# chaoting-sun/GCT-Plus

Measured on AMD Instinct MI355X. Metric: SMILES/sec training step (vaetf, seq_len=80, d_model=512), higher is better.
Workload: dtype f32

## Files before the change

gct_plus_amd/csrc/gemm.hip:

```cpp
#include <limits.h>
#include <stdlib.h>

#include <type_traits>

#include "common.h"

typedef float f32x16 __attribute__((ext_vector_type(16)));

namespace {

constexpr int BM = 128, BN = 128, BK = 32;
constexpr int TILE_FLOATS = BM * BK;

struct Seg3 {
  const float* p0;
  int64_t d1, d2;
};

struct GemmArgs {
  int64_t M, N, K;
  Seg3 a;
  int64_t lda;
  int64_t a_nper;
  Seg3 b;
  int64_t ldb;
  int64_t b_nper;
  float* c0;
  int64_t c_d1, c_d2;
  int64_t ldc;
  int64_t c_nper;
  int64_t slab_stride;
  int64_t ksplit;
  int nsplit;
  int epi;
  const float* bias0;
  int64_t bias_d1, bias_d2;
  const float* resid;
  float* pre;
  const float* pre_in;
  float keep_scale;
  uint32_t thr;
  GctRng rng;
  float* bias_slab;
  int64_t row_base;
  const int32_t* quad_map;
  int64_t pre_rows;
  const int32_t* kt_list;
  const int32_t* kt_count;
  const uint16_t* bp0;
  int64_t bp_stride;
#ifdef GCT_STAMPS
  unsigned long long* stamps;
#endif
};

enum { EPI_SLAB = 32, EPI_D0 = 16 };

__device__ __forceinline__ int64_t pre_row0(const GemmArgs& g, int64_t row) {
  if (g.pre_rows <= 0 || !g.quad_map) return row;
  const int v = g.quad_map[(row + g.row_base) >> 2];
  return v < 0 ? -1 : (int64_t)v * 4;
}

__device__ __forceinline__ uint32_t drop_quad(const GemmArgs& g, int64_t row) {
  int64_t q = (row + g.row_base) >> 2;
  if (g.quad_map) {
    const int v = g.quad_map[q];
    q = v < 0 ? 0 : v;
  }
  return (uint32_t)q;
}

#ifdef GCT_STAMPS
#define STAMP(i)                                                                       \
  do {                                                                                 \
    __builtin_amdgcn_sched_barrier(0);                                                 \
    unsigned long long t__;                                                            \
    asm volatile("s_memtime %0\n\ts_waitcnt lgkmcnt(0)" : "=s"(t__)::"memory");         \
    __builtin_amdgcn_sched_barrier(0);                                                 \
    seg[i] += t__ - tprev;                                                             \
    tprev = t__;                                                                       \
  } while (0)
#else
#define STAMP(i)
#endif

__device__ __forceinline__ const float* seg_ptr(const Seg3& s, int64_t idx, int64_t nper,
                                                int64_t& local) {
  const bool g1 = idx >= nper, g2 = idx >= 2 * nper;
  local = idx - (g2 ? 2 * nper : (g1 ? nper : 0));
  return s.p0 + (g2 ? s.d2 : (g1 ? s.d1 : 0));
}

template <bool VEC, bool SEG_ON_K>
__device__ __forceinline__ void load_kc(float4 (&r)[4], const Seg3& s, int64_t ld, int64_t nper,
                                        int64_t row0, int64_t rows, int64_t k0, int64_t kend,
                                        int tid) {
  const int c8 = tid & 7;
  const int64_t k = k0 + c8 * 4;
#pragma unroll
  for (int i = 0; i < 4; ++i) {
    const int64_t row = row0 + (tid >> 3) + 32 * i;
    float4 v = make_float4(0.f, 0.f, 0.f, 0.f);
    if (row < rows) {
      if (VEC) {
        if (k < kend) {
          int64_t loc;
          const float* base;
          if (SEG_ON_K) {
            base = seg_ptr(s, k, nper, loc);
            v = *reinterpret_cast<const float4*>(base + row * ld + loc);
          } else {
            base = seg_ptr(s, row, nper, loc);
            v = *reinterpret_cast<const float4*>(base + loc * ld + k);
          }
        }
      } else {
        float t[4] = {0.f, 0.f, 0.f, 0.f};
#pragma unroll
        for (int e = 0; e < 4; ++e) {
          if (k + e < kend) {
            int64_t loc;
            if (SEG_ON_K) {
              const float* base = seg_ptr(s, k + e, nper, loc);
              t[e] = base[row * ld + loc];
            } else {
              const float* base = seg_ptr(s, row, nper, loc);
              t[e] = base[loc * ld + k + e];
            }
          }
        }
        v = make_float4(t[0], t[1], t[2], t[3]);
      }
    }
    r[i] = v;
  }
}

template <bool VEC, bool SEG_ON_K>
__device__ __forceinline__ void load_rc(float4 (&r)[4], const Seg3& s, int64_t ld, int64_t nper,
                                        int64_t col0, int64_t cols, int64_t k0, int64_t kend,
                                        int tid) {
  const int c32 = tid & 31;
  const int64_t col = col0 + c32 * 4;
#pragma unroll
  for (int i = 0; i < 4; ++i) {
    const int64_t k = k0 + (tid >> 5) + 8 * i;
    float4 v = make_float4(0.f, 0.f, 0.f, 0.f);
    if (k < kend) {
      if (VEC) {
        if (col < cols) {
          int64_t loc;
          if (SEG_ON_K) {
            const float* base = seg_ptr(s, k, nper, loc);
            v = *reinterpret_cast<const float4*>(base + loc * ld + col);
          } else {
            const float* base = seg_ptr(s, col, nper, loc);
            v = *reinterpret_cast<const float4*>(base + k * ld + loc);
          }
        }
      } else {
        float t[4] = {0.f, 0.f, 0.f, 0.f};
#pragma unroll
        for (int e = 0; e < 4; ++e) {
          if (col + e < cols) {
            int64_t loc;
            if (SEG_ON_K) {
              const float* base = seg_ptr(s, k, nper, loc);
              t[e] = base[loc * ld + col + e];
            } else {
              const float* base = seg_ptr(s, col + e, nper, loc);
              t[e] = base[k * ld + loc];
            }
          }
        }
        v = make_float4(t[0], t[1], t[2], t[3]);
      }
    }
    r[i] = v;
  }
}

__device__ __forceinline__ void store_kc(float* lds, const float4 (&r)[4], int tid) {
  const int c8 = tid & 7;
#pragma unroll
  for (int i = 0; i < 4; ++i) {
    const int row = (tid >> 3) + 32 * i;
    const int chunk = c8 ^ ((row >> 1) & 7);
    *reinterpret_cast<float4*>(lds + row * BK + chunk * 4) = r[i];
  }
}
__device__ __forceinline__ void store_rc(float* lds, const float4 (&r)[4], int tid) {
  const int c32 = tid & 31;
#pragma unroll
  for (int i = 0; i < 4; ++i) {
    const int k = (tid >> 5) + 8 * i;
    *reinterpret_cast<float4*>(lds + k * BM + c32 * 4) = r[i];
  }
}

__device__ __forceinline__ void fragq_kc(float (&f)[2][4], const float* lds, int base, int lane,
                                         int c) {
  const int h = lane >> 5;
#pragma unroll
  for (int t = 0; t < 2; ++t) {
    const int row = base + t * 32 + (lane & 31);
    const int sw = (row >> 1) & 7;
    const float4 v = *reinterpret_cast<const float4*>(lds + row * BK + (((h * 4 + c) ^ sw) * 4));
    f[t][0] = v.x; f[t][1] = v.y; f[t][2] = v.z; f[t][3] = v.w;
  }
}
__device__ __forceinline__ void fragq_rc(float (&f)[2][4], const float* lds, int base, int lane,
                                         int c) {
  const int h = lane >> 5;
#pragma unroll
  for (int t = 0; t < 2; ++t) {
    const int col = base + t * 32 + (lane & 31);
#pragma unroll
    for (int e = 0; e < 4; ++e) f[t][e] = lds[(h * 16 + c * 4 + e) * BM + col];
  }
}

template <bool A_KC, bool B_KC, bool VEC>
__global__ __launch_bounds__(256, 2) void gemm_f32_kernel(const GemmArgs g) {
  __shared__ __attribute__((aligned(16))) float lds[4 * TILE_FLOATS];
  const int tid = threadIdx.x, lane = tid & 63, wave = tid >> 6;
  const int wm = (wave >> 1) * 64, wn = (wave & 1) * 64;

  const unsigned tiles_n = (unsigned)((g.N + BN - 1) / BN);
  const unsigned tiles_m = (unsigned)((g.M + BM - 1) / BM);
  const unsigned per_split = tiles_m * tiles_n;
  const unsigned lid = gct_xcd_remap(blockIdx.x, gridDim.x);
  const unsigned z = lid / per_split, rest = lid - z * per_split;
  const int64_t m0 = (int64_t)(rest / tiles_n) * BM, n0 = (int64_t)(rest % tiles_n) * BN;
  const int64_t kbeg = (int64_t)z * g.ksplit;
  const int64_t kend = (kbeg + g.ksplit < g.K) ? kbeg + g.ksplit : g.K;

  const Seg3 sa = g.a, sb = g.b;

  f32x16 acc[2][2];
#pragma unroll
  for (int i = 0; i < 2; ++i)
#pragma unroll
    for (int j = 0; j < 2; ++j)
#pragma unroll
      for (int r = 0; r < 16; ++r) acc[i][j][r] = 0.f;

  float4 ra[4], rb[4];
  auto gload = [&](int64_t k0) {
    if (A_KC)
      load_kc<VEC, true>(ra, sa, g.lda, g.a_nper, m0, g.M, k0, kend, tid);
    else
      load_rc<VEC, false>(ra, sa, g.lda, g.a_nper, m0, g.M, k0, kend, tid);
    if (B_KC)
      load_kc<VEC, false>(rb, sb, g.ldb, g.b_nper, n0, g.N, k0, kend, tid);
    else
      load_rc<VEC, true>(rb, sb, g.ldb, g.b_nper, n0, g.N, k0, kend, tid);
  };
  auto lstore = [&](int buf) {
    float* la = lds + buf * 2 * TILE_FLOATS;
    float* lb = la + TILE_FLOATS;
    if (A_KC) store_kc(la, ra, tid); else store_rc(la, ra, tid);
    if (B_KC) store_kc(lb, rb, tid); else store_rc(lb, rb, tid);
  };

  const int64_t nkt = (kend - kbeg + BK - 1) / BK;
#ifdef GCT_STAMPS
  unsigned long long seg[8] = {0, 0, 0, 0, 0, 0, 0, 0}, tprev;
  asm volatile("s_memtime %0\n\ts_waitcnt lgkmcnt(0)" : "=s"(tprev)::"memory");
#endif
  if (nkt > 0) {
    gload(kbeg);
    lstore(0);
  }
  __syncthreads();
  STAMP(0);
  for (int64_t kt = 0; kt < nkt; ++kt) {
    const int cur = (int)(kt & 1);
    if (kt + 1 < nkt) gload(kbeg + (kt + 1) * BK);
    STAMP(1);
    const float* la = lds + cur * 2 * TILE_FLOATS;
    const float* lb = la + TILE_FLOATS;
    float fa[2][2][4], fb[2][2][4];
    auto fragq = [&](int set, int c) {
      if (A_KC) fragq_kc(fa[set], la, wm, lane, c); else fragq_rc(fa[set], la, wm, lane, c);
      if (B_KC) fragq_kc(fb[set], lb, wn, lane, c); else fragq_rc(fb[set], lb, wn, lane, c);
    };
    fragq(0, 0);
#pragma unroll
    for (int c = 0; c < 4; ++c) {
      const int set = c & 1;
      if (c < 3) fragq(set ^ 1, c + 1);
      __builtin_amdgcn_sched_barrier(0);
#pragma unroll
      for (int e = 0; e < 4; ++e) {
#pragma unroll
        for (int i = 0; i < 2; ++i)
#pragma unroll
          for (int j = 0; j < 2; ++j)
            acc[i][j] = __builtin_amdgcn_mfma_f32_32x32x2f32(fa[set][i][e], fb[set][j][e], acc[i][j],
                                                             0, 0, 0);
      }
      __builtin_amdgcn_sched_barrier(0);
    }
    STAMP(2);
#ifdef GCT_STAMPS
    asm volatile("s_waitcnt vmcnt(0)" ::: "memory");
    STAMP(3);
#endif
    if (kt + 1 < nkt) lstore(cur ^ 1);
    STAMP(4);
    __syncthreads();
    STAMP(5);
  }

  const int h = lane >> 5;
#pragma unroll
  for (int i = 0; i < 2; ++i) {
#pragma unroll
    for (int j = 0; j < 2; ++j) {
      const int64_t col = n0 + wn + j * 32 + (lane & 31);
      if (col >= g.N) continue;
      int64_t cloc;
      float* cbase;
      float bias = 0.f;
      if (g.epi == EPI_SLAB) {
        cbase = g.c0 + (int64_t)z * g.slab_stride;
        cloc = col;
      } else {
        const bool g1 = col >= g.c_nper, g2 = col >= 2 * g.c_nper;
        cloc = col - (g2 ? 2 * g.c_nper : (g1 ? g.c_nper : 0));
        cbase = g.c0 + (g2 ? g.c_d2 : (g1 ? g.c_d1 : 0));
        if (g.epi < EPI_D0 && g.bias0)
          bias = g.bias0[(g2 ? g.bias_d2 : (g1 ? g.bias_d1 : 0)) + cloc];
      }
#pragma unroll
      for (int q4 = 0; q4 < 4; ++q4) {
        const int64_t row_base = m0 + wm + i * 32 + 8 * q4 + 4 * h;
        uint4 bits = make_uint4(~0u, ~0u, ~0u, ~0u);
        const bool need_rng = g.thr != 0u && (g.epi == GCT_EPI_GELU_DROP ||
                                              g.epi == GCT_EPI_GELU_DROP_SAVE ||
                                              g.epi == GCT_EPI_DROP_RESID ||
                                              g.epi == EPI_D0 + GCT_DEPI_GELU_BWD);
        if (need_rng) bits = gct_drop_bits(g.rng, drop_quad(g, row_base), (uint32_t)col);
#pragma unroll
        for (int e = 0; e < 4; ++e) {
          const int64_t row = row_base + e;
          if (row >= g.M) continue;
          float v = acc[i][j][q4 * 4 + e];
          const int64_t off = row * g.ldc + cloc;
          const bool keep = gct_drop_keep(bits, e, (uint32_t)col, g.thr);
          switch (g.epi) {
            case GCT_EPI_BIAS:
              v += bias;
              break;
            case GCT_EPI_GELU_DROP: {
// ... 568 lines not shown
    if (kt + 1 < nkt) gload(kbeg + (kt + 1) * BK);
    const float* la = lds + cur * 2 * STILE;
    const float* lb = la + STILE;
    const int rowa = wm + (lane & 31), rowb = wn + (lane & 31);
    const int swa = (rowa >> 1) & 7, swb = (rowb >> 1) & 7;
#pragma unroll
    for (int c = 0; c < 4; ++c) {
      const float4 a4 = *reinterpret_cast<const float4*>(la + rowa * BK + (((h * 4 + c) ^ swa) * 4));
      const float4 b4 = *reinterpret_cast<const float4*>(lb + rowb * BK + (((h * 4 + c) ^ swb) * 4));
      acc = __builtin_amdgcn_mfma_f32_32x32x2f32(a4.x, b4.x, acc, 0, 0, 0);
      acc = __builtin_amdgcn_mfma_f32_32x32x2f32(a4.y, b4.y, acc, 0, 0, 0);
      acc = __builtin_amdgcn_mfma_f32_32x32x2f32(a4.z, b4.z, acc, 0, 0, 0);
      acc = __builtin_amdgcn_mfma_f32_32x32x2f32(a4.w, b4.w, acc, 0, 0, 0);
    }
    if (kt + 1 < nkt) lstore(cur ^ 1);
    __syncthreads();
  }
  float* stg = lds + wave * 1024;
  {
    const int c32 = lane & 31;
#pragma unroll
    for (int r = 0; r < 16; ++r) stg[((r & 3) + 8 * (r >> 2) + 4 * h) * 32 + c32] = acc[r];
  }
  __builtin_amdgcn_s_waitcnt(0xC07F);
  __builtin_amdgcn_wave_barrier();
  const FastEpi ep{g};
  const int rg = lane >> 3, c4 = lane & 7;
  const int64_t row0 = m0 + wm + rg * 4, col0 = n0 + wn + c4 * 4;
  if (row0 < g.M && col0 < g.N) {
    float4 v[4];
#pragma unroll
    for (int rr = 0; rr < 4; ++rr) v[rr] = *reinterpret_cast<const float4*>(stg + (rg * 4 + rr) * 32 + c4 * 4);
    if (g.epi == EPI_SLAB) {
      float* sl = g.c0 + (int64_t)z * g.slab_stride;
#pragma unroll
      for (int rr = 0; rr < 4; ++rr)
        if (row0 + rr < g.M) *reinterpret_cast<float4*>(sl + (row0 + rr) * g.N + col0) = v[rr];
      return;
    }
    const bool q1 = col0 >= g.c_nper, q2 = col0 >= 2 * g.c_nper;
    const int64_t cloc = col0 - (q2 ? 2 * g.c_nper : (q1 ? g.c_nper : 0));
    float* cbase = g.c0 + (q2 ? g.c_d2 : (q1 ? g.c_d1 : 0));
    float4 bias = make_float4(0.f, 0.f, 0.f, 0.f);
    if (g.bias0) bias = *reinterpret_cast<const float4*>(g.bias0 + (q2 ? g.bias_d2 : (q1 ? g.bias_d1 : 0)) + cloc);
    ep.apply(v, row0, col0, cbase, cloc, bias);
  }
}


template <int TN, bool RAGGED = false>
__global__ __launch_bounds__(256) void gemm_f32_panel_kernel(const GemmArgs g) {
  constexpr int TM = 32, KC = 256, SD = KC + 4, NBL = TN / 4;
  extern __shared__ __attribute__((aligned(16))) float plds[];
  float* As = plds;
  float* Bs = plds + TM * SD;
  const int tid = threadIdx.x, lane = tid & 63, wave = tid >> 6, g4 = lane >> 4, c16 = lane & 15;
  const unsigned tiles_m = (unsigned)((g.M + TM - 1) / TM);
  const unsigned lid = gct_xcd_remap(blockIdx.x, gridDim.x);
  const int64_t m0 = (int64_t)(lid % tiles_m) * TM, n0 = (int64_t)(lid / tiles_m) * TN;
  const bool s1 = n0 >= g.b_nper, s2 = n0 >= 2 * g.b_nper;
  const float* bbase = g.b.p0 + (s2 ? g.b.d2 : (s1 ? g.b.d1 : 0)) + (n0 - (s2 ? 2 * g.b_nper : (s1 ? g.b_nper : 0))) * g.ldb;
  const float* abase = g.a.p0;
  uint32_t offa[8], offb[NBL];
#pragma unroll
  for (int i = 0; i < 8; ++i) {
    const int idx = tid + 256 * i, row = idx >> 6, c4 = idx & 63;
    int64_t r = m0 + row;
    if (r > g.M - 1) r = g.M - 1;
    offa[i] = (uint32_t)(r * g.lda + c4 * 4);
  }
#pragma unroll
  for (int i = 0; i < NBL; ++i) {
    const int idx = tid + 256 * i, c4 = idx & 63;
    int64_t row = idx >> 6;
    if (RAGGED && n0 + row > g.N - 1) row = g.N - 1 - n0;
    offb[i] = (uint32_t)(row * g.ldb + c4 * 4);
  }
  f32x4_t ra[8], rb[NBL];
  auto gload = [&](int64_t k0) {
#pragma unroll
    for (int i = 0; i < 8; ++i) ra[i] = *reinterpret_cast<const f32x4_t*>(abase + k0 + offa[i]);
#pragma unroll
    for (int i = 0; i < NBL; ++i) rb[i] = *reinterpret_cast<const f32x4_t*>(bbase + k0 + offb[i]);
  };
  auto lstore = [&]() {
#pragma unroll
    for (int i = 0; i < 8; ++i) {
      const int idx = tid + 256 * i;
      *reinterpret_cast<f32x4_t*>(As + (idx >> 6) * SD + (idx & 63) * 4) = ra[i];
    }
#pragma unroll
    for (int i = 0; i < NBL; ++i) {
      const int idx = tid + 256 * i;
      *reinterpret_cast<f32x4_t*>(Bs + (idx >> 6) * SD + (idx & 63) * 4) = rb[i];
    }
  };
  constexpr int NS = TN / 32;
  const int wm = (wave >> 1) * 16, wn = (wave & 1) * (TN / 2);
  f32x4_t acc[NS];
#pragma unroll
  for (int j = 0; j < NS; ++j) acc[j] = (f32x4_t){0.f, 0.f, 0.f, 0.f};
  const int64_t nch = g.K / KC;
  gload(0);
  lstore();
  __syncthreads();
  for (int64_t c = 0; c < nch; ++c) {
    if (c + 1 < nch) gload((c + 1) * KC);
    const float* ap = As + (wm + c16) * SD + g4 * 64;
#pragma unroll 4
    for (int j = 0; j < 16; ++j) {
      const float4 a4 = *reinterpret_cast<const float4*>(ap + 4 * j);
#pragma unroll
      for (int u = 0; u < NS; ++u) {
        const float4 b4 = *reinterpret_cast<const float4*>(Bs + (wn + 16 * u + c16) * SD + g4 * 64 + 4 * j);
        acc[u] = __builtin_amdgcn_mfma_f32_16x16x4f32(a4.x, b4.x, acc[u], 0, 0, 0);
        acc[u] = __builtin_amdgcn_mfma_f32_16x16x4f32(a4.y, b4.y, acc[u], 0, 0, 0);
        acc[u] = __builtin_amdgcn_mfma_f32_16x16x4f32(a4.z, b4.z, acc[u], 0, 0, 0);
        acc[u] = __builtin_amdgcn_mfma_f32_16x16x4f32(a4.w, b4.w, acc[u], 0, 0, 0);
      }
    }
    __syncthreads();
    if (c + 1 < nch) {
      lstore();
      __syncthreads();
    }
  }
  float* stg = plds + wave * (16 * 20);
  const FastEpi ep{g};
#pragma unroll
  for (int u = 0; u < NS; ++u) {
#pragma unroll
    for (int i = 0; i < 4; ++i) stg[(4 * g4 + i) * 20 + c16] = acc[u][i];
    __builtin_amdgcn_s_waitcnt(0xC07F);
    __builtin_amdgcn_wave_barrier();
    if (lane < 16) {
      const int pr = lane >> 2, pc = lane & 3;
      const int64_t row0 = m0 + wm + 4 * pr, col0 = n0 + wn + 16 * u + 4 * pc;
      if (RAGGED) {
        for (int rr = 0; rr < 4; ++rr)
          for (int cc = 0; cc < 4; ++cc)
            if (row0 + rr < g.M && col0 + cc < g.N)
              g.c0[(row0 + rr) * g.ldc + col0 + cc] = stg[(4 * pr + rr) * 20 + 4 * pc + cc] + (g.bias0 ? g.bias0[col0 + cc] : 0.f);
      } else if (row0 < g.M && col0 < g.N) {
        float4 v[4];
#pragma unroll
        for (int rr = 0; rr < 4; ++rr) v[rr] = *reinterpret_cast<const float4*>(stg + (4 * pr + rr) * 20 + 4 * pc);
        const bool q1 = col0 >= g.c_nper, q2 = col0 >= 2 * g.c_nper;
        const int64_t cloc = col0 - (q2 ? 2 * g.c_nper : (q1 ? g.c_nper : 0));
        float* cbase = g.c0 + (q2 ? g.c_d2 : (q1 ? g.c_d1 : 0));
        float4 bias = make_float4(0.f, 0.f, 0.f, 0.f);
        if (g.bias0) bias = *reinterpret_cast<const float4*>(g.bias0 + (q2 ? g.bias_d2 : (q1 ? g.bias_d1 : 0)) + cloc);
        ep.apply(v, row0, col0, cbase, cloc, bias);
      }
    }
    __builtin_amdgcn_s_waitcnt(0xC07F);
    __builtin_amdgcn_wave_barrier();
  }
}

template <int TN, bool RAGGED = false>
int launch_panel(const GemmArgs& g, hipStream_t st) {
  constexpr size_t LDS = (size_t)(32 + TN) * 260 * sizeof(float);
  static bool attr_set = false;
  if (!attr_set) {
    hipError_t e = hipFuncSetAttribute((const void*)gemm_f32_panel_kernel<TN, RAGGED>, hipFuncAttributeMaxDynamicSharedMemorySize, (int)LDS);
    if (e != hipSuccess) {
      gct_set_error("gemm_f32_panel: cannot reserve %zu bytes of LDS: %s", LDS, hipGetErrorString(e));
      return GCT_ERR_HIP;
    }
    attr_set = true;
  }
  const int64_t tiles = ((g.M + 31) / 32) * (RAGGED ? 1 : g.N / TN);
  hipLaunchKernelGGL((gemm_f32_panel_kernel<TN, RAGGED>), dim3((unsigned)tiles), dim3(256), LDS, st, g);
  GCT_LAUNCH_CHECK("gemm_f32_panel");
  return GCT_OK;
}

__global__ __launch_bounds__(256) void splitk_epilogue_kernel(const GemmArgs g, const float* slabs,
                                                              int nslab, int64_t slab_stride) {
  const int64_t pc = g.N / 4, pr = (g.M + 3) / 4;
  const int64_t idx = (int64_t)blockIdx.x * blockDim.x + threadIdx.x;
  if (idx >= pc * pr) return;
  const int64_t row0 = (idx / pc) * 4, col0 = (idx % pc) * 4;
  float4 v[4];
#pragma unroll
  for (int rr = 0; rr < 4; ++rr) {
    v[rr] = make_float4(0.f, 0.f, 0.f, 0.f);
    if (row0 + rr < g.M) {
      const float* p = slabs + (row0 + rr) * g.N + col0;
      for (int s = 0; s < nslab; ++s) {
        const float4 t = *reinterpret_cast<const float4*>(p + (int64_t)s * slab_stride);
        v[rr].x += t.x; v[rr].y += t.y; v[rr].z += t.z; v[rr].w += t.w;
      }
    }
  }
  const bool q1 = col0 >= g.c_nper, q2 = col0 >= 2 * g.c_nper;
  const int64_t cloc = col0 - (q2 ? 2 * g.c_nper : (q1 ? g.c_nper : 0));
  float* cbase = g.c0 + (q2 ? g.c_d2 : (q1 ? g.c_d1 : 0));
  float4 bias = make_float4(0.f, 0.f, 0.f, 0.f);
  if (g.bias0) bias = *reinterpret_cast<const float4*>(g.bias0 + (q2 ? g.bias_d2 : (q1 ? g.bias_d1 : 0)) + cloc);
  const FastEpi ep{g};
  ep.apply(v, row0, col0, cbase, cloc, bias);
}

int g_gemm_mode = -1;
int64_t g_gemm_launches[2] = {0, 0};
inline int gemm_mode() {
  if (g_gemm_mode < 0) {
    const char* e = getenv("GCT_GEMM_MODE");
    g_gemm_mode = (e && (e[0] == 'f' || e[0] == '0')) ? GCT_GEMM_F32 : GCT_GEMM_BF16X6;
  }
  return g_gemm_mode;
}

template <bool A_KC, bool B_KC>
bool fast_ok(const GemmArgs& g, bool vec) {
  auto seg_ok = [](int64_t nper, int64_t extent, int64_t gran) { return nper >= extent || nper % gran == 0; };
  return vec && g.K % BK == 0 && g.ksplit % BK == 0 && g.M >= 4 && g.N >= 4 &&
         (A_KC ? seg_ok(g.a_nper, g.K, BK) : (seg_ok(g.a_nper, g.M, BM) && g.M % 4 == 0)) &&
         (B_KC ? seg_ok(g.b_nper, g.N, BN) : (seg_ok(g.b_nper, g.K, BK) && g.N % 4 == 0)) &&
         g.N % 4 == 0 && g.ldc % 4 == 0 && gct_aligned16(g.c0) && g.c_d1 % 4 == 0 && g.c_d2 % 4 == 0 &&
         (g.c_nper >= g.N || g.c_nper % 4 == 0) && g.slab_stride % 4 == 0 &&
         (!g.bias0 || (gct_aligned16(g.bias0) && g.bias_d1 % 4 == 0 && g.bias_d2 % 4 == 0)) &&
         (!g.resid || gct_aligned16(g.resid)) && (!g.pre || gct_aligned16(g.pre)) &&
         (!g.pre_in || gct_aligned16(g.pre_in)) && 130 * g.lda < (1ll << 31) && 130 * g.ldb < (1ll << 31);
}


inline int64_t slab_bytes(int64_t s, int64_t rows, int64_t cols) {
  return s > 1 ? s * rows * cols * (int64_t)sizeof(float) : 0;
}

inline bool skinny_m(int64_t M, int64_t N) { return ((M + BM - 1) / BM) * ((N + BN - 1) / BN) < 192; }

int skinny_splits(int64_t M, int64_t N, int64_t K) {
  const int64_t tiles = ((M + 63) / 64) * ((N + 63) / 64);
  if (tiles <= 0) return 1;
  int64_t ns = 768 / tiles;
  if (ns > K / BK / 4) ns = K / BK / 4;
  return ns < 1 ? 1 : (int)ns;
}

int x6_tail_plan(int64_t M, int64_t N, int64_t K, int64_t* m1_out) {
  constexpr int64_t CUS = 256;
  const int64_t tm = (M + XBM - 1) / XBM, tn = (N + XBN - 1) / XBN, tiles = tm * tn;
  const int64_t rem = tiles % CUS;
  if (tiles <= CUS || rem == 0 || rem % tn != 0 || K % XBK != 0) return 1;
  const int64_t nkt = K / XBK;
  int best = 1;
  double cost = 1.0;
  const double o = 3.3;
  for (int s2 = 2; s2 <= 8 && nkt / s2 >= 2; ++s2) {
    const double c = (double)((rem * s2 + CUS - 1) / CUS) * (o + (double)nkt / s2) / (o + nkt) + 0.05;
    if (c < cost - 1e-9) { cost = c; best = s2; }
  }
  if (best == 1 || cost > 0.75) return 1;
  *m1_out = (tiles - rem) / tn * XBM;
  return best;
}

int x6_splitk_all_plan(int64_t M, int64_t N, int64_t K) {
  constexpr int64_t CUS = 256;
  const int64_t tiles = ((M + XBM - 1) / XBM) * ((N + XBN - 1) / XBN), nkt = K / XBK;
  if (tiles > CUS / 2 || K % XBK != 0 || nkt < 32 || M < 1024 || (nkt < 64 && M < 2048)) return 1;
  int64_t sp = CUS / tiles;
  if (sp > nkt / 8) sp = nkt / 8;
  if (sp > 8) sp = 8;
  return sp < 2 ? 1 : (int)sp;
}


inline int64_t x6s_tiles(int64_t M, int64_t N) { return ((M + SBM - 1) / SBM) * ((N + SBN - 1) / SBN); }

inline bool x6s_shape(const GemmArgs& g) {
  const int64_t big = ((g.M + XBM - 1) / XBM) * ((g.N + XBN - 1) / XBN), small = x6s_tiles(g.M, g.N), nkt = g.K / XBK;
  return big <= 160 && small >= 96 && small <= (nkt <= 16 ? 512 : 256) && nkt <= 32;
}

constexpr int64_t X6_TAIL_SMALL_MAX = 512;

constexpr int64_t PANEL32_MAX_TILES = 4096, PANEL64_MAX_TILES = 768;


static_assert(BK == XBK, "the fp32 and bf16x6 kernels split K at the same granularity");
GemmArgs slab_args(const GemmArgs& g, int splits, float* ws) {
  const int64_t nkt = g.K / BK;
  GemmArgs p = g;
  p.ksplit = ((nkt + splits - 1) / splits) * BK;
  p.nsplit = (int)((g.K + p.ksplit - 1) / p.ksplit);
  p.epi = EPI_SLAB; p.c0 = ws; p.ldc = g.N; p.slab_stride = g.M * g.N;
  p.c_d1 = p.c_d2 = 0; p.c_nper = INT64_MAX / 4; p.bias0 = nullptr; p.resid = nullptr; p.pre = nullptr; p.pre_in = nullptr;
  return p;
}

int launch_fixup(const GemmArgs& g, const GemmArgs& slabs, hipStream_t st, const char* name) {
  const int64_t patches = ((g.M + 3) / 4) * (g.N / 4);
  hipLaunchKernelGGL(splitk_epilogue_kernel, dim3((unsigned)((patches + 255) / 256)), dim3(256), 0, st, g,
                     (const float*)slabs.c0, slabs.nsplit, slabs.slab_stride);
  GCT_LAUNCH_CHECK(name);
  return GCT_OK;
}

template <int MODE, int NP>
int launch_x6_tail_split(const GemmArgs& g, hipStream_t st, float* ws, int64_t ws_bytes) {
  if (MODE == X6_WGRAD || g.nsplit != 1 || !ws || !gct_aligned16(ws)) return launch_x6<MODE, NP>(g, st);
  int64_t m1 = 0;
  const int best = x6_tail_plan(g.M, g.N, g.K, &m1);
  const int64_t m2 = g.M - m1, nkt = g.K / XBK;
  hipStreamCaptureStatus cap = hipStreamCaptureStatusNone;
  if (best == 1 || slab_bytes(best, m2, g.N) > ws_bytes ||
      hipStreamIsCapturing(st, &cap) != hipSuccess || cap != hipStreamCaptureStatusNone)
    return launch_x6<MODE, NP>(g, st);
  GemmArgs head = g;
  head.M = m1;
  int rc = launch_x6<MODE, NP>(head, st);
  if (rc) return rc;
  GemmArgs e = g;
  e.M = m2; e.row_base = g.row_base + m1;
  e.a.p0 += m1 * g.lda;
  e.c0 += m1 * g.ldc;
  if (e.resid) e.resid += m1 * g.ldc;
  if (e.pre) e.pre += m1 * g.ldc;
  if (e.pre_in && !(g.pre_rows > 0 && g.quad_map)) e.pre_in += m1 * g.ldc;
  if (nkt <= 32 && x6s_tiles(m2, g.N) <= X6_TAIL_SMALL_MAX) {
    if (MODE == X6_FWD && x6s_ok(e, true)) return launch_x6s<X6_FWD, NP>(e, st);
    if (MODE == X6_DGRAD && x6s_dgrad_ok(e, true)) return launch_x6s<X6_DGRAD, NP>(e, st);
  }
  const GemmArgs p = slab_args(e, best, ws);
  rc = launch_x6<MODE, NP>(p, st);
  if (rc) return rc;
  return launch_fixup(e, p, st, "x6 tail fix-up");
}

struct GemmRoute {
  enum Kind {
    X6S,
    X6_SPLITK_ALL,
    PANEL_THIN,
    PANEL32,
    PANEL64,
    F32_SMALL,
    X6,
    F32_FAST,
    F32_VEC,
    F32,
  } kind;
  int splits;
};

template <bool A_KC, bool B_KC>
GemmRoute plan_gemm(const GemmArgs& g, bool vec, int mode, const float* ws, int64_t ws_bytes) {
  constexpr bool FWD = A_KC && B_KC, DGRAD = A_KC && !B_KC;
  constexpr int MODE = A_KC ? (B_KC ? X6_FWD : X6_DGRAD) : X6_WGRAD;
  const bool x6 = mode == GCT_GEMM_BF16X6 || mode == GCT_GEMM_BF16X3;
  const bool x6_fwd = x6 && FWD && g.epi < EPI_D0, x6_dgrad = x6 && DGRAD && g.epi >= EPI_D0 && g.epi < EPI_SLAB;
  const bool ws_ok = ws && gct_aligned16(ws);
  if (x6_fwd || x6_dgrad) {
    const bool x6s = x6_fwd ? x6s_ok(g, vec) : x6s_dgrad_ok(g, vec);
    if (x6s && x6s_shape(g)) return {GemmRoute::X6S, 1};
    if (x6_fwd && x6s && !x6_ok<X6_FWD>(g, vec) && x6s_tiles(g.M, g.N) >= 96) return {GemmRoute::X6S, 1};
    const int sp = x6_splitk_all_plan(g.M, g.N, g.K);
    if (x6_ok<MODE>(g, vec) && g.nsplit == 1 && ws_ok && sp > 1 && slab_bytes(sp, g.M, g.N) <= ws_bytes)
      return {GemmRoute::X6_SPLITK_ALL, sp};
  }
  if (FWD && vec && g.N <= 32 && g.K % 256 == 0 && g.epi == GCT_EPI_BIAS && g.nsplit == 1 && g.b_nper >= g.N &&
      g.c_nper >= g.N && g.M >= 1 && g.lda * 4 * 33 < (1ll << 31) && g.ldb * 4 * 33 < (1ll << 31) && g.M < (1ll << 36))
    return {GemmRoute::PANEL_THIN, 1};
  const bool fast = fast_ok<A_KC, B_KC>(g, vec);
  if (FWD && fast && g.nsplit == 1 && skinny_m(g.M, g.N) && g.epi < EPI_D0 && (g.b_nper >= g.N || g.b_nper % 64 == 0)) {
    if (g.K % 256 == 0 && g.lda * 4 * 33 < (1ll << 31) && g.ldb * 4 * 65 < (1ll << 31) &&
        (g.c_nper >= g.N || g.c_nper % 64 == 0)) {
      const int64_t tm32 = (g.M + 31) / 32;
      if (g.N % 32 == 0 && (g.b_nper >= g.N || g.b_nper % 32 == 0) && tm32 * (g.N / 32) <= PANEL32_MAX_TILES)
        return {GemmRoute::PANEL32, 1};
      if (g.N % 64 == 0 && tm32 * (g.N / 64) <= PANEL64_MAX_TILES) return {GemmRoute::PANEL64, 1};
    }
    int64_t ns = 1;
    if (ws_ok) {
      const int64_t slab = g.M * g.N * (int64_t)sizeof(float);
      ns = skinny_splits(g.M, g.N, g.K);
      if (ns * slab > ws_bytes) ns = ws_bytes / slab;
      if (ns < 1) ns = 1;
    }
    return {GemmRoute::F32_SMALL, (int)ns};
  }
  if (x6 && (A_KC || !B_KC) && x6_ok<MODE>(g, vec)) return {GemmRoute::X6, 1};
  return {fast ? GemmRoute::F32_FAST : (vec ? GemmRoute::F32_VEC : GemmRoute::F32), 1};
}

template <bool A_KC, bool B_KC>
int launch(const GemmArgs& g, bool vec, hipStream_t st, float* ws = nullptr, int64_t ws_bytes = 0) {
  constexpr int MODE = A_KC ? (B_KC ? X6_FWD : X6_DGRAD) : X6_WGRAD;
  const int64_t tiles = ((g.M + BM - 1) / BM) * ((g.N + BN - 1) / BN) * g.nsplit;
  if (tiles <= 0) return GCT_OK;
  if (tiles > INT_MAX) {
    gct_set_error("gemm: grid too large");
    return GCT_ERR_ARG;
  }
  const int mode = gemm_mode();
  const bool x3 = mode == GCT_GEMM_BF16X3;
  const GemmRoute r = plan_gemm<A_KC, B_KC>(g, vec, mode, ws, ws_bytes);
  switch (r.kind) {
    case GemmRoute::X6S:
      if (x3) return launch_x6s<B_KC ? X6_FWD : X6_DGRAD, 2>(g, st);
      ++g_gemm_launches[1];
      return launch_x6s<B_KC ? X6_FWD : X6_DGRAD, 3>(g, st);
    case GemmRoute::X6_SPLITK_ALL: {
      const GemmArgs p = slab_args(g, r.splits, ws);
      int rc = x3 ? launch_x6<MODE, 2>(p, st) : launch_x6<MODE, 3>(p, st);
      if (!rc) rc = launch_fixup(g, p, st, "x6 split-K fix-up");
      if (!rc && !x3) ++g_gemm_launches[1];
      return rc;
    }
    case GemmRoute::PANEL_THIN:
      ++g_gemm_launches[0];
      return launch_panel<32, true>(g, st);
    case GemmRoute::PANEL32:
      return launch_panel<32>(g, st);
    case GemmRoute::PANEL64:
      return launch_panel<64>(g, st);
    case GemmRoute::F32_SMALL: {
      const int64_t tiles64 = ((g.M + 63) / 64) * ((g.N + 63) / 64);
      if (r.splits == 1) {
        hipLaunchKernelGGL(gemm_f32_small_kernel, dim3((unsigned)tiles64), dim3(256), 0, st, g);
        GCT_LAUNCH_CHECK("gemm_f32_small");
        return GCT_OK;
      }
      const GemmArgs p = slab_args(g, r.splits, ws);
      hipLaunchKernelGGL(gemm_f32_small_kernel, dim3((unsigned)(tiles64 * p.nsplit)), dim3(256), 0, st, p);
      GCT_LAUNCH_CHECK("gemm_f32_small(split-K)");
      return launch_fixup(g, p, st, "splitk_epilogue");
    }
    case GemmRoute::X6:
      if (x3) return launch_x6_tail_split<MODE, 2>(g, st, ws, ws_bytes);
      ++g_gemm_launches[1];
      return launch_x6_tail_split<MODE, 3>(g, st, ws, ws_bytes);
    default:
      break;
  }
  ++g_gemm_launches[0];
  const dim3 grid((unsigned)tiles), block(256);
  if (r.kind == GemmRoute::F32_FAST)
    hipLaunchKernelGGL((gemm_f32_fast_kernel<A_KC, B_KC>), grid, block, 0, st, g);
  else if (r.kind == GemmRoute::F32_VEC)
    hipLaunchKernelGGL((gemm_f32_kernel<A_KC, B_KC, true>), grid, block, 0, st, g);
  else
    hipLaunchKernelGGL((gemm_f32_kernel<A_KC, B_KC, false>), grid, block, 0, st, g);
  GCT_LAUNCH_CHECK("gemm_f32");
  return GCT_OK;
}

inline bool al16(const void* p) { return p == nullptr || gct_aligned16(p); }

inline Seg3 mkseg(const float* p0, const float* p1, const float* p2) {
  Seg3 r;
  r.p0 = p0;
  r.d1 = p1 ? (int64_t)(p1 - p0) : 0;
  r.d2 = p2 ? (int64_t)(p2 - p0) : 0;
  return r;
}

}

int gct_reduce_slabs_seg(const float* slabs, int nslab, int64_t stride, float* d0, float* d1,
                         float* d2, int64_t nper_elems, int64_t n, hipStream_t st);
int gct_reduce_slabs_seg2(const float* sa, int nslab, int64_t stride_a, float* a0, float* a1, float* a2,
                          int64_t nper_a, int64_t na, const float* sb, int64_t stride_b, float* b0, float* b1,
                          float* b2, int64_t nper_b, int64_t nb, hipStream_t st);
int gct_colsum(const float* y0, const float* y1, const float* y2, int64_t ld, int64_t M, int nseg,
               int nper, float* d0, float* d1, float* d2, float* ws, hipStream_t st);
int64_t gct_colsum_ws_floats(int64_t M, int64_t N);

static int wgrad_splits(int64_t M, int64_t Ntot, int64_t K, bool x6 = false) {
  const int64_t tiles = x6 ? ((Ntot + XBM - 1) / XBM) * ((K + XBN - 1) / XBN)
                           : ((Ntot + BM - 1) / BM) * ((K + BN - 1) / BN);
  int64_t want = (x6 ? 256 : 512) / tiles;
  const int64_t maxs = (M + 4 * BK - 1) / (4 * BK);
  if (want > maxs) want = maxs;
  if (want < 1) want = 1;
  if (want > 64) want = 64;
  return (int)want;
}

extern "C" int64_t gct_wgrad_ws_bytes(int64_t M, int64_t Ntot, int64_t K) {
  const int s1 = wgrad_splits(M, Ntot, K), s2 = wgrad_splits(M, Ntot, K, true);
  const int s = s1 > s2 ? s1 : s2;
  const int64_t slab = (int64_t)s * Ntot * K;
  const int64_t cs = gct_colsum_ws_floats(M, Ntot);
  const int64_t need = slab + 4 + (int64_t)s * Ntot;
  return (need > cs ? need : cs) * (int64_t)sizeof(float) + 256;
}

extern "C" int gct_linear_fwd(const float* x, int64_t ldx, int64_t M, int K, const float* w0,
                              const float* w1, const float* w2, int64_t ldw, const uint16_t* wp0,
                              int64_t plane_stride, const float* b0, const float* b1,
                              const float* b2, int nseg, int nper, float* y0, float* y1, float* y2,
                              int64_t ldy, int epi, const float* resid, float* pre, float p,
                              uint64_t seed, uint32_t site, float* ws, int64_t ws_bytes,
                              const int32_t* quad_map, void* stream) {
  GCT_CHECK_ARG(x && w0 && y0 && M >= 0 && K > 0 && nseg >= 1 && nseg <= 3 && nper > 0,
                "linear_fwd: bad args");
  GCT_CHECK_ARG(!quad_map || M % 4 == 0, "linear_fwd: compacted rows come in quads");
  GCT_CHECK_ARG(ws_bytes >= 0, "linear_fwd: negative workspace size");
  GCT_CHECK_ARG(nseg < 2 || (w1 && y1), "linear_fwd: missing segment 1");
  GCT_CHECK_ARG(nseg < 3 || (w2 && y2), "linear_fwd: missing segment 2");
  GCT_CHECK_ARG(epi == GCT_EPI_BIAS || nseg == 1, "linear_fwd: fused epilogues need nseg == 1");
  GCT_CHECK_ARG(epi >= GCT_EPI_BIAS && epi <= GCT_EPI_GELU_DROP_SAVE, "linear_fwd: unknown epilogue %d", epi);
  GCT_CHECK_ARG((epi != GCT_EPI_GELU_DROP && epi != GCT_EPI_GELU_DROP_SAVE) || pre, "linear_fwd: GELU epilogue needs pre");
  GCT_CHECK_ARG(epi != GCT_EPI_DROP_RESID || resid, "linear_fwd: residual epilogue needs resid");
  GCT_CHECK_ARG(p >= 0.f && p < 1.f, "linear_fwd: dropout p out of range");
  GemmArgs g = {};
  g.M = M; g.N = (int64_t)nseg * nper; g.K = K;
  GCT_CHECK_ARG(!b0 || nseg < 2 || b1, "linear_fwd: bias of segment 1 missing");
  GCT_CHECK_ARG(!b0 || nseg < 3 || b2, "linear_fwd: bias of segment 2 missing");
  g.a = mkseg(x, nullptr, nullptr); g.lda = ldx; g.a_nper = INT64_MAX / 4;
  g.b = mkseg(w0, w1, w2); g.ldb = ldw; g.b_nper = nper;
  g.c0 = y0; g.c_d1 = y1 ? y1 - y0 : 0; g.c_d2 = y2 ? y2 - y0 : 0; g.ldc = ldy; g.c_nper = nper;
  g.ksplit = K; g.nsplit = 1; g.epi = epi;
  g.bias0 = b0; g.bias_d1 = (b0 && b1) ? b1 - b0 : 0; g.bias_d2 = (b0 && b2) ? b2 - b0 : 0;
  g.resid = resid; g.pre = pre;
  g.thr = gct_drop_threshold(p); g.keep_scale = 1.0f / (1.0f - p); g.rng = gct_rng_make(seed, site);
  g.bp0 = wp0; g.bp_stride = plane_stride;
  g.quad_map = quad_map;
  const bool vec = al16(x) && al16(w0) && al16(w1) && al16(w2) && (ldx % 4 == 0) &&
                   (ldw % 4 == 0) && (K % 4 == 0);
  return launch<true, true>(g, vec, (hipStream_t)stream, ws, ws ? ws_bytes : 0);
}

extern "C" int gct_gemm_set_mode(int mode) {
  GCT_CHECK_ARG(mode == GCT_GEMM_F32 || mode == GCT_GEMM_BF16X6 || mode == GCT_GEMM_BF16X3,
                "gemm_set_mode: unknown mode %d", mode);
  g_gemm_mode = mode;
  return GCT_OK;
}
extern "C" int gct_gemm_get_mode(void) { return gemm_mode(); }
extern "C" int64_t gct_gemm_x6_kernel_launches(void) { return g_x6_kernel_launches; }
extern "C" int64_t gct_gemm_x3_launches(void) { return g_x3_kernel_launches; }
extern "C" int gct_gemm_launch_counts(int64_t* out2) {
  GCT_CHECK_ARG(out2, "gemm_launch_counts: null");
  out2[0] = g_gemm_launches[0]; out2[1] = g_gemm_launches[1];
  return GCT_OK;
}

extern "C" int gct_split_planes(const float* src, int64_t numel, uint16_t* planes, int64_t plane_stride,
                                void* stream) {
  GCT_CHECK_ARG(src && planes && numel >= 0 && numel % 4 == 0 && plane_stride >= numel && plane_stride % 4 == 0 &&
                    gct_aligned16(src) && ((((uintptr_t)planes) & 7u) == 0),
                "split_planes: bad args (numel and plane_stride must be multiples of 4, src 16-B aligned)");
  if (numel == 0) return GCT_OK;
  const int64_t n4 = numel / 4;
  hipLaunchKernelGGL(split_planes_kernel, dim3((unsigned)((n4 + 255) / 256)), dim3(256), 0, (hipStream_t)stream,
                     src, planes, n4, plane_stride);
  GCT_LAUNCH_CHECK("split_planes");
  return GCT_OK;
}

extern "C" int64_t gct_linear_fwd_ws_bytes(int64_t M, int K, int Ntot) {
  int64_t need = 0, m1 = 0;
  if (skinny_m(M, Ntot)) {
    need = slab_bytes(skinny_splits(M, Ntot, K), M, Ntot);
  } else {
    const int s = x6_tail_plan(M, Ntot, K, &m1);
    need = slab_bytes(s, M - m1, Ntot);
  }
  const int64_t all = slab_bytes(x6_splitk_all_plan(M, Ntot, K), M, Ntot);
  return (need > all ? need : all) + 256;
}

extern "C" int64_t gct_linear_dgrad_ws_bytes(int64_t M, int Ntot, int K) {
  int64_t m1 = 0;
  const int s = x6_tail_plan(M, K, Ntot, &m1);
  const int64_t tail = slab_bytes(s, M - m1, K);
  const int64_t all = slab_bytes(x6_splitk_all_plan(M, K, Ntot), M, K);
  return (tail > all ? tail : all) + 256;
}

extern "C" int gct_linear_dgrad(const float* dy0, const float* dy1, const float* dy2, int64_t lddy,
                                int64_t M, int nseg, int nper, const float* w0, const float* w1,
                                const float* w2, int64_t ldw, const uint16_t* wp0,
                                int64_t plane_stride, int K, float* dx, int64_t lddx, int depi,
                                const float* pre, float p, uint64_t seed, uint32_t site,
                                float* ws, int64_t ws_bytes, const int32_t* quad_map, int64_t pre_rows,
                                void* stream) {
  GCT_CHECK_ARG(ws_bytes >= 0, "linear_dgrad: negative workspace size");
  GCT_CHECK_ARG(dy0 && w0 && dx && M >= 0 && K > 0 && nseg >= 1 && nseg <= 3 && nper > 0,
                "linear_dgrad: bad args");
  GCT_CHECK_ARG(!quad_map || M % 4 == 0, "linear_dgrad: compacted rows come in quads");
  GCT_CHECK_ARG(nseg < 2 || (w1 && dy1), "linear_dgrad: missing segment 1");
  GCT_CHECK_ARG(nseg < 3 || (w2 && dy2), "linear_dgrad: missing segment 2");
  GCT_CHECK_ARG(depi >= GCT_DEPI_STORE && depi <= GCT_DEPI_MUL_SAVED, "linear_dgrad: unknown epilogue %d", depi);
  GCT_CHECK_ARG(depi != GCT_DEPI_GELU_BWD || pre, "linear_dgrad: GELU bwd needs pre");
  GCT_CHECK_ARG(depi != GCT_DEPI_MUL_SAVED || pre, "linear_dgrad: saved-factor epilogue needs pre");
  GCT_CHECK_ARG(p >= 0.f && p < 1.f, "linear_dgrad: dropout p out of range");
  GemmArgs g = {};
  g.M = M; g.N = K; g.K = (int64_t)nseg * nper;
  g.a = mkseg(dy0, dy1, dy2); g.lda = lddy; g.a_nper = nper;
  g.b = mkseg(w0, w1, w2); g.ldb = ldw; g.b_nper = nper;
  g.c0 = dx; g.ldc = lddx; g.c_nper = INT64_MAX / 4;
  g.ksplit = g.K; g.nsplit = 1; g.epi = EPI_D0 + depi;
  g.pre_in = pre;
  g.thr = gct_drop_threshold(p); g.keep_scale = 1.0f / (1.0f - p); g.rng = gct_rng_make(seed, site);
  g.bp0 = wp0; g.bp_stride = plane_stride;
  g.quad_map = quad_map;
  g.pre_rows = quad_map ? pre_rows : 0;
  const bool vec = al16(dy0) && al16(dy1) && al16(dy2) && al16(w0) && al16(w1) && al16(w2) &&
                   (lddy % 4 == 0) && (ldw % 4 == 0) && (nper % 4 == 0) && (K % 4 == 0);
  return launch<true, false>(g, vec, (hipStream_t)stream, ws, ws ? ws_bytes : 0);
}

extern "C" int gct_linear_wgrad(const float* dy0, const float* dy1, const float* dy2, int64_t lddy,
                                int64_t M, int nseg, int nper, const float* x, int64_t ldx, int K,
                                float* dw0, float* dw1, float* dw2, int64_t lddw, float* db0,
                                float* db1, float* db2, float* ws, const int32_t* tile_list,
                                const int32_t* tile_count, void* stream) {
  GCT_CHECK_ARG(dy0 && x && dw0 && ws && M >= 0 && K > 0 && nseg >= 1 && nseg <= 3 && nper > 0,
                "linear_wgrad: bad args");
  GCT_CHECK_ARG(nseg < 2 || (dy1 && dw1), "linear_wgrad: missing segment 1");
  GCT_CHECK_ARG(nseg < 3 || (dy2 && dw2), "linear_wgrad: missing segment 2");
  GCT_CHECK_ARG(lddw == K, "linear_wgrad: dW must be dense [nper][K]");
  hipStream_t st = (hipStream_t)stream;
  const int64_t Ntot = (int64_t)nseg * nper;
  const bool vec = al16(dy0) && al16(dy1) && al16(dy2) && al16(x) && (lddy % 4 == 0) &&
                   (ldx % 4 == 0) && (nper % 4 == 0) && (K % 4 == 0);
  GemmArgs g = {};
  g.M = Ntot; g.N = K; g.K = M;
  g.a = mkseg(dy0, dy1, dy2); g.lda = lddy; g.a_nper = nper;
  g.b = mkseg(x, nullptr, nullptr); g.ldb = ldx; g.b_nper = INT64_MAX / 4;
  g.c0 = ws; g.ldc = K; g.c_nper = INT64_MAX / 4;
  g.slab_stride = Ntot * K;
  g.ksplit = BK; g.nsplit = 1; g.epi = EPI_SLAB;
  const bool use_x6 = gemm_mode() != GCT_GEMM_F32 && x6_ok<X6_WGRAD>(g, vec);
  if (use_x6 && tile_list && tile_count) { g.kt_list = tile_list; g.kt_count = tile_count; }
  const int splits = wgrad_splits(M, Ntot, K, use_x6);
  int64_t ks = (M + splits - 1) / splits;
  ks = (ks + BK - 1) / BK * BK;
  g.ksplit = ks > 0 ? ks : BK;
  g.nsplit = (int)((M + g.ksplit - 1) / g.ksplit);
  if (g.nsplit < 1) g.nsplit = 1;
  g.epi = EPI_SLAB;
  float* bslab = nullptr;
  if (db0) {
    if (use_x6 || fast_ok<false, false>(g, vec)) {
      int64_t off = (int64_t)g.nsplit * g.slab_stride;
      off = (off + 3) / 4 * 4;
      bslab = ws + off;
      g.bias_slab = bslab;
    } else {
      int rc = gct_colsum(dy0, dy1, dy2, lddy, M, nseg, nper, db0, db1, db2, ws, st);
      if (rc) return rc;
    }
  }
  int rc = launch<false, false>(g, vec, st);
  if (rc) return rc;
  if (bslab)
    return gct_reduce_slabs_seg2(ws, g.nsplit, g.slab_stride, dw0, dw1, dw2, (int64_t)nper * K, Ntot * K, bslab, Ntot,
                                 db0, db1, db2, nper, Ntot, st);
  return gct_reduce_slabs_seg(ws, g.nsplit, g.slab_stride, dw0, dw1, dw2, (int64_t)nper * K, Ntot * K, st);
}
```

gct_plus_amd/csrc/gemm_x6.inc:

```

typedef __bf16 x6_bf16x8 __attribute__((ext_vector_type(8)));
typedef __bf16 x6_bf16x2 __attribute__((ext_vector_type(2)));
typedef float x6_f32x2 __attribute__((ext_vector_type(2)));
typedef unsigned x6_u32x4 __attribute__((ext_vector_type(4)));
typedef unsigned x6_u32x2 __attribute__((ext_vector_type(2)));
typedef short x6_s16x4 __attribute__((ext_vector_type(4)));
typedef short x6_s16x8 __attribute__((ext_vector_type(8)));

enum { X6_FWD = 0, X6_DGRAD = 1, X6_WGRAD = 2 };
constexpr int XBM = 128, XBN = 256, XBK = 32;
constexpr int X_APL = 8192, X_BPL = 16384, X_STAGE = 3 * X_APL + 3 * X_BPL;
constexpr int X_KLIST_MAX = 1024;
constexpr int X_LDS_BYTES = 2 * X_STAGE + X_KLIST_MAX * 4;

__device__ __forceinline__ unsigned x6_pk(float a, float b) {
  x6_f32x2 v = {a, b};
  return __builtin_bit_cast(unsigned, __builtin_convertvector(v, x6_bf16x2));
}
__device__ __forceinline__ float x6_sub(float a, float b) {
  float r;
  asm("v_sub_f32 %0, %1, %2" : "=v"(r) : "v"(a), "v"(b));
  return r;
}
__device__ __forceinline__ void x6_split2(float a, float b, unsigned& h, unsigned& m, unsigned& l) {
  h = x6_pk(a, b);
  const float ra = x6_sub(a, __uint_as_float(h << 16)), rb = x6_sub(b, __uint_as_float(h & 0xffff0000u));
  m = x6_pk(ra, rb);
  const float sa = x6_sub(ra, __uint_as_float(m << 16)), sb = x6_sub(rb, __uint_as_float(m & 0xffff0000u));
  l = x6_pk(sa, sb);
}
__device__ __forceinline__ void x6_split4(const float4 v, x6_u32x2& h, x6_u32x2& m, x6_u32x2& l) {
  unsigned h0, m0, l0, h1, m1, l1;
  x6_split2(v.x, v.y, h0, m0, l0);
  x6_split2(v.z, v.w, h1, m1, l1);
  h = x6_u32x2{h0, h1}; m = x6_u32x2{m0, m1}; l = x6_u32x2{l0, l1};
}
template <int NP>
__device__ __forceinline__ void x6_split4n(const float4 v, x6_u32x2 (&pc)[NP]) {
  if constexpr (NP == 3) {
    x6_split4(v, pc[0], pc[1], pc[2]);
  } else {
    static_assert(NP == 2, "bf16x6 (3 pieces) or bf16x3 (2 pieces)");
    unsigned h0, h1;
    h0 = x6_pk(v.x, v.y);
    h1 = x6_pk(v.z, v.w);
    const float r0 = x6_sub(v.x, __uint_as_float(h0 << 16)), r1 = x6_sub(v.y, __uint_as_float(h0 & 0xffff0000u));
    const float r2 = x6_sub(v.z, __uint_as_float(h1 << 16)), r3 = x6_sub(v.w, __uint_as_float(h1 & 0xffff0000u));
    pc[0] = x6_u32x2{h0, h1};
    pc[1] = x6_u32x2{x6_pk(r0, r1), x6_pk(r2, r3)};
  }
}

__device__ __forceinline__ int x6_row_off(int r, int c) {
  const int g = (0x78 >> (2 * ((r >> 2) & 3))) & 3;
  return r * 64 + ((c ^ g) << 4);
}
__device__ __forceinline__ int x6_tr_off(int k, int cb, int stride) {
  return k * stride + (cb ^ (((k & 3) << 6) | (((k >> 3) & 1) << 5)));
}

__device__ __forceinline__ x6_bf16x8 x6_tr_frag(const unsigned char* p, int stride) {
  typedef __attribute__((address_space(3))) x6_s16x4 lds_s16x4;
  const x6_s16x4 lo = __builtin_amdgcn_ds_read_tr16_b64_v4i16((lds_s16x4*)(p));
  const x6_s16x4 hi = __builtin_amdgcn_ds_read_tr16_b64_v4i16((lds_s16x4*)(p + 4 * stride));
  const x6_s16x8 v = __builtin_shufflevector(lo, hi, 0, 1, 2, 3, 4, 5, 6, 7);
  return __builtin_bit_cast(x6_bf16x8, v);
}

typedef float x6_f32x4 __attribute__((ext_vector_type(4)));
#define X6_MFMA(a_, b_, c_) c_ = __builtin_amdgcn_mfma_f32_16x16x32_bf16(a_, b_, c_, 0, 0, 0)

template <int MODE, int NP = 3>
__global__ __launch_bounds__(512) __attribute__((amdgpu_waves_per_eu(2, 2))) void
gemm_x6_kernel(const GemmArgs g) {
  static_assert(NP == 2 || NP == 3, "bf16x3 or bf16x6");
  extern __shared__ __attribute__((aligned(16))) unsigned char xlds[];
  constexpr bool A_TR = MODE == X6_WGRAD, B_TR = MODE != X6_FWD, B_PL = MODE != X6_WGRAD;
  constexpr int NB = B_PL ? 2 : 4;
  const int tid = threadIdx.x, lane = tid & 63, wave = tid >> 6;
  const int wm = (wave >> 2) * 64, wn = (wave & 3) * 64;

  const unsigned tiles_n = (unsigned)((g.N + XBN - 1) / XBN);
  const unsigned tiles_m = (unsigned)((g.M + XBM - 1) / XBM);
  const unsigned per_split = tiles_m * tiles_n;
  const unsigned lid = gct_xcd_remap(blockIdx.x, gridDim.x);
  const unsigned z = lid / per_split, rest = lid - z * per_split;
  const int64_t m0 = (int64_t)(rest / tiles_n) * XBM, n0 = (int64_t)(rest % tiles_n) * XBN;
  const int64_t kbeg = (int64_t)z * g.ksplit;
  const int64_t kend = (kbeg + g.ksplit < g.K) ? kbeg + g.ksplit : g.K;

  uint32_t offa[2], offb[NB];
  int sta[2], stb[NB];
#pragma unroll
  for (int j = 0; j < 2; ++j) {
    if (!A_TR) {
      int64_t r = (tid >> 3) + 64 * j;
      sta[j] = x6_row_off((int)r, (tid & 7) >> 1) + (tid & 1) * 8;
      if (m0 + r > g.M - 1) r = g.M - 1 - m0;
      offa[j] = (uint32_t)(r * g.lda + (tid & 7) * 4);
    } else {
      const int kr = (tid >> 5) + 16 * j;
      int64_t c = (tid & 31) * 4;
      sta[j] = x6_tr_off(kr, (tid & 31) * 8, 256);
      if (m0 + c > g.M - 4) c = g.M - 4 - m0;
      offa[j] = (uint32_t)(kr * g.lda + c);
    }
  }
#pragma unroll
  for (int j = 0; j < NB; ++j) {
    if (MODE == X6_FWD) {
      int64_t r = (tid >> 2) + 128 * j;
      stb[j] = x6_row_off((int)r, tid & 3);
      if (n0 + r > g.N - 1) r = g.N - 1 - n0;
      offb[j] = (uint32_t)(r * g.ldb + (tid & 3) * 8);
    } else if (MODE == X6_DGRAD) {
      const int kr = (tid >> 5) + 16 * j;
      int64_t c = (tid & 31) * 8;
      stb[j] = x6_tr_off(kr, (tid & 31) * 16, 512);
      if (n0 + c > g.N - 8) c = g.N - 8 - n0;
      offb[j] = (uint32_t)(kr * g.ldb + c);
    } else {
      const int kr = (tid >> 6) + 8 * j;
      int64_t c = (tid & 63) * 4;
      stb[j] = x6_tr_off(kr, (tid & 63) * 8, 512);
      if (n0 + c > g.N - 4) c = g.N - 4 - n0;
      offb[j] = (uint32_t)(kr * g.ldb + c);
    }
  }
  auto seg_off = [](const Seg3& s, int64_t idx, int64_t nper, int64_t& local) -> int64_t {
    const bool g1 = idx >= nper, g2 = idx >= 2 * nper;
    local = idx - (g2 ? 2 * nper : (g1 ? nper : 0));
    return g2 ? s.d2 : (g1 ? s.d1 : 0);
  };
  int64_t a_fix = 0, b_fix = 0;
  {
    int64_t loc;
    if (A_TR) { a_fix = seg_off(g.a, m0, g.a_nper, loc); a_fix += loc; }
    else a_fix = m0 * g.lda;
    if (MODE == X6_FWD) { b_fix = seg_off(g.b, n0, g.b_nper, loc); b_fix += loc * g.ldb; }
    else b_fix = n0;
  }
  auto abase = [&](int64_t k0) -> const float* {
    if (A_TR) return g.a.p0 + a_fix + k0 * g.lda;
    int64_t loc;
    const int64_t so = seg_off(g.a, k0, g.a_nper, loc);
    return g.a.p0 + so + a_fix + loc;
  };
  auto boff = [&](int64_t k0) -> int64_t {
    if (MODE == X6_FWD) return b_fix + k0;
    int64_t loc;
    const int64_t so = seg_off(g.b, k0, g.b_nper, loc);
    return so + loc * g.ldb + b_fix;
  };

  x6_f32x4 acc[4][4];
#pragma unroll
  for (int i = 0; i < 4; ++i)
#pragma unroll
    for (int j = 0; j < 4; ++j) acc[i][j] = x6_f32x4{0.f, 0.f, 0.f, 0.f};

  float4 pa[2];
  x6_u32x4 pbp[NP][2];
  float4 pbf[4];
#define X6_GLOAD(k0_)                                                                          \
  do {                                                                                         \
    const float* ab__ = abase(k0_);                                                            \
    const int64_t bo__ = boff(k0_);                                                            \
    _Pragma("unroll") for (int j = 0; j < 2; ++j)                                              \
        pa[j] = *reinterpret_cast<const float4*>(ab__ + offa[j]);                              \
    if (B_PL) {                                                                                \
      _Pragma("unroll") for (int p = 0; p < NP; ++p)                                           \
      _Pragma("unroll") for (int j = 0; j < 2; ++j)                                            \
          pbp[p][j] = *reinterpret_cast<const x6_u32x4*>(g.bp0 + p * g.bp_stride + bo__ + offb[j]); \
    } else {                                                                                   \
      _Pragma("unroll") for (int j = 0; j < 4; ++j)                                            \
          pbf[j] = *reinterpret_cast<const float4*>(g.b.p0 + bo__ + offb[j]);                  \
    }                                                                                          \
  } while (0)
#define X6_LSTORE(st_)                                                                         \
  do {                                                                                         \
    unsigned char* s__ = (st_);                                                                \
    _Pragma("unroll") for (int j = 0; j < 2; ++j) {                                            \
      x6_u32x2 pc__[NP];                                                                       \
      x6_split4n<NP>(pa[j], pc__);                                                             \
      _Pragma("unroll") for (int p = 0; p < NP; ++p)                                           \
          *reinterpret_cast<x6_u32x2*>(s__ + p * X_APL + sta[j]) = pc__[p];                    \
    }                                                                                          \
    if (B_PL) {                                                                                \
      _Pragma("unroll") for (int p = 0; p < NP; ++p)                                           \
      _Pragma("unroll") for (int j = 0; j < 2; ++j)                                            \
          *reinterpret_cast<x6_u32x4*>(s__ + 3 * X_APL + p * X_BPL + stb[j]) = pbp[p][j];      \
    } else {                                                                                   \
      _Pragma("unroll") for (int j = 0; j < 4; ++j) {                                          \
        x6_u32x2 pc__[NP];                                                                     \
        x6_split4n<NP>(pbf[j], pc__);                                                          \
        _Pragma("unroll") for (int p = 0; p < NP; ++p)                                         \
            *reinterpret_cast<x6_u32x2*>(s__ + 3 * X_APL + p * X_BPL + stb[j]) = pc__[p];      \
      }                                                                                        \
    }                                                                                          \
  } while (0)

  constexpr bool BAL = B_PL;
  x6_u32x2 pk[2][NP];
#define X6_GLOAD_A(k0_)                                                                        \
  do {                                                                                         \
    const float* ab__ = abase(k0_);                                                            \
    _Pragma("unroll") for (int j = 0; j < 2; ++j)                                              \
        pa[j] = *reinterpret_cast<const float4*>(ab__ + offa[j]);                              \
  } while (0)
#define X6_GLOAD_B(k0_)                                                                        \
  do {                                                                                         \
    const int64_t bo__ = boff(k0_);                                                            \
    _Pragma("unroll") for (int p = 0; p < NP; ++p)                                             \
    _Pragma("unroll") for (int j = 0; j < 2; ++j)                                              \
        pbp[p][j] = *reinterpret_cast<const x6_u32x4*>(g.bp0 + p * g.bp_stride + bo__ + offb[j]); \
  } while (0)
#define X6_SPLIT_A()                                                                           \
  _Pragma("unroll") for (int j = 0; j < 2; ++j) x6_split4n<NP>(pa[j], pk[j]);
#define X6_LSTORE_PK(st_)                                                                      \
  do {                                                                                         \
    unsigned char* s__ = (st_);                                                                \
    _Pragma("unroll") for (int j = 0; j < 2; ++j)                                              \
    _Pragma("unroll") for (int p = 0; p < NP; ++p)                                             \
        *reinterpret_cast<x6_u32x2*>(s__ + p * X_APL + sta[j]) = pk[j][p];                     \
    _Pragma("unroll") for (int p = 0; p < NP; ++p)                                             \
    _Pragma("unroll") for (int j = 0; j < 2; ++j)                                              \
        *reinterpret_cast<x6_u32x4*>(s__ + 3 * X_APL + p * X_BPL + stb[j]) = pbp[p][j];        \
  } while (0)

  const int fr = lane & 15, fc = lane >> 4;
  const int tq = (lane & 15) >> 2, tp = lane & 3;
  int fao[4], fbo[4];
#pragma unroll
  for (int i = 0; i < 4; ++i) {
    fao[i] = A_TR ? x6_tr_off(8 * fc + tq, (wm + 16 * i + 4 * tp) * 2, 256) : x6_row_off(wm + 16 * i + fr, fc);
    fbo[i] = 3 * X_APL + (B_TR ? x6_tr_off(8 * fc + tq, (wn + 16 * i + 4 * tp) * 2, 512)
                               : x6_row_off(wn + 16 * i + fr, fc));
  }
  x6_bf16x8 fA01[2][NP], fA23[2][NP], fB01[2][NP], fB23[2][NP];
#define X6_LD_A(dst_, st_, i0_)                                                                \
  _Pragma("unroll") for (int ii = 0; ii < 2; ++ii)                                             \
  _Pragma("unroll") for (int p = 0; p < NP; ++p) {                                             \
    if (A_TR) dst_[ii][p] = x6_tr_frag((st_) + p * X_APL + fao[(i0_) + ii], 256);              \
    else dst_[ii][p] = *reinterpret_cast<const x6_bf16x8*>((st_) + p * X_APL + fao[0] + ((i0_) + ii) * 1024); \
  }
#define X6_LD_B(dst_, st_, j0_)                                                                \
  _Pragma("unroll") for (int jj = 0; jj < 2; ++jj)                                             \
  _Pragma("unroll") for (int p = 0; p < NP; ++p) {                                             \
    if (B_TR) dst_[jj][p] = x6_tr_frag((st_) + p * X_BPL + fbo[(j0_) + jj], 512);              \
    else dst_[jj][p] = *reinterpret_cast<const x6_bf16x8*>((st_) + p * X_BPL + fbo[0] + ((j0_) + jj) * 1024); \
  }
#define X6_MM(a_, b_, i0_, j0_)                                                                \
  _Pragma("unroll") for (int ii = 0; ii < 2; ++ii)                                             \
  _Pragma("unroll") for (int jj = 0; jj < 2; ++jj) {                                           \
    if constexpr (NP == 3) {                                                                   \
      X6_MFMA(a_[ii][NP - 1], b_[jj][0], acc[(i0_) + ii][(j0_) + jj]);                         \
      X6_MFMA(a_[ii][0], b_[jj][NP - 1], acc[(i0_) + ii][(j0_) + jj]);                         \
      X6_MFMA(a_[ii][1], b_[jj][1], acc[(i0_) + ii][(j0_) + jj]);                              \
    }                                                                                          \
    X6_MFMA(a_[ii][1], b_[jj][0], acc[(i0_) + ii][(j0_) + jj]);                                \
    X6_MFMA(a_[ii][0], b_[jj][1], acc[(i0_) + ii][(j0_) + jj]);                                \
    X6_MFMA(a_[ii][0], b_[jj][0], acc[(i0_) + ii][(j0_) + jj]);                                \
  }

  float4 bsum = make_float4(0.f, 0.f, 0.f, 0.f);
  const float bw0 = (MODE == X6_WGRAD && g.bias_slab && n0 == 0) ? 1.f : 0.f;
#define X6_BSUM(w_)                                                                            \
  _Pragma("unroll") for (int j = 0; j < 2; ++j) {                                              \
    bsum.x = fmaf(w_, pa[j].x, bsum.x); bsum.y = fmaf(w_, pa[j].y, bsum.y);                    \
    bsum.z = fmaf(w_, pa[j].z, bsum.z); bsum.w = fmaf(w_, pa[j].w, bsum.w);                    \
  }

#ifdef GCT_STAMPS
  unsigned long long seg[8] = {0, 0, 0, 0, 0, 0, 0, 0}, tprev;
  asm volatile("s_memtime %0\n\ts_waitcnt lgkmcnt(0)" : "=s"(tprev)::"memory");
#endif
  int64_t nkt = (kend - kbeg) / XBK;
  int64_t lt0 = 0;
  const int32_t* klist = (MODE == X6_WGRAD) ? g.kt_list : nullptr;
  if (klist) {
    const int64_t cnt = *g.kt_count;
    const int64_t per = (cnt + g.nsplit - 1) / g.nsplit;
    lt0 = (int64_t)z * per;
    nkt = cnt - lt0 < per ? cnt - lt0 : per;
    if (nkt < 0) nkt = 0;
  }
  int32_t* kl_s = reinterpret_cast<int32_t*>(xlds + 2 * X_STAGE);
  const bool kl_cached = klist && nkt <= X_KLIST_MAX;
  if (kl_cached) {
    for (int i = tid; i < nkt; i += 512) kl_s[i] = klist[lt0 + i];
    __syncthreads();
  }
  auto ktile = [&](int64_t t) -> int64_t {
    const int64_t tc = t < nkt ? t : nkt - 1;
    if (kl_cached) return (int64_t)__builtin_amdgcn_readfirstlane(kl_s[tc]) * XBK;
    return klist ? (int64_t)klist[lt0 + tc] * XBK : kbeg + tc * XBK;
  };
  if (nkt > 0) {
    if (BAL) {
      X6_GLOAD_A(ktile(0));
      X6_GLOAD_B(ktile(0));
      X6_SPLIT_A()
      X6_LSTORE_PK(xlds);
      X6_GLOAD_A(ktile(1));
      X6_GLOAD_B(ktile(1));
      X6_SPLIT_A()
      X6_GLOAD_A(ktile(2));
    } else {
      X6_GLOAD(ktile(0));
      if (MODE == X6_WGRAD) { X6_BSUM(bw0) }
      X6_LSTORE(xlds);
      X6_GLOAD(ktile(1));
    }
  }
  __syncthreads();
  if (nkt > 0) {
    X6_LD_A(fA01, xlds, 0)
    X6_LD_B(fB01, xlds, 0)
  }
  STAMP(0);
  constexpr int RA = 2 * NP * (A_TR ? 2 : 1), RB = 2 * NP * (B_TR ? 2 : 1);
  constexpr int NWR = B_PL ? 4 * NP : 6 * NP;
  constexpr int NG = 2 * NP;
  constexpr int MPW = NP == 3 ? 2 : 1;
  auto ktile_in = [&](int64_t t) -> int64_t { return kbeg + t * XBK; };
  int64_t k2n = nkt > 0 ? ktile(2) : 0;
  const int64_t mw = m0 + wm, nw = n0 + wn;
  constexpr int SIDE = MODE == X6_FWD ? 1 : (MODE == X6_DGRAD ? 2 : 3);
  EpiLane el;
  EpiAhead ah;
  float4 ex[4][4];
  int qv[4];
  if (BAL) epi_ahead_quads<SIDE>(g, lane, mw, nw, qv);
  auto ktile_iter = [&](auto tail_c, const int64_t kt) __attribute__((always_inline)) {
    constexpr int TAIL = decltype(tail_c)::value;
    constexpr bool NEXT1 = TAIL != 1 && TAIL != 4, NEXT2 = TAIL == 0 || TAIL == 3, NEXT3 = TAIL == 0, AHEAD = TAIL == 4;
    unsigned char* st = xlds + (kt & 1) * X_STAGE;
    unsigned char* stn = xlds + ((kt + 1) & 1) * X_STAGE;
    const int64_t k2 = k2n;
    if (TAIL == 0) k2n = BAL ? ktile_in(kt + 3) : ktile(kt + 3);
    __builtin_amdgcn_sched_barrier(0);
    X6_LD_A(fA23, st, 2)
    X6_LD_B(fB23, st, 2)
    if (MODE == X6_WGRAD) {
      const float bw = (kt + 1 < nkt) ? bw0 : 0.f;
      X6_BSUM(bw)
    }
    if (BAL) {
      if (NEXT1) { X6_LSTORE_PK(stn); }
      if (NEXT2) { X6_GLOAD_B(k2); }
      if (AHEAD) epi_ahead_issue<0, 1>(g, ah, ex);
    } else {
      X6_LSTORE(stn);
    }
    X6_MM(fA01, fB01, 0, 0)
    X6_MM(fA23, fB01, 2, 0)
#pragma unroll
    for (int q = 0; q < NG; ++q) {
      __builtin_amdgcn_sched_group_barrier(0x008, 1, 0);
      __builtin_amdgcn_sched_group_barrier(0x100, (RA + RB) / NG, 0);
    }
    if (BAL) {
#pragma unroll
      for (int q = 0; q < (NEXT1 ? NWR : 0); ++q) {
        __builtin_amdgcn_sched_group_barrier(0x008, MPW, 0);
        __builtin_amdgcn_sched_group_barrier(0x200, 1, 0);
      }
#pragma unroll
      for (int q = 0; q < (NEXT2 ? 2 * NP : (AHEAD ? 4 : 0)); ++q) {
        __builtin_amdgcn_sched_group_barrier(0x008, 2, 0);
        __builtin_amdgcn_sched_group_barrier(0x020, 1, 0);
      }
    } else {
#pragma unroll
      for (int q = 0; q < (NP == 3 ? 21 : 8); ++q) {
        __builtin_amdgcn_sched_group_barrier(0x008, 1, 0);
        __builtin_amdgcn_sched_group_barrier(0x002, NP == 3 ? 6 : 9, 0);
      }
#pragma unroll
      for (int q = 0; q < NWR; ++q) {
        __builtin_amdgcn_sched_group_barrier(0x008, 1, 0);
        __builtin_amdgcn_sched_group_barrier(0x200, 1, 0);
      }
    }
    __builtin_amdgcn_sched_barrier(0);
    STAMP(1);
    __syncthreads();
    STAMP(2);
    if (NEXT1) { X6_LD_B(fB01, stn, 0) }
    if (BAL) {
      if (NEXT2) { X6_SPLIT_A() }
      if (NEXT3) { X6_GLOAD_A(k2n); }
      if (AHEAD) epi_ahead_issue<1, 2>(g, ah, ex);
    } else {
      X6_GLOAD(k2);
    }
    X6_MM(fA01, fB23, 0, 2)
#pragma unroll
    for (int q = 0; q < (NEXT1 ? NG : 0); ++q) {
      __builtin_amdgcn_sched_group_barrier(0x008, 1, 0);
      __builtin_amdgcn_sched_group_barrier(0x100, RB / NG, 0);
    }
    if (BAL) {
#pragma unroll
      for (int q = 0; q < (NEXT2 ? (NP == 3 ? 14 : 6) : 0); ++q) {
        __builtin_amdgcn_sched_group_barrier(0x008, 1, 0);
        __builtin_amdgcn_sched_group_barrier(0x002, NP == 3 ? 3 : 4, 0);
      }
      if (NEXT3) {
        __builtin_amdgcn_sched_group_barrier(0x008, 2, 0);
        __builtin_amdgcn_sched_group_barrier(0x020, 2, 0);
      }
#pragma unroll
      for (int q = 0; q < (AHEAD ? 4 : 0); ++q) {
        __builtin_amdgcn_sched_group_barrier(0x008, 2, 0);
        __builtin_amdgcn_sched_group_barrier(0x020, 1, 0);
      }
    } else {
#pragma unroll
      for (int q = 0; q < (NP == 3 ? 8 : 4); ++q) {
        __builtin_amdgcn_sched_group_barrier(0x008, 2, 0);
        __builtin_amdgcn_sched_group_barrier(0x020, 1, 0);
      }
    }
    __builtin_amdgcn_sched_barrier(0);
    if (NEXT1) { X6_LD_A(fA01, stn, 0) }
    if (AHEAD) epi_ahead_issue<2, 4>(g, ah, ex);
    X6_MM(fA23, fB23, 2, 2)
#pragma unroll
    for (int q = 0; q < (AHEAD ? 8 : 0); ++q) {
      __builtin_amdgcn_sched_group_barrier(0x008, 2, 0);
      __builtin_amdgcn_sched_group_barrier(0x020, 1, 0);
    }
#pragma unroll
    for (int q = 0; q < (NEXT1 ? NG : 0); ++q) {
      __builtin_amdgcn_sched_group_barrier(0x008, 1, 0);
      __builtin_amdgcn_sched_group_barrier(0x100, RA / NG, 0);
    }
    __builtin_amdgcn_sched_barrier(0);
    STAMP(3);
    };
  if (BAL) {
    int64_t kt = 0;
    for (; kt < nkt - 3; ++kt) ktile_iter(std::integral_constant<int, 0>{}, kt);
    el = epi_lane(g, lane, nw, z);
    const bool ahead = nkt > 0 && epi_ahead_ok<SIDE>(g);
    ah.have = 0;
    if (ahead) ah = epi_ahead_plan<SIDE>(g, el, lane, mw, qv);
    if (nkt >= 3) ktile_iter(std::integral_constant<int, 3>{}, nkt - 3);
    if (nkt >= 2) ktile_iter(std::integral_constant<int, 2>{}, nkt - 2);
    if (ahead) ktile_iter(std::integral_constant<int, 4>{}, nkt - 1);
    else if (nkt >= 1) ktile_iter(std::integral_constant<int, 1>{}, nkt - 1);
  } else {
    for (int64_t kt = 0; kt < nkt; ++kt) ktile_iter(std::integral_constant<int, 0>{}, kt);
    __syncthreads();
  }
#undef X6_GLOAD
#undef X6_GLOAD_A
#undef X6_GLOAD_B
#undef X6_SPLIT_A
#undef X6_LSTORE_PK
#undef X6_LSTORE
#undef X6_LD_A
#undef X6_LD_B
#undef X6_MM
#undef X6_BSUM
  if (MODE == X6_WGRAD) {
    if (g.bias_slab && n0 == 0) {
      float4* red = reinterpret_cast<float4*>(xlds);
      red[tid] = bsum;
      __syncthreads();
      if (tid < 32) {
        float4 t4 = red[tid];
        for (int r = 1; r < 16; ++r) {
          const float4 u = red[r * 32 + tid];
          t4.x += u.x; t4.y += u.y; t4.z += u.z; t4.w += u.w;
        }
        const int64_t col = m0 + tid * 4;
        if (col + 3 < g.M) *reinterpret_cast<float4*>(g.bias_slab + (int64_t)z * g.M + col) = t4;
      }
      __syncthreads();
    }
  }
  STAMP(4);
  {
    float* stg = reinterpret_cast<float*>(xlds) + wave * 4096;
#pragma unroll
    for (int i = 0; i < 4; ++i)
#pragma unroll
      for (int j = 0; j < 4; ++j)
#pragma unroll
        for (int r = 0; r < 4; ++r) stg[(16 * i + 4 * fc + r) * 64 + 16 * j + fr] = acc[i][j][r];
#ifdef GCT_LAB_NO_EPI
    if (acc[0][0][0] == 123456.789f)
#endif
    {
      if (BAL) wave_epilogue_finish<SIDE>(g, stg, lane, mw, el, ex, ah.have);
      else wave_epilogue_tail<SIDE>(g, stg, lane, mw, nw, z);
    }
  }
#ifdef GCT_STAMPS
  __builtin_amdgcn_s_waitcnt(0x0070);
  STAMP(5);
  if (g.stamps && (threadIdx.x & 63) == 0 && blockIdx.x < 64) {
    for (int i = 0; i < 8; ++i) g.stamps[((size_t)blockIdx.x * 8 + (threadIdx.x >> 6)) * 8 + i] = seg[i];
  }
#endif
}

template <int MODE>
bool x6_ok(const GemmArgs& g, bool vec, int fwd_bn = XBN) {
  auto seg_ok = [](int64_t nper, int64_t extent, int64_t gran) { return nper >= extent || nper % gran == 0; };
  const bool common = vec && g.K % XBK == 0 && g.ksplit % XBK == 0 && g.K >= XBK && g.M >= 8 && g.N >= 8 &&
      g.N % 4 == 0 && g.ldc % 4 == 0 && gct_aligned16(g.c0) && g.c_d1 % 4 == 0 && g.c_d2 % 4 == 0 &&
      (g.c_nper >= g.N || g.c_nper % 4 == 0) && g.slab_stride % 4 == 0 &&
      (!g.bias0 || (gct_aligned16(g.bias0) && g.bias_d1 % 4 == 0 && g.bias_d2 % 4 == 0)) &&
      (!g.resid || gct_aligned16(g.resid)) && (!g.pre || gct_aligned16(g.pre)) &&
      (!g.pre_in || gct_aligned16(g.pre_in)) && 130 * g.lda < (1ll << 31) && 260 * g.ldb < (1ll << 31);
  if (!common) return false;
  if (MODE == X6_FWD)
    return g.bp0 && seg_ok(g.a_nper, g.K, XBK) && seg_ok(g.b_nper, g.N, fwd_bn) && g.ldb % 8 == 0 &&
           g.b.d1 % 8 == 0 && g.b.d2 % 8 == 0 && g.bp_stride % 8 == 0 && (((uintptr_t)g.bp0) & 15u) == 0;
  if (MODE == X6_DGRAD)
    return g.bp0 && seg_ok(g.a_nper, g.K, XBK) && seg_ok(g.b_nper, g.K, XBK) && g.N % 8 == 0 && g.ldb % 8 == 0 &&
           g.b.d1 % 8 == 0 && g.b.d2 % 8 == 0 && g.bp_stride % 8 == 0 && (((uintptr_t)g.bp0) & 15u) == 0;
  return seg_ok(g.a_nper, g.M, XBM) && g.M % 4 == 0;
}

template <int MODE, int NP>
int launch_x6(const GemmArgs& g, hipStream_t st) {
  const int64_t tiles = ((g.M + XBM - 1) / XBM) * ((g.N + XBN - 1) / XBN) * g.nsplit;
  if (tiles <= 0) return GCT_OK;
  if (tiles > INT_MAX) {
    gct_set_error("gemm_x6: grid too large");
    return GCT_ERR_ARG;
  }
  static bool attr_set = false;
  if (!attr_set) {
    hipError_t e = hipFuncSetAttribute((const void*)gemm_x6_kernel<MODE, NP>,
                                       hipFuncAttributeMaxDynamicSharedMemorySize, X_LDS_BYTES);
    if (e != hipSuccess) {
      gct_set_error("gemm_x6: cannot reserve %d bytes of LDS: %s", X_LDS_BYTES, hipGetErrorString(e));
      return GCT_ERR_HIP;
    }
    attr_set = true;
  }
  hipLaunchKernelGGL((gemm_x6_kernel<MODE, NP>), dim3((unsigned)tiles), dim3(512), X_LDS_BYTES, st, g);
  ++(NP == 3 ? g_x6_kernel_launches : g_x3_kernel_launches);
  GCT_LAUNCH_CHECK("gemm_x6");
  return GCT_OK;
}

constexpr int SBM = 64, SBN = 128;
constexpr int XS_APL = SBM * 64, XS_BPL = SBN * 64, XS_STAGE = 3 * XS_APL + 3 * XS_BPL;
constexpr int XS_LDS_BYTES = 2 * XS_STAGE;

template <int MODE, int NP = 3>
__global__ __launch_bounds__(512) void gemm_x6s_kernel(const GemmArgs g) {
  static_assert(NP == 2 || NP == 3, "bf16x3 or bf16x6");
  extern __shared__ __attribute__((aligned(16))) unsigned char xlds[];
  constexpr bool B_TR = MODE == X6_DGRAD;
  const int tid = threadIdx.x, lane = tid & 63, wave = tid >> 6;
  const int wm = (wave >> 2) * 32, wn = (wave & 3) * 32;
  const unsigned tiles_n = (unsigned)((g.N + SBN - 1) / SBN);
  const unsigned lid = gct_xcd_remap(blockIdx.x, gridDim.x);
  const int64_t m0 = (int64_t)(lid / tiles_n) * SBM, n0 = (int64_t)(lid % tiles_n) * SBN;
  int64_t ra = tid >> 3, rb = tid >> 2;
  const int sta = x6_row_off((int)ra, (tid & 7) >> 1) + (tid & 1) * 8;
  const int stb = B_TR ? x6_tr_off(tid >> 4, (tid & 15) * 16, 256) : x6_row_off((int)rb, tid & 3);
  if (m0 + ra > g.M - 1) ra = g.M - 1 - m0;
  if (n0 + rb > g.N - 1) rb = g.N - 1 - n0;
  const float* ap = g.a.p0 + (m0 + ra) * g.lda + (tid & 7) * 4;
  int64_t bo;
  if (B_TR) {
    int64_t c = (tid & 15) * 8;
    if (n0 + c > g.N - 8) c = g.N - 8 - n0;
    bo = (int64_t)(tid >> 4) * g.ldb + n0 + c;
  } else {
    const bool s1 = n0 >= g.b_nper, s2 = n0 >= 2 * g.b_nper;
    bo = (s2 ? g.b.d2 : (s1 ? g.b.d1 : 0)) + (n0 - (s2 ? 2 * g.b_nper : (s1 ? g.b_nper : 0)) + rb) * g.ldb + (tid & 3) * 8;
  }
  const uint16_t* bp = g.bp0 + bo;
  auto koff = [&](int64_t k0, int64_t& ao, int64_t& bko) {
    if (!B_TR) { ao = k0; bko = k0; return; }
    const bool a1 = k0 >= g.a_nper, a2 = k0 >= 2 * g.a_nper;
    ao = (a2 ? g.a.d2 : (a1 ? g.a.d1 : 0)) + (k0 - (a2 ? 2 * g.a_nper : (a1 ? g.a_nper : 0)));
    const bool b1 = k0 >= g.b_nper, b2 = k0 >= 2 * g.b_nper;
    bko = (b2 ? g.b.d2 : (b1 ? g.b.d1 : 0)) + (k0 - (b2 ? 2 * g.b_nper : (b1 ? g.b_nper : 0))) * g.ldb;
  };

  x6_f32x4 acc[2][2];
#pragma unroll
  for (int i = 0; i < 2; ++i)
#pragma unroll
    for (int j = 0; j < 2; ++j) acc[i][j] = x6_f32x4{0.f, 0.f, 0.f, 0.f};
  float4 pa;
  x6_u32x4 pb[NP];
  auto gload = [&](int64_t k0) {
    int64_t ao, bko;
    koff(k0, ao, bko);
    pa = *reinterpret_cast<const float4*>(ap + ao);
#pragma unroll
    for (int p = 0; p < NP; ++p) pb[p] = *reinterpret_cast<const x6_u32x4*>(bp + p * g.bp_stride + bko);
  };
  auto lstore = [&](unsigned char* st) {
    x6_u32x2 pc[NP];
    x6_split4n<NP>(pa, pc);
#pragma unroll
    for (int p = 0; p < NP; ++p) *reinterpret_cast<x6_u32x2*>(st + p * XS_APL + sta) = pc[p];
#pragma unroll
    for (int p = 0; p < NP; ++p) *reinterpret_cast<x6_u32x4*>(st + 3 * XS_APL + p * XS_BPL + stb) = pb[p];
  };
  const int fr = lane & 15, fc = lane >> 4;
  const int tq = (lane & 15) >> 2, tp = lane & 3;
  const int fao = x6_row_off(wm + fr, fc);
  int fbo[2];
#pragma unroll
  for (int j = 0; j < 2; ++j)
    fbo[j] = 3 * XS_APL + (B_TR ? x6_tr_off(8 * fc + tq, (wn + 16 * j + 4 * tp) * 2, 256)
                                : x6_row_off(wn + fr, fc) + j * 1024);
  const int64_t nkt = g.K / XBK;
  gload(0);
  lstore(xlds);
  if (nkt > 1) gload(XBK);
  __syncthreads();
  for (int64_t kt = 0; kt < nkt; ++kt) {
    const unsigned char* st = xlds + (kt & 1) * XS_STAGE;
    x6_bf16x8 fa[2][NP], fb[2][NP];
#pragma unroll
    for (int i = 0; i < 2; ++i)
#pragma unroll
      for (int p = 0; p < NP; ++p) {
        fa[i][p] = *reinterpret_cast<const x6_bf16x8*>(st + p * XS_APL + fao + i * 1024);
        if (B_TR) fb[i][p] = x6_tr_frag(st + p * XS_BPL + fbo[i], 256);
        else fb[i][p] = *reinterpret_cast<const x6_bf16x8*>(st + p * XS_BPL + fbo[i]);
      }
    if (kt + 1 < nkt) lstore(xlds + ((kt + 1) & 1) * XS_STAGE);
    if (kt + 2 < nkt) gload((kt + 2) * XBK);
#pragma unroll
    for (int i = 0; i < 2; ++i)
#pragma unroll
      for (int j = 0; j < 2; ++j) {
        if constexpr (NP == 3) {
          X6_MFMA(fa[i][NP - 1], fb[j][0], acc[i][j]);
          X6_MFMA(fa[i][0], fb[j][NP - 1], acc[i][j]);
          X6_MFMA(fa[i][1], fb[j][1], acc[i][j]);
        }
        X6_MFMA(fa[i][1], fb[j][0], acc[i][j]);
        X6_MFMA(fa[i][0], fb[j][1], acc[i][j]);
        X6_MFMA(fa[i][0], fb[j][0], acc[i][j]);
      }
#ifndef GCT_X6S_PLAIN
    __builtin_amdgcn_sched_group_barrier(0x100, NP == 3 ? (B_TR ? 15 : 9) : (B_TR ? 10 : 6), 0);
#pragma unroll
    for (int q = 0; q < (NP == 3 ? 3 : 2); ++q) {
      __builtin_amdgcn_sched_group_barrier(0x008, NP == 3 ? 2 : 1, 0);
      __builtin_amdgcn_sched_group_barrier(0x100, 1, 0);
    }
#pragma unroll
    for (int q = 0; q < (NP == 3 ? 6 : 3); ++q) {
      __builtin_amdgcn_sched_group_barrier(0x008, 1, 0);
      __builtin_amdgcn_sched_group_barrier(0x002, NP == 3 ? 5 : 4, 0);
    }
#pragma unroll
    for (int q = 0; q < 2 * NP; ++q) {
      __builtin_amdgcn_sched_group_barrier(0x008, 1, 0);
      __builtin_amdgcn_sched_group_barrier(0x200, 1, 0);
    }
#pragma unroll
    for (int q = 0; q < NP + 1; ++q) {
      __builtin_amdgcn_sched_group_barrier(0x008, 1, 0);
      __builtin_amdgcn_sched_group_barrier(0x020, 1, 0);
    }
    if constexpr (NP == 3) __builtin_amdgcn_sched_group_barrier(0x008, 2, 0);
#endif
    __syncthreads();
  }
  float* stg = reinterpret_cast<float*>(xlds) + wave * 1024;
#pragma unroll
  for (int i = 0; i < 2; ++i)
#pragma unroll
    for (int j = 0; j < 2; ++j)
#pragma unroll
      for (int r = 0; r < 4; ++r) stg[(16 * i + 4 * fc + r) * 32 + 16 * j + fr] = acc[i][j][r];
  __builtin_amdgcn_s_waitcnt(0xC07F);
  __builtin_amdgcn_wave_barrier();
  const FastEpiT<MODE == X6_FWD ? 1 : 2> ep{g};
  const int rg = lane >> 3, c4 = lane & 7;
  const int64_t row0 = m0 + wm + rg * 4, col0 = n0 + wn + c4 * 4;
  if (row0 < g.M && col0 < g.N) {
    float4 v[4];
#pragma unroll
    for (int rr = 0; rr < 4; ++rr) v[rr] = *reinterpret_cast<const float4*>(stg + (rg * 4 + rr) * 32 + c4 * 4);
    const bool q1 = col0 >= g.c_nper, q2 = col0 >= 2 * g.c_nper;
    const int64_t cloc = col0 - (q2 ? 2 * g.c_nper : (q1 ? g.c_nper : 0));
    float* cbase = g.c0 + (q2 ? g.c_d2 : (q1 ? g.c_d1 : 0));
    float4 bias = make_float4(0.f, 0.f, 0.f, 0.f);
    if (g.epi < EPI_D0 && g.bias0)
      bias = *reinterpret_cast<const float4*>(g.bias0 + (q2 ? g.bias_d2 : (q1 ? g.bias_d1 : 0)) + cloc);
    ep.apply(v, row0, col0, cbase, cloc, bias);
  }
}

inline bool x6s_ok(const GemmArgs& g, bool vec) {
  return x6_ok<X6_FWD>(g, vec, SBN) && g.nsplit == 1 && g.a_nper >= g.K && (g.b_nper >= g.N || g.b_nper % SBN == 0) &&
         (g.c_nper >= g.N || g.c_nper % 4 == 0) && g.epi < EPI_D0 && 70 * g.lda < (1ll << 31);
}
inline bool x6s_dgrad_ok(const GemmArgs& g, bool vec) {
  return x6_ok<X6_DGRAD>(g, vec) && g.nsplit == 1 && g.c_nper >= g.N && g.epi >= EPI_D0 && g.epi < EPI_SLAB &&
         70 * g.lda < (1ll << 31) && 40 * g.ldb < (1ll << 31);
}

template <int MODE, int NP>
inline int launch_x6s(const GemmArgs& g, hipStream_t st) {
  const int64_t tiles = ((g.M + SBM - 1) / SBM) * ((g.N + SBN - 1) / SBN);
  if (tiles <= 0) return GCT_OK;
  static bool attr_set = false;
  if (!attr_set) {
    hipError_t e = hipFuncSetAttribute((const void*)gemm_x6s_kernel<MODE, NP>, hipFuncAttributeMaxDynamicSharedMemorySize, XS_LDS_BYTES);
    if (e != hipSuccess) {
      gct_set_error("gemm_x6s: cannot reserve %d bytes of LDS: %s", XS_LDS_BYTES, hipGetErrorString(e));
      return GCT_ERR_HIP;
    }
    attr_set = true;
  }
  hipLaunchKernelGGL((gemm_x6s_kernel<MODE, NP>), dim3((unsigned)tiles), dim3(512), XS_LDS_BYTES, st, g);
  ++(NP == 3 ? g_x6_kernel_launches : g_x3_kernel_launches);
  GCT_LAUNCH_CHECK("gemm_x6s");
  return GCT_OK;
}

__global__ __launch_bounds__(256) void split_planes_kernel(const float* __restrict__ src, uint16_t* __restrict__ planes,
                                                           int64_t n4, int64_t pstride) {
  const int64_t i = (int64_t)blockIdx.x * 256 + threadIdx.x;
  if (i >= n4) return;
  const float4 v = reinterpret_cast<const float4*>(src)[i];
  x6_u32x2 h, m, l;
  x6_split4(v, h, m, l);
  *reinterpret_cast<x6_u32x2*>(planes + 4 * i) = h;
  *reinterpret_cast<x6_u32x2*>(planes + pstride + 4 * i) = m;
  *reinterpret_cast<x6_u32x2*>(planes + 2 * pstride + 4 * i) = l;
}
```

gct_plus_amd/engine.py:

```python
from __future__ import annotations

import math
import os
from typing import List, NamedTuple, Optional

import torch

from . import ops
from .flat import HANDED_SLOTS

_SEED = {"base": None, "ctr": 0}

COMPACT_BWD = os.environ.get("GCT_COMPACT_BWD", "1") != "0"
COMPACT_MAX_FRACTION = 0.85
COMPACT_KV = os.environ.get("GCT_COMPACT_KV", "1") != "0"
COMPACT_FWD = os.environ.get("GCT_COMPACT_FWD", "1") != "0"
COMPACT_ENC_KV = os.environ.get("GCT_COMPACT_ENC_KV", "1") != "0"


GRAD_NOTIFY = None


def _grads_done(module, G: "GradSink"):
    if GRAD_NOTIFY is not None:
        if ops.SIDE_ENABLED:
            ops.join_side()
        ps = list(module.parameters())
        GRAD_NOTIFY(ps, [G.out.get(p) for p in ps])


MODEL = "model"
DECODER = "decoder"
PREFILL = "prefill"
ENCODER = "encoder"


class RowMaps(NamedTuple):
    enc_keys: bool = False
    dec_keys: bool = False
    live: bool = False
    nc_lat: int = 0
    enc_rows: int = 0
    dec_rows: int = 0
    live_rows: int = 0


def plan_rows(caller, B=0, T=0, Le=0, mask_shape=None, *, loss_rows=False, trg_mask=False, get_attn=False,
              cond2dec=False, cond2lat=False, nconds=0, n_enc=0, n_dec=0, capturing=False, compact_fwd=False,
              compact_kv=False, compact_enc_kv=False) -> RowMaps:
    c2d = cond2dec and nconds > 0
    nc_lat = nconds if (not c2d and cond2lat and nconds > 0) else 0
    Td, Lk = T + (nconds if c2d else 0), Le + nc_lat
    none = RowMaps(nc_lat=nc_lat, enc_rows=B * Le, dec_rows=B * Lk, live_rows=B * Td)
    if caller == ENCODER or capturing:
        return none
    if caller == MODEL:
        if get_attn or mask_shape is None or tuple(mask_shape) != (B, 1, Le):
            return none
        mask_ok = True
    elif caller in (DECODER, PREFILL):
        mask_ok = mask_shape is not None and math.prod(mask_shape) == B * Le
    else:
        raise ValueError(f"plan_rows: unknown caller {caller!r}")
    return none._replace(
        enc_keys=bool(caller == MODEL and compact_enc_kv and n_enc > 0),
        dec_keys=bool(mask_ok and compact_kv and n_dec > 0),
        live=bool(compact_fwd and loss_rows and trg_mask and not get_attn and not c2d and n_dec > 0
                  and Td <= ops.ATTN_DIRECT_MAX_KEYS and Lk <= ops.ATTN_DIRECT_MAX_KEYS))


class RowPlan:

    def __init__(self, ek=None, dk=None, lr=None, rows=(0, 0, 0)):
        self._maps, self._rows = (ek, dk, lr), rows
        self._pending = ops.PendingReadBack(ek, dk, lr)
        self._usable = None
        self.enc_keys = self.dec_keys = self.live = None

    @staticmethod
    def usable_keys(h, rows):
        return h["nonprefix"] == 0 and h["empty"] == 0 and 0 < h["padded"] <= COMPACT_MAX_FRACTION * rows

    @staticmethod
    def usable_live(h, rows):
        return h["violations"] == 0 and h["nonprefix"] == 0 and 0 < h["padded"] <= COMPACT_MAX_FRACTION * rows

    @classmethod
    def launch(cls, caller, dec=None, src_mask=None, trg_mask=None, loss_rows=None, B=0, T=0, Le=0, n_enc=0):
        shape = None if (src_mask is None or not src_mask.is_cuda) else tuple(src_mask.shape)
        want = plan_rows(caller, B, T, Le, shape, loss_rows=loss_rows is not None, trg_mask=trg_mask is not None,
                         get_attn=getattr(dec, "get_attn", False), cond2dec=getattr(dec, "use_cond2dec", False),
                         cond2lat=getattr(dec, "use_cond2lat", False), nconds=getattr(dec, "nconds", 0), n_enc=n_enc,
                         n_dec=0 if dec is None else len(dec.layers), capturing=torch.cuda.is_current_stream_capturing(),
                         compact_fwd=COMPACT_FWD, compact_kv=COMPACT_KV, compact_enc_kv=COMPACT_ENC_KV)
        if not (want.enc_keys or want.dec_keys or want.live):
            return cls()
        ek = dk = lr = None
        if want.enc_keys or want.dec_keys:
            sm = ops.to_mask_u8(src_mask).view(B, Le)
            if want.enc_keys:
                ek = ops.KeyRows(sm, B, Le)
            if want.dec_keys and want.nc_lat > 0:
                ones = torch.ones(B, want.nc_lat, dtype=torch.uint8, device=sm.device)
                dk = ops.KeyRows(torch.cat([ones, sm], dim=1).contiguous(), B, Le + want.nc_lat)
            elif want.dec_keys:
                dk = ek if ek is not None else ops.KeyRows(sm, B, Le)
        if want.live:
            lr = ops.LiveRows.from_rows(loss_rows.to(torch.uint8).contiguous().reshape(B, T), B, T,
                                        ops.to_mask_u8(trg_mask))
        return cls(ek, dk, lr, (want.enc_rows, want.dec_rows, want.live_rows))

    def finish(self) -> "RowPlan":
        if self._usable is None:
            self._pending.finish()
            (ek, dk, lr), (re, rd, rt) = self._maps, self._rows
            self._usable = (ek if ek is not None and self.usable_keys(ek.host(), re) else None,
                            dk if dk is not None and self.usable_keys(dk.host(), rd) else None,
                            lr if lr is not None and self.usable_live(lr.host(), rt) else None)
            if self._usable[2] is not None:
                self._usable[2].fwd = True
        self.enc_keys, self.dec_keys, self.live = self._usable
        if self.live is not None and torch.cuda.is_current_stream_capturing():
            self.live = None
        return self


def next_seed() -> int:
    if _SEED["base"] != torch.initial_seed():
        _SEED["base"] = torch.initial_seed()
        _SEED["ctr"] = 0
    _SEED["ctr"] += 1
    return (_SEED["base"] * 0x9E3779B97F4A7C15 + _SEED["ctr"] * 0xD1B54A32D192ED03) & ((1 << 64) - 1)


class Run:

    def __init__(self, p: float, training: bool):
        self.p = float(p) if training else 0.0
        self.seed = next_seed() if self.p > 0 else 0
        self._site = 0
        self.kt = None

    def site(self) -> int:
        self._site += 1
        return self._site


class GradSink:

    def __init__(self):
        self.out = {}

    def __call__(self, p: torch.nn.Parameter) -> torch.Tensor:
        t = self.out.get(p)
        if t is None:
            v = getattr(p, "_gct_gview", None)
            if v is not None and id(p) not in HANDED_SLOTS and \
                    (p.grad is None or p.grad.data_ptr() != v.data_ptr()):
                t = v.view(v.shape)
                HANDED_SLOTS.add(id(p))
            else:
                t = torch.empty_like(p)
            self.out[p] = t
        return t

    def collect(self, params):
        ops.join_side()
        return tuple(self.out.get(p) for p in params)


def _empty(rows, cols, like):
    return torch.empty(rows, cols, dtype=torch.float32, device=like.device)


class MhaSaved(NamedTuple):
    xq: torch.Tensor
    xkv: torch.Tensor
    qb: torch.Tensor
    kvb: Optional[torch.Tensor]
    o: torch.Tensor
    lse: torch.Tensor
    mask_u8: object
    B: int
    Lq: int
    Lk: int
    site_p: int
    site_o: int
    fused: bool
    keys: object
    self_split: bool

    @property
    def qkv(self) -> torch.Tensor:
        assert self.kvb is None, "no fused q | k | v buffer: K | V were projected on their own"
        return self.qb


class FfnSaved(NamedTuple):
    x: torch.Tensor
    gelu_d: torch.Tensor
    hdn: torch.Tensor
    site_h: int
    site_o: int
    fused: bool


class EncLayerSaved(NamedTuple):
    x_in: torch.Tensor
    m1: torch.Tensor
    r1: torch.Tensor
    attn: MhaSaved
    a: torch.Tensor
    m2: torch.Tensor
    r2: torch.Tensor
    ffn: FfnSaved


class DecLayerSaved(NamedTuple):
    x: torch.Tensor
    m1: torch.Tensor
    r1: torch.Tensor
    attn_1: MhaSaved
    xa: torch.Tensor
    m2: torch.Tensor
    r2: torch.Tensor
    attn_2: MhaSaved
    xb: torch.Tensor
    m3: torch.Tensor
    r3: torch.Tensor
    ffn: FfnSaved


class EncoderSaved(NamedTuple):
    src: torch.Tensor
    econds: Optional[torch.Tensor]
    site_pe: int
    layers: List[EncLayerSaved]
    x_last: torch.Tensor
    mean: torch.Tensor
    rstd: torch.Tensor
    B: int
    L: int


class DecoderSaved(NamedTuple):
    trg: torch.Tensor
    z2: torch.Tensor
    dconds: Optional[torch.Tensor]
    site_pe: int
    layers: List[DecLayerSaved]
    x_last: torch.Tensor
    mean: torch.Tensor
    rstd: torch.Tensor
    B: int
    T: int
    Le: int
    Lk: int
    c2d: bool
    c2l: bool
    trg_mask_u8: Optional[torch.Tensor]
    keys: object
    live: object


def mha_fwd(run: Run, m, xq, xkv, B, Lq, Lk, mask_u8, resid, want_probs=False, keys=None, live=None):
    d, H = m.d_model, m.h
    dk = d // H
    self_attn = xkv is xq
    Mq = xq.shape[0]
    self_split = self_attn and keys is not None and live is None and not want_probs
    if self_split:
        xkv = keys.gather(xq)
    if self_attn and not self_split:
        qkv = _empty(Mq, 3 * d, xq)
        ops.linear_fwd(xq, [m.q_linear.weight, m.k_linear.weight, m.v_linear.weight],
                       [m.q_linear.bias, m.k_linear.bias, m.v_linear.bias],
                       [qkv, qkv[:, d:], qkv[:, 2 * d:]], 3 * d)
        q, k, v, ldq, ldkv = qkv, qkv[:, d:], qkv[:, 2 * d:], 3 * d, 3 * d
        qb, kvb = qkv, None
        if live is not None:
            keys = live
    else:
        qb = _empty(Mq, d, xq)
        ops.linear_fwd(xq, [m.q_linear.weight], [m.q_linear.bias], [qb], d)
        kvb = _empty(B * Lk, 2 * d, xkv) if keys is None else keys.empty(2 * d)
        ops.linear_fwd(xkv, [m.k_linear.weight, m.v_linear.weight],
                       [m.k_linear.bias, m.v_linear.bias], [kvb, kvb[:, d:]], 2 * d)
        q, k, v, ldq, ldkv = qb, kvb, kvb[:, d:], d, 2 * d
    site_p = run.site()
    o, lse, probs = ops.attn_fwd(q, k, v, ldq, ldkv, ldkv, mask_u8, B, H, Lq, Lk, dk, run.p,
                                 run.seed, site_p, want_probs=want_probs, keys=keys, live=live)
    y = _empty(Mq, d, xq)
    site_o = run.site()
    if resid is not None:
        ops.linear_fwd(o, [m.out.weight], [m.out.bias], [y], d, epi=ops.EPI_DROP_RESID,
                       resid=resid, p=run.p, seed=run.seed, site=site_o, live=live)
    else:
        ops.linear_fwd(o, [m.out.weight], [m.out.bias], [y], d)
    saved = MhaSaved(xq, xkv, qb, kvb, o, lse, mask_u8, B, Lq, Lk, site_p, site_o, resid is not None,
                     None if (self_attn and live is not None) else keys, self_split)
    return y, saved, probs


def mha_bwd(run: Run, m, sv: MhaSaved, dy, G: GradSink, dxq_out, depi_q, dxkv_out=None,
            depi_kv=ops.DEPI_STORE, live=None, gdrop=None):
    B, Lq, Lk, keys = sv.B, sv.Lq, sv.Lk, sv.keys
    d, H = m.d_model, m.h
    dk = d // H
    Mq, Mk = B * Lq, sv.xkv.shape[0]
    kt = run.kt
    new = lambda cols: _empty(Mq, cols, dy)
    if live is not None:
        Mq, kt = live.Mc, None
        new = live.empty_zero_gaps
        o_in, xq_in = (sv.o, sv.xq) if live.fwd else (live.gather(sv.o), live.gather(sv.xq))
    else:
        o_in, xq_in = sv.o, sv.xq
    if gdrop is not None:
        g = gdrop
    else:
        g = ops.dropout_bwd(dy, run.p, run.seed, sv.site_o, live=live) if (sv.fused and run.p > 0) else dy
    ops.linear_wgrad([g], d, o_in, [G(m.out.weight)], [G(m.out.bias)], kt=kt)
    do = _empty(Mq, d, dy) if live is None else live.empty(d)
    ops.linear_dgrad([g], d, Mq, [m.out.weight], do)
    if sv.kvb is None:
        dqkv = new(3 * d)
        fwdc = live is not None and live.fwd
        ops.attn_bwd(sv.qb, sv.qb[:, d:], sv.qb[:, 2 * d:], 3 * d, 3 * d, 3 * d, sv.mask_u8, sv.o, do, sv.lse, dqkv,
                     dqkv[:, d:], dqkv[:, 2 * d:], 3 * d, 3 * d, 3 * d, B, H, Lq, Lk, dk, run.p,
                     run.seed, sv.site_p, live=live, kv_compact=live is not None and not fwdc,
                     keys=live if fwdc else None)
        segs = [dqkv, dqkv[:, d:], dqkv[:, 2 * d:]]
        ops.linear_wgrad(segs, 3 * d, xq_in,
                         [G(m.q_linear.weight), G(m.k_linear.weight), G(m.v_linear.weight)],
                         [G(m.q_linear.bias), G(m.k_linear.bias), G(m.v_linear.bias)], kt=kt)
        ops.linear_dgrad(segs, 3 * d, Mq,
                         [m.q_linear.weight, m.k_linear.weight, m.v_linear.weight], dxq_out,
                         depi=depi_q)
    else:
        dq = new(d)
        if keys is None:
            dkv = _empty(Mk, 2 * d, dy)
        else:
            dkv = keys.empty_zero_gaps(2 * d)
        ops.attn_bwd(sv.qb, sv.kvb, sv.kvb[:, d:], d, 2 * d, 2 * d, sv.mask_u8, sv.o, do, sv.lse, dq, dkv, dkv[:, d:],
                     d, 2 * d, 2 * d, B, H, Lq, Lk, dk, run.p, run.seed, sv.site_p, live=live, keys=keys)
        ops.linear_wgrad([dq], d, xq_in, [G(m.q_linear.weight)], [G(m.q_linear.bias)], kt=kt)
        ops.linear_wgrad([dkv, dkv[:, d:]], 2 * d, sv.xkv,
                         [G(m.k_linear.weight), G(m.v_linear.weight)],
                         [G(m.k_linear.bias), G(m.v_linear.bias)])
        ops.linear_dgrad([dq], d, Mq, [m.q_linear.weight], dxq_out, depi=depi_q)
        if sv.self_split:
            dxk = keys.empty(d)
            ops.linear_dgrad([dkv, dkv[:, d:]], 2 * d, Mk, [m.k_linear.weight, m.v_linear.weight], dxk)
            keys.scatter_add(dxk, dxq_out)
        elif dxkv_out is not None:
            ops.linear_dgrad([dkv, dkv[:, d:]], 2 * d, Mk, [m.k_linear.weight, m.v_linear.weight],
                             dxkv_out, depi=depi_kv)


def ffn_fwd(run: Run, ff, x, resid, live=None):
    M, d = x.shape
    dff = ff.linear_1.weight.shape[0]
    gelu_d = _empty(M, dff, x)
    hdn = _empty(M, dff, x)
    site_h = run.site()
    ops.linear_fwd(x, [ff.linear_1.weight], [ff.linear_1.bias], [hdn], dff, epi=ops.EPI_GELU_DROP_SAVE,
                   pre=gelu_d, p=run.p, seed=run.seed, site=site_h, live=live)
    y = _empty(M, d, x)
    site_o = run.site()
    if resid is not None:
        ops.linear_fwd(hdn, [ff.linear_2.weight], [ff.linear_2.bias], [y], d,
                       epi=ops.EPI_DROP_RESID, resid=resid, p=run.p, seed=run.seed, site=site_o, live=live)
    else:
        ops.linear_fwd(hdn, [ff.linear_2.weight], [ff.linear_2.bias], [y], d)
    return y, FfnSaved(x, gelu_d, hdn, site_h, site_o, resid is not None)


def ffn_bwd(run: Run, ff, sv: FfnSaved, dy, G: GradSink, dx_out, depi, live=None, gdrop=None):
    x, gelu_d, hdn = sv.x, sv.gelu_d, sv.hdn
    M, d = x.shape
    dff = gelu_d.shape[1]
    kt = run.kt
    if live is not None:
        M, kt = live.Mc, None
        if not live.fwd:
            x, hdn = live.gather(x), live.gather(hdn)
    if gdrop is not None:
        g = gdrop
    else:
        g = ops.dropout_bwd(dy, run.p, run.seed, sv.site_o, live=live) if (sv.fused and run.p > 0) else dy
    ops.linear_wgrad([g], d, hdn, [G(ff.linear_2.weight)], [G(ff.linear_2.bias)], kt=kt)
    dpre = _empty(M, dff, dy) if live is None else live.empty(dff)
    ops.linear_dgrad([g], d, M, [ff.linear_2.weight], dpre, depi=ops.DEPI_MUL_SAVED, pre=gelu_d,
                     p=run.p, seed=run.seed, site=sv.site_h, live=live, pre_full=live is not None and not live.fwd)
    ops.linear_wgrad([dpre], dff, x, [G(ff.linear_1.weight)], [G(ff.linear_1.bias)], kt=kt)
    ops.linear_dgrad([dpre], dff, M, [ff.linear_1.weight], dx_out, depi=depi)


def enc_layer_fwd(run: Run, layer, x_in, B, L, mask_u8, want_probs=False, keys=None):
    n1, m1, r1 = ops.norm_fwd(x_in, layer.norm_1.alpha, layer.norm_1.bias, layer.norm_1.eps)
    a, sv_a, probs = mha_fwd(run, layer.attn, n1, n1, B, L, L, mask_u8, n1, want_probs, keys=keys)
    n2, m2, r2 = ops.norm_fwd(a, layer.norm_2.alpha, layer.norm_2.bias, layer.norm_2.eps)
    out, sv_f = ffn_fwd(run, layer.ff, n2, n2)
    return out, EncLayerSaved(x_in, m1, r1, sv_a, a, m2, r2, sv_f), probs


def _mha_drop(run: Run, sv: MhaSaved, buf):
    return (buf, run.p, run.seed, sv.site_o) if (buf is not None and sv.fused and run.p > 0) else None


def _ffn_drop(run: Run, sv: Optional[FfnSaved], buf):
    return (buf, run.p, run.seed, sv.site_o) if (buf is not None and sv is not None and sv.fused and run.p > 0) else None


def enc_layer_bwd(run: Run, layer, sv: EncLayerSaved, g, G: GradSink, gd=None, gdbuf=None, below=None):
    with ops.deferred_reductions():
        ffn_bwd(run, layer.ff, sv.ffn, g, G, g, ops.DEPI_ACCUM, gdrop=gd)
        dr = _mha_drop(run, sv.attn, gdbuf)
        ops.norm_bwd(g, sv.a, layer.norm_2.alpha, sv.m2, sv.r2, G(layer.norm_2.alpha), G(layer.norm_2.bias),
                     out=g, eps=layer.norm_2.eps, drop=dr)
        mha_bwd(run, layer.attn, sv.attn, g, G, g, ops.DEPI_ACCUM, gdrop=None if dr is None else gdbuf)
        dr = _ffn_drop(run, below, gdbuf)
        ops.norm_bwd(g, sv.x_in, layer.norm_1.alpha, sv.m1, sv.r1, G(layer.norm_1.alpha), G(layer.norm_1.bias),
                     out=g, eps=layer.norm_1.eps, drop=dr)
    _grads_done(layer, G)
    return g, (None if dr is None else gdbuf)


def dec_layer_fwd(run: Run, layer, x, e, B, T, Lk, src_mask_u8, trg_mask_u8, want_probs=False, keys=None, live=None):
    x2, m1, r1 = ops.norm_fwd(x, layer.norm_1.alpha, layer.norm_1.bias, layer.norm_1.eps)
    xa, sa1, p1 = mha_fwd(run, layer.attn_1, x2, x2, B, T, T, trg_mask_u8, x, want_probs, live=live)
    x2, m2, r2 = ops.norm_fwd(xa, layer.norm_2.alpha, layer.norm_2.bias, layer.norm_2.eps)
    xb, sa2, p2 = mha_fwd(run, layer.attn_2, x2, e, B, T, Lk, src_mask_u8, xa, want_probs, keys=keys, live=live)
    x2, m3, r3 = ops.norm_fwd(xb, layer.norm_3.alpha, layer.norm_3.bias, layer.norm_3.eps)
    xc, sf = ffn_fwd(run, layer.ff, x2, xb, live=live)
    return xc, DecLayerSaved(x, m1, r1, sa1, xa, m2, r2, sa2, xb, m3, r3, sf), p1, p2


def dec_layer_bwd(run: Run, layer, sv: DecLayerSaved, g, de, first_de, G: GradSink, live=None, gd=None, gdbuf=None,
                  below=None):
    t = torch.empty_like(g) if live is None else live.empty(g.shape[1])
    with ops.deferred_reductions():
        ffn_bwd(run, layer.ff, sv.ffn, g, G, t, ops.DEPI_STORE, live=live, gdrop=gd)
        dr = _mha_drop(run, sv.attn_2, gdbuf)
        ops.norm_bwd(t, sv.xb, layer.norm_3.alpha, sv.m3, sv.r3, G(layer.norm_3.alpha), G(layer.norm_3.bias),
                     dres=g, out=g, eps=layer.norm_3.eps, live=live, drop=dr)
        mha_bwd(run, layer.attn_2, sv.attn_2, g, G, t, ops.DEPI_STORE, de,
                ops.DEPI_STORE if first_de else ops.DEPI_ACCUM, live=live, gdrop=None if dr is None else gdbuf)
        dr = _mha_drop(run, sv.attn_1, gdbuf)
        ops.norm_bwd(t, sv.xa, layer.norm_2.alpha, sv.m2, sv.r2, G(layer.norm_2.alpha), G(layer.norm_2.bias),
                     dres=g, out=g, eps=layer.norm_2.eps, live=live, drop=dr)
        mha_bwd(run, layer.attn_1, sv.attn_1, g, G, t, ops.DEPI_STORE, live=live, gdrop=None if dr is None else gdbuf)
        dr = _ffn_drop(run, below, gdbuf)
        ops.norm_bwd(t, sv.x, layer.norm_1.alpha, sv.m1, sv.r1, G(layer.norm_1.alpha), G(layer.norm_1.bias),
                     dres=g, out=g, eps=layer.norm_1.eps, live=live, drop=dr)
    _grads_done(layer, G)
    return g, (None if dr is None else gdbuf)


def _pe2d(pe_mod, L):
    pe = pe_mod.pe
    if L > pe.shape[1]:
        raise ValueError(f"sequence length {L} exceeds the positional table ({pe.shape[1]})")
    return pe[0]


def encoder_trunk_fwd(enc, run: Run, src, mask_u8, econds, want_probs, plan: RowPlan):
    keys = plan.enc_keys
    B, S = src.shape
    d, nc = enc.d_model, enc.nconds
    cond = None
    if nc > 0:
        if econds is None:
            raise ValueError("econds required when nconds > 0")
        cond = ops.small_linear_fwd(econds.contiguous(), enc.embed_cond2enc.weight,
                                    enc.embed_cond2enc.bias)
    L = S + nc
    mask_u8 = ops.pack_mask(mask_u8, B, L, L)
    site_pe = run.site()
    x = ops.embed_pe_fwd(src, enc.embed_sentence.embed.weight, cond, _pe2d(enc.pe, L), nc,
                         math.sqrt(d), run.p, run.seed, site_pe)
    layers, probs = [], []
    for layer in enc.layers:
        x, sv, pr = enc_layer_fwd(run, layer, x, B, L, mask_u8, want_probs, keys=keys)
        layers.append(sv)
        probs.append(pr)
    y, mean, rstd = ops.norm_fwd(x, enc.norm.alpha, enc.norm.bias, enc.norm.eps)
    return y.view(B, L, d), EncoderSaved(src, econds, site_pe, layers, x, mean, rstd, B, L), probs


def encoder_trunk_bwd(enc, run: Run, sv: EncoderSaved, dy, G: GradSink):
    layers, B, L = sv.layers, sv.B, sv.L
    d, nc = enc.d_model, enc.nconds
    g = dy.reshape(B * L, d).clone()
    gdbuf = torch.empty_like(g) if (run.p > 0 and len(layers) > 0) else None
    dr = _ffn_drop(run, layers[-1].ffn if layers else None, gdbuf)
    ops.norm_bwd(g, sv.x_last, enc.norm.alpha, sv.mean, sv.rstd, G(enc.norm.alpha), G(enc.norm.bias), out=g,
                 eps=enc.norm.eps, drop=dr)
    gd = None if dr is None else gdbuf
    for i in range(len(layers) - 1, -1, -1):
        g, gd = enc_layer_bwd(run, enc.layers[i], layers[i], g, G, gd=gd, gdbuf=gdbuf,
                              below=layers[i - 1].ffn if i > 0 else None)
    dcond = torch.empty(B, nc * d, dtype=torch.float32, device=g.device) if nc > 0 else None
    ops.embed_pe_bwd(g, sv.src, G(enc.embed_sentence.embed.weight), dcond, nc, math.sqrt(d), run.p,
                     run.seed, sv.site_pe)
    if nc > 0:
        ops.small_linear_bwd(dcond, sv.econds.contiguous(), G(enc.embed_cond2enc.weight),
                             G(enc.embed_cond2enc.bias))


def decoder_trunk_fwd(dec, run: Run, trg, z, src_mask_u8, trg_mask_u8, dconds, want_probs, plan: RowPlan):
    B, T0 = trg.shape
    d, nc = dec.d_model, dec.nconds
    Le, lat = z.shape[1], z.shape[2]
    z2 = z.reshape(B * Le, lat)
    c2d = dec.use_cond2dec and nc > 0
    c2l = (not c2d) and dec.use_cond2lat and nc > 0
    cond_x = None
    if c2d:
        cond_x = ops.small_linear_fwd(dconds.contiguous(), dec.embed_cond2dec.weight,
                                      dec.embed_cond2dec.bias)
    T = T0 + (nc if c2d else 0)
    site_pe = run.site()
    x = ops.embed_pe_fwd(trg, dec.embed.embed.weight, cond_x, _pe2d(dec.pe, T), nc if c2d else 0,
                         math.sqrt(d), run.p, run.seed, site_pe)
    ez = _empty(B * Le, d, z2)
    ops.linear_fwd(z2, [dec.fc_z.weight], [dec.fc_z.bias], [ez], d)
    Lk = Le
    e = ez
    if c2l:
        Lk = Le + nc
        cl = ops.small_linear_fwd(dconds.contiguous(), dec.embed_cond2lat.weight,
                                  dec.embed_cond2lat.bias)
        e = _empty(B * Lk, d, z2)
        ops.copy_rows(cl, nc, 0, e, Lk, 0, B * nc, nc, d)
        ops.copy_rows(ez, Le, 0, e, Lk, nc, B * Le, Le, d)
        if src_mask_u8 is not None:
            ones = torch.ones(B, nc, dtype=torch.uint8, device=src_mask_u8.device)
            src_mask_u8 = torch.cat([ones, src_mask_u8.view(B, Le)], dim=1).contiguous()
    layers, p1s, p2s = [], [], []
    live, keys = plan.live, plan.dec_keys
    if live is not None:
        x = live.gather(x)
    if keys is not None:
        e = keys.gather(e)
    src_m = ops.pack_mask(src_mask_u8, B, T, Lk)
    trg_m = ops.pack_mask(trg_mask_u8, B, T, T)
    for layer in dec.layers:
        x, sv, p1, p2 = dec_layer_fwd(run, layer, x, e, B, T, Lk, src_m, trg_m, want_probs, keys=keys, live=live)
        layers.append(sv)
        p1s.append(p1)
        p2s.append(p2)
    y, mean, rstd = ops.norm_fwd(x, dec.norm.alpha, dec.norm.bias, dec.norm.eps)
    saved = DecoderSaved(trg, z2, dconds, site_pe, layers, x, mean, rstd, B, T, Le, Lk, c2d, c2l,
                         trg_mask_u8.u8 if isinstance(trg_mask_u8, ops.MaskBits) else trg_mask_u8, keys, live)
    if live is not None:
        return y, saved, p1s, p2s
    return y.view(B, T, d), saved, p1s, p2s


def decoder_trunk_bwd(dec, run: Run, sv: DecoderSaved, dy, G: GradSink, need_dz=True):
    layers, keys, live_fwd = sv.layers, sv.keys, sv.live
    B, T, Le, Lk = sv.B, sv.T, sv.Le, sv.Lk
    new_de = (lambda: _empty(B * Lk, d, dy)) if keys is None else (lambda: keys.empty(d))
    d, nc = dec.d_model, dec.nconds
    live, lr = live_fwd, None
    if live_fwd is None:
        lr = ops.LiveRows(dy.reshape(B * T, d), B, T, sv.trg_mask_u8) if (COMPACT_BWD or (B * T) % 32 == 0) else None
        if COMPACT_BWD and len(dec.layers) > 0 and not torch.cuda.is_current_stream_capturing():
            live = lr if RowPlan.usable_live(lr.host(), B * T) else None
    if live_fwd is not None:
        g = dy.reshape(live.Mc, d).clone()
    elif live is not None:
        g = live.gather(dy.reshape(B * T, d))
    else:
        g = dy.reshape(B * T, d).clone()
        run.kt = lr.kt if (lr is not None and (B * T) % 32 == 0) else None
    gdbuf = None
    if run.p > 0 and len(layers) > 0:
        gdbuf = torch.empty_like(g) if live is None else live.empty(d)
    dr = _ffn_drop(run, layers[-1].ffn if layers else None, gdbuf)
    ops.norm_bwd(g, sv.x_last, dec.norm.alpha, sv.mean, sv.rstd, G(dec.norm.alpha), G(dec.norm.bias), out=g,
                 eps=dec.norm.eps, live=live, drop=dr)
    gd = None if dr is None else gdbuf
    de = new_de()
    for i in range(len(layers) - 1, -1, -1):
        g, gd = dec_layer_bwd(run, dec.layers[i], layers[i], g, de, i == len(layers) - 1, G, live=live, gd=gd,
                              gdbuf=gdbuf, below=layers[i - 1].ffn if i > 0 else None)
    run.kt = None
    if live is not None:
        g = live.scatter(g)
    if len(dec.layers) == 0:
        de.zero_()
    if keys is not None:
        de = keys.scatter(de)
    dcx = torch.empty(B, nc * d, dtype=torch.float32, device=g.device) if sv.c2d else None
    ops.embed_pe_bwd(g, sv.trg, G(dec.embed.embed.weight), dcx, nc if sv.c2d else 0, math.sqrt(d), run.p,
                     run.seed, sv.site_pe)
    if sv.c2d:
        ops.small_linear_bwd(dcx, sv.dconds.contiguous(), G(dec.embed_cond2dec.weight),
                             G(dec.embed_cond2dec.bias))
    dez = de
    if sv.c2l:
        dcl = torch.empty(B, nc * d, dtype=torch.float32, device=g.device)
        ops.copy_rows(de, Lk, 0, dcl, nc, 0, B * nc, nc, d)
        ops.small_linear_bwd(dcl, sv.dconds.contiguous(), G(dec.embed_cond2lat.weight),
                             G(dec.embed_cond2lat.bias))
        dez = _empty(B * Le, d, g)
        ops.copy_rows(de, Lk, nc, dez, Le, 0, B * Le, Le, d)
    ops.linear_wgrad([dez], d, sv.z2, [G(dec.fc_z.weight)], [G(dec.fc_z.bias)])
    dz = None
    if need_dz:
        dz = _empty(B * Le, sv.z2.shape[1], g)
        ops.linear_dgrad([dez], d, B * Le, [dec.fc_z.weight], dz)
        dz = dz.view(B, Le, -1)
    return dz


def _f32c(t):
    return t if (t.dtype == torch.float32 and t.is_contiguous()) else t.float().contiguous()


class EncoderFn(torch.autograd.Function):
    @staticmethod
    def forward(ctx, enc, run, src, mask_u8, econds, want_probs, plan, *params):
        y, saved, probs = encoder_trunk_fwd(enc, run, src, mask_u8, econds, want_probs, plan)
        ctx.enc, ctx.run, ctx.saved, ctx.params = enc, run, saved, params
        if want_probs:
            for p in probs:
                ctx.mark_non_differentiable(p)
            return (y, *probs)
        return y

    @staticmethod
    def backward(ctx, dy, *unused):
        G = GradSink()
        encoder_trunk_bwd(ctx.enc, ctx.run, ctx.saved, _f32c(dy), G)
        ctx.saved = None
        return (None,) * 7 + G.collect(ctx.params)


class DecoderFn(torch.autograd.Function):
    @staticmethod
    def forward(ctx, dec, run, trg, z, src_mask_u8, trg_mask_u8, dconds, want_probs, plan, *params):
        y, saved, p1, p2 = decoder_trunk_fwd(dec, run, trg, _f32c(z), src_mask_u8, trg_mask_u8, dconds, want_probs,
                                             plan)
        ctx.dec, ctx.run, ctx.saved, ctx.params = dec, run, saved, params
        ctx.need_dz = z.requires_grad
        if want_probs:
            for p in p1 + p2:
                ctx.mark_non_differentiable(p)
            return (y, *p1, *p2)
        return y

    @staticmethod
    def backward(ctx, dy, *unused):
        G = GradSink()
        dz = decoder_trunk_bwd(ctx.dec, ctx.run, ctx.saved, _f32c(dy), G, ctx.need_dz)
        ctx.saved = None
        return (None, None, None, dz, None, None, None, None, None) + G.collect(ctx.params)


class ScatterRowsFn(torch.autograd.Function):

    @staticmethod
    def forward(ctx, xc, live, B, T):
        ctx.live, ctx.shape = live, xc.shape
        return live.scatter(_f32c(xc)).view(B, T, xc.shape[-1])

    @staticmethod
    def backward(ctx, dy):
        live = ctx.live
        g = _f32c(dy).reshape(live.M, dy.shape[-1])
        live.check_grad(g)
        return live.gather(g).view(ctx.shape), None, None, None


class SamplerFn(torch.autograd.Function):

    @staticmethod
    def forward(ctx, x, w_mu, b_mu, w_lv, b_lv, eps, variational):
        B, L, d = x.shape
        lat = w_mu.shape[0]
        x2 = _f32c(x).view(B * L, d)
        mu = _empty(B * L, lat, x2)
        lv = _empty(B * L, lat, x2)
        ops.linear_fwd(x2, [w_mu, w_lv], [b_mu, b_lv], [mu, lv], lat)
        if variational:
            z, eps_used = ops.reparam_fwd(mu, lv, None if eps is None else _f32c(eps).view(B * L, lat),
                                          next_seed(), 0)
        else:
            z, eps_used = mu, None
        ctx.save_for_backward(x2, w_mu, w_lv, lv, eps_used if eps_used is not None else lv)
        ctx.variational = variational
        ctx.shape = (B, L, d, lat)
        ctx.params = (w_mu, b_mu, w_lv, b_lv)
        shp = (B, L, lat)
        if variational:
            return z.view(shp), mu.view(shp), lv.view(shp)
        return mu.view(shp), mu.view(shp).clone(), lv.view(shp)

    @staticmethod
    def backward(ctx, dz, dmu, dlv):
        x2, w_mu, w_lv, lv, eps = ctx.saved_tensors
        B, L, d, lat = ctx.shape
        M = B * L
        zeros = None
        def flat(t):
            return None if t is None else _f32c(t).view(M, lat)
        dz, dmu, dlv = flat(dz), flat(dmu), flat(dlv)
        gmu = _empty(M, lat, x2)
        glv = _empty(M, lat, x2)
        if ctx.variational:
            if dz is None:
                dz = torch.zeros(M, lat, dtype=torch.float32, device=x2.device)
            ops.reparam_bwd(dz, lv, eps, dmu, dlv, gmu, glv)
        else:
            z0 = torch.zeros(M, lat, dtype=torch.float32, device=x2.device)
            a = dz if dz is not None else z0
            b = dmu if dmu is not None else z0
            ops.add(a, b, out=gmu)
            glv = dlv if dlv is not None else z0
        G = GradSink()
        w_mu_p, b_mu_p, w_lv_p, b_lv_p = ctx.params
        ops.linear_wgrad([gmu, glv], lat, x2, [G(w_mu_p), G(w_lv_p)], [G(b_mu_p), G(b_lv_p)])
        dx = _empty(M, d, x2)
        ops.linear_dgrad([gmu, glv], lat, M, [w_mu, w_lv], dx)
        return (dx.view(B, L, d),) + G.collect(ctx.params) + (None, None)


class LinearFn(torch.autograd.Function):

    @staticmethod
    def forward(ctx, x, w, b):
        shp = x.shape
        x2 = _f32c(x).reshape(-1, shp[-1])
        y = _empty(x2.shape[0], w.shape[0], x2)
        ops.linear_fwd(x2, [w], [b], [y], w.shape[0])
        ctx.save_for_backward(x2, w)
        ctx.params = (w, b)
        ctx.shp = shp
        return y.view(*shp[:-1], w.shape[0])

    @staticmethod
    def backward(ctx, dy):
        x2, w = ctx.saved_tensors
        N = w.shape[0]
        dy2 = _f32c(dy).reshape(-1, N)
        G = GradSink()
        wp, bp = ctx.params
        ops.linear_wgrad([dy2], N, x2, [G(wp)], [G(bp) if bp is not None else None])
        dx = None
        if ctx.needs_input_grad[0]:
            dx = _empty(x2.shape[0], x2.shape[1], x2)
            ops.linear_dgrad([dy2], N, x2.shape[0], [w], dx)
            dx = dx.view(ctx.shp)
        ops.join_side()
        return dx, G.out.get(wp), G.out.get(bp) if bp is not None else None


class CrossEntropySumFn(torch.autograd.Function):

    @staticmethod
    def forward(ctx, logits, target, pad_id):
        l2 = _f32c(logits).reshape(-1, logits.shape[-1])
        t = target.reshape(-1).contiguous()
        ctx.save_for_backward(l2, t)
        ctx.pad_id, ctx.shp = int(pad_id), logits.shape
        return ops.ce_fwd(l2, t, int(pad_id))

    @staticmethod
    def backward(ctx, g):
        l2, t = ctx.saved_tensors
        return ops.ce_bwd(l2, t, _f32c(g), ctx.pad_id).view(ctx.shp), None, None


class KldFn(torch.autograd.Function):

    @staticmethod
    def forward(ctx, mu, log_var):
        m, l = _f32c(mu), _f32c(log_var)
        ctx.save_for_backward(m, l)
        return ops.kld_fwd(m, l)

    @staticmethod
    def backward(ctx, g):
        m, l = ctx.saved_tensors
        dmu, dlv = ops.kld_bwd(m, l, _f32c(g))
        return dmu, dlv


class NormFn(torch.autograd.Function):

    @staticmethod
    def forward(ctx, x, alpha, bias, eps):
        x2 = _f32c(x).reshape(-1, x.shape[-1])
        y, mean, rstd = ops.norm_fwd(x2, alpha, bias, eps)
        ctx.save_for_backward(x2, alpha, mean, rstd)
        ctx.params, ctx.eps, ctx.shp = (alpha, bias), eps, x.shape
        return y.view(x.shape)

    @staticmethod
    def backward(ctx, dy):
        x2, alpha, mean, rstd = ctx.saved_tensors
        G = GradSink()
        a, b = ctx.params
        dx = ops.norm_bwd(_f32c(dy).reshape(x2.shape), x2, alpha, mean, rstd, G(a), G(b), eps=ctx.eps)
        return dx.view(ctx.shp), G.out[a], G.out[b], None


class EmbedFn(torch.autograd.Function):

    @staticmethod
    def forward(ctx, tok, table):
        B, S = tok.shape
        d = table.shape[1]
        zeros = torch.zeros(S, d, dtype=torch.float32, device=table.device)
        out = ops.embed_pe_fwd(tok.contiguous(), table, None, zeros, 0, 1.0, 0.0, 0, 0)
        ctx.tok, ctx.param = tok.contiguous(), table
        return out.view(B, S, d)

    @staticmethod
    def backward(ctx, dy):
        G = GradSink()
        d = ctx.param.shape[1]
        ops.embed_pe_bwd(_f32c(dy).reshape(-1, d), ctx.tok, G(ctx.param), None, 0, 1.0, 0.0, 0, 0)
        return None, G.out[ctx.param]


class PosEncFn(torch.autograd.Function):

    @staticmethod
    def forward(ctx, x, pe, scale, run):
        B, L, d = x.shape
        x2 = _f32c(x).view(B, L * d)
        site = run.site()
        dummy_tok = torch.zeros(B, 0, dtype=torch.int64, device=x.device)
        out = ops.embed_pe_fwd(dummy_tok, None, x2, _pe2d_raw(pe, L), L, scale, run.p, run.seed,
                               site, d=d)
        ctx.cfg = (B, L, d, scale, run, site)
        return out.view(B, L, d)

    @staticmethod
    def backward(ctx, dy):
        B, L, d, scale, run, site = ctx.cfg
        dx = torch.empty(B, L * d, dtype=torch.float32, device=dy.device)
        dummy_tok = torch.zeros(B, 0, dtype=torch.int64, device=dy.device)
        ops.embed_pe_bwd(_f32c(dy).reshape(B * L, d), dummy_tok, None, dx, L, scale, run.p,
                         run.seed, site, d=d)
        return dx.view(B, L, d), None, None, None


def _pe2d_raw(pe, L):
    if L > pe.shape[1]:
        raise ValueError(f"sequence length {L} exceeds the positional table ({pe.shape[1]})")
    return pe[0]


def _flat3(x):
    B, L, d = x.shape
    return _f32c(x).view(B * L, d), B, L, d


class MhaFn(torch.autograd.Function):
    @staticmethod
    def forward(ctx, m, run, q, kv, mask_u8, want_probs, *params):
        xq, B, Lq, d = _flat3(q)
        if kv is None:
            xkv, Lk = xq, Lq
        else:
            xkv, _, Lk, _ = _flat3(kv)
        y, saved, probs = mha_fwd(run, m, xq, xkv, B, Lq, Lk, mask_u8, None, want_probs)
        ctx.m, ctx.run, ctx.saved, ctx.params = m, run, saved, params
        ctx.shapes = (B, Lq, Lk, d, kv is not None)
        if want_probs:
            ctx.mark_non_differentiable(probs)
            return y.view(B, Lq, d), probs
        return (y.view(B, Lq, d),)

    @staticmethod
    def backward(ctx, dy, *unused):
        B, Lq, Lk, d, cross = ctx.shapes
        G = GradSink()
        dxq = torch.empty(B * Lq, d, dtype=torch.float32, device=dy.device)
        dxkv = torch.empty(B * Lk, d, dtype=torch.float32, device=dy.device) if cross else None
        mha_bwd(ctx.run, ctx.m, ctx.saved, _f32c(dy).reshape(B * Lq, d), G, dxq, ops.DEPI_STORE,
                dxkv, ops.DEPI_STORE)
        ctx.saved = None
        return (None, None, dxq.view(B, Lq, d), dxkv.view(B, Lk, d) if cross else None, None,
                None) + G.collect(ctx.params)


class FfnFn(torch.autograd.Function):
    @staticmethod
    def forward(ctx, ff, run, x, *params):
        x2 = _f32c(x).reshape(-1, x.shape[-1])
        y, saved = ffn_fwd(run, ff, x2, None)
        ctx.ff, ctx.run, ctx.saved, ctx.params, ctx.shp = ff, run, saved, params, x.shape
        return y.view(x.shape)

    @staticmethod
    def backward(ctx, dy):
        G = GradSink()
        dy2 = _f32c(dy).reshape(-1, dy.shape[-1])
        dx = torch.empty_like(dy2)
        ffn_bwd(ctx.run, ctx.ff, ctx.saved, dy2, G, dx, ops.DEPI_STORE)
        ctx.saved = None
        return (None, None, dx.view(ctx.shp)) + G.collect(ctx.params)


class EncLayerFn(torch.autograd.Function):
    @staticmethod
# ... 43 lines not shown
```

gct_plus_amd/ops.py:

```python
from __future__ import annotations

import contextlib
import math
import os
import threading
import weakref
from typing import List, Optional, Sequence

import torch

from . import _lib
from ._lib import check

EPI_BIAS, EPI_GELU_DROP, EPI_DROP_RESID, EPI_GELU_DROP_SAVE = 0, 1, 2, 3
DEPI_STORE, DEPI_ACCUM, DEPI_GELU_BWD, DEPI_MUL_SAVED = 0, 1, 2, 3


def _L():
    return _lib.load()


_raw_stream, _cur_dev = torch._C._cuda_getCurrentRawStream, torch._C._cuda_getDevice


def _st():
    return _raw_stream(_cur_dev())


def _p(t: Optional[torch.Tensor]):
    return None if t is None else t.data_ptr()


def _chk(t: torch.Tensor, name: str, dtype=torch.float32):
    if not t.is_cuda:
        raise _lib.GctError(f"{name}: expected a CUDA (ROCm) tensor; gct_plus_amd has no CPU path")
    if t.dtype != dtype:
        raise _lib.GctError(f"{name}: expected {dtype}, got {t.dtype}")
    return t


SIDE_ENABLED = os.environ.get("GCT_SIDE_STREAM", "0") != "0"
_SIDE = {}
_PENDING = {}


def _side_stream(device):
    idx = device.index if device.index is not None else torch.cuda.current_device()
    st = _SIDE.get(idx)
    if st is None:
        st = torch.cuda.Stream(device=idx)
        _SIDE[idx] = st
    return st


def _wait_pending(t):
    if _PENDING and t is not None:
        ev = _PENDING.pop(t.untyped_storage().data_ptr(), None)
        if ev is not None:
            torch.cuda.current_stream().wait_event(ev)


def join_side(device=None):
    if _SIDE:
        cur = torch.cuda.current_stream()
        for st in _SIDE.values():
            cur.wait_stream(st)
        _PENDING.clear()


_WS = {}


def workspace(nbytes: int, device) -> torch.Tensor:
    key = (device.index if device.index is not None else torch.cuda.current_device(), _st())
    buf = _WS.get(key)
    if buf is None or buf.numel() * 4 < nbytes:
        n = max(int(nbytes * 1.25) // 4 + 64, 1 << 20)
        buf = torch.empty(n, dtype=torch.float32, device=device)
        _WS[key] = buf
    return buf


DEFER_REDUCTIONS = os.environ.get("GCT_DEFER_REDUCTIONS", "1") != "0"
class _DeferState(threading.local):
    def __init__(self):
        self.d = {"on": False, "off": 0, "demand": 0, "want": 0}


_DEFER_TL = _DeferState()
_ARENA = {}


def kept_workspace(nbytes: int, device) -> torch.Tensor:
    if not _DEFER_TL.d["on"]:
        return workspace(nbytes, device)
    key = (device.index if device.index is not None else torch.cuda.current_device(), _st())
    n = (int(nbytes) + 255) // 256 * 64
    _DEFER_TL.d["demand"] += n
    buf = _ARENA.get(key)
    if buf is None or _DEFER_TL.d["off"] + n > buf.numel():
        check(_L().gct_reduce_defer_flush(_st()), "gct_reduce_defer_flush")
        _DEFER_TL.d["off"] = 0
        if buf is None or n > buf.numel():
            buf = _ARENA[key] = torch.empty(max(n, _DEFER_TL.d["want"], 1 << 22), dtype=torch.float32, device=device)
    out = buf[_DEFER_TL.d["off"]:_DEFER_TL.d["off"] + n]
    _DEFER_TL.d["off"] += n
    return out


class deferred_reductions:

    def __enter__(self):
        self.mine = (DEFER_REDUCTIONS and not _DEFER_TL.d["on"] and not SIDE_ENABLED
                     and not torch.cuda.is_current_stream_capturing())
        if self.mine:
            key = (torch.cuda.current_device(), _st())
            buf = _ARENA.get(key)
            if buf is not None and buf.numel() < _DEFER_TL.d["want"]:
                del _ARENA[key]
            _DEFER_TL.d.update(on=True, off=0, demand=0)
            check(_L().gct_reduce_defer_begin(), "gct_reduce_defer_begin")
        return self

    def __exit__(self, et, ev, tb):
        if self.mine:
            _DEFER_TL.d["on"] = False
            _DEFER_TL.d["want"] = max(_DEFER_TL.d["want"], _DEFER_TL.d["demand"])
            rc = _L().gct_reduce_defer_end(_st())
            if et is None:
                check(rc, "gct_reduce_defer_end")
        return False


_WS_NEED = {}


def _ws_need(fn: str, a: int, b: int, c: int) -> int:
    key = (fn, a, b, c)
    v = _WS_NEED.get(key)
    if v is None:
        v = _WS_NEED[key] = int(getattr(_L(), fn)(a, b, c))
    return v


def norm_fwd(x2d, alpha, bias, eps=1e-6, out=None):
    _chk(x2d, "norm_fwd.x")
    rows, d = x2d.shape
    y = torch.empty_like(x2d) if out is None else out
    mean = torch.empty(rows, dtype=torch.float32, device=x2d.device)
    rstd = torch.empty(rows, dtype=torch.float32, device=x2d.device)
    check(_L().gct_norm_fwd(_p(x2d), _p(alpha), _p(bias), _p(y), _p(mean), _p(rstd), rows, d, eps,
                            _st()), "gct_norm_fwd")
    return y, mean, rstd


def norm_bwd(dy, x2d, alpha, mean, rstd, dalpha, dbias, dres=None, out=None, eps=1e-6, live=None, drop=None):
    src_rows, d = x2d.shape
    rows = src_rows if live is None else live.Mc
    if live is not None and live.fwd:
        src_rows = 0
    dx = (torch.empty_like(x2d) if live is None else live.empty(d)) if out is None else out
    _wait_pending(out)
    if drop is not None:
        _wait_pending(drop[0])
    ws = kept_workspace(_L().gct_rowred_ws_bytes(rows, 2 * d), x2d.device)
    check(_L().gct_norm_bwd(_p(dy), _p(x2d), _p(alpha), _p(mean), _p(rstd), _p(dres), _p(dx),
                            _p(dalpha), _p(dbias), _p(ws), rows, d, eps,
                            None if live is None else _p(live.quad_list), src_rows,
                            None if drop is None else _p(drop[0]), 0.0 if drop is None else drop[1],
                            0 if drop is None else drop[2], 0 if drop is None else drop[3], _st()), "gct_norm_bwd")
    return dx


def embed_pe_fwd(tok, table, cond, pe2d, n_c, scale, p, seed, site, d=None):
    _chk(tok, "embed.tok", torch.int64)
    B, S = tok.shape
    if table is not None:
        vocab, d = table.shape
    else:
        vocab = 1
    out = torch.empty(B * (S + n_c), d, dtype=torch.float32, device=pe2d.device)
    check(_L().gct_embed_pe_fwd(_p(tok), _p(table), _p(cond), _p(pe2d), _p(out), B, S, n_c, d, vocab,
                                scale, p, seed, site, _st()), "gct_embed_pe_fwd")
    return out


def embed_pe_bwd(dout, tok, dtable, dcond, n_c, scale, p, seed, site, d=None):
    B, S = tok.shape
    if dtable is not None:
        vocab, d = dtable.shape
    else:
        vocab = 1
    ws = workspace(_L().gct_embed_ws_bytes(B, S, d, vocab), dout.device)
    check(_L().gct_embed_pe_bwd(_p(dout), _p(tok), _p(dtable), _p(dcond), _p(ws), B, S, n_c, d, vocab,
                                scale, p, seed, site, _st()), "gct_embed_pe_bwd")


PROFILE = None
PROFILE_KINDS = None


class _Timed:
    def __init__(self, kind, flops, nbytes=0):
        self.kind, self.flops, self.nbytes = kind, flops, nbytes

    def __enter__(self):
        self.on = PROFILE is not None and (PROFILE_KINDS is None or self.kind in PROFILE_KINDS)
        if self.on:
            self.c0 = gemm_launch_counts()[1]
            self.k0 = _L().gct_gemm_x6_kernel_launches()
            self.e0 = torch.cuda.Event(enable_timing=True)
            self.e1 = torch.cuda.Event(enable_timing=True)
            self.e0.record()
        return self

    def __exit__(self, *a):
        if self.on:
            self.e1.record()
            kind = self.kind + "[x6]" if gemm_launch_counts()[1] > self.c0 else self.kind
            PROFILE.setdefault(kind, []).append((self.flops, self.e0, self.e1))
            PROFILE["_x6_kernel_launches:" + kind] = PROFILE.get("_x6_kernel_launches:" + kind, 0) + \
                (_L().gct_gemm_x6_kernel_launches() - self.k0)
            PROFILE["_bytes:" + kind] = PROFILE.get("_bytes:" + kind, 0) + self.nbytes


def _seg3(ts: Sequence[Optional[torch.Tensor]]):
    ts = list(ts) + [None] * (3 - len(ts))
    return [_p(t) for t in ts]


GEMM_F32, GEMM_BF16X6 = 0, 1
GEMM_BF16X3 = 2
_PLANES = []


def gemm_set_mode(mode: int):
    check(_L().gct_gemm_set_mode(int(mode)), "gct_gemm_set_mode")


def gemm_get_mode() -> int:
    return _L().gct_gemm_get_mode()


def gemm_x3_launches() -> int:
    return int(_L().gct_gemm_x3_launches())


def gemm_launch_counts():
    import ctypes
    out = (ctypes.c_int64 * 2)()
    check(_L().gct_gemm_launch_counts(ctypes.cast(out, ctypes.c_void_p)), "gct_gemm_launch_counts")
    return int(out[0]), int(out[1])


def split_planes(flat: torch.Tensor, planes: Optional[torch.Tensor] = None) -> torch.Tensor:
    _chk(flat, "flat")
    n = flat.numel()
    if planes is None:
        planes = torch.empty(3, n, dtype=torch.int16, device=flat.device)
    check(_L().gct_split_planes(_p(flat), n, _p(planes), planes.stride(0), _st()), "gct_split_planes")
    return planes


def _drop_planes(base: int, end: int):
    _PLANES[:] = [e for e in _PLANES if e[1] <= base or e[0] >= end]


def register_planes(flat: torch.Tensor, planes: torch.Tensor):
    base, end = flat.data_ptr(), flat.data_ptr() + flat.numel() * 4
    known = any(e[0] == base and e[1] == end and e[4]() is flat for e in _PLANES)
    _drop_planes(base, end)
    _PLANES.append((base, end, planes, flat.numel(), weakref.ref(flat)))
    if not known:
        weakref.finalize(flat, _drop_planes, base, end)


def unregister_planes(flat: torch.Tensor):
    _drop_planes(flat.data_ptr(), flat.data_ptr() + flat.numel() * 4)


def _plane_ptr(ws_):
    if not _PLANES:
        return None, 0
    a = ws_[0].data_ptr()
    for base, end, planes, numel, ref in _PLANES:
        if base <= a < end:
            if ref() is None:
                return None, 0
            if all(base <= w.data_ptr() < end for w in ws_[1:]):
                return planes.data_ptr() + (a - base) // 2, planes.stride(0)
            return None, 0
    return None, 0


def linear_fwd(x2d, ws_: Sequence[torch.Tensor], bs: Sequence[Optional[torch.Tensor]],
               outs: Sequence[torch.Tensor], ldy: int, epi=EPI_BIAS, resid=None, pre=None,
               p=0.0, seed=0, site=0, splitk_ws: Optional[torch.Tensor] = None, ws: Optional[torch.Tensor] = None,
               live=None):
    M, K = x2d.shape
    nper = ws_[0].shape[0]
    w = _seg3(ws_)
    b = _seg3(bs)
    y = _seg3(outs)
    need = _ws_need("gct_linear_fwd_ws_bytes", M, K, nper * len(ws_))
    for t in (splitk_ws, ws):
        if t is not None and t.numel() * 4 < need:
            raise _lib.GctError(f"linear_fwd: workspace of {t.numel() * 4} B < {need} B "
                                f"(gct_linear_fwd_ws_bytes({M}, {K}, {nper * len(ws_)}))")
    if splitk_ws is not None:
        wp, pstride, wsb, quad_map, timed = None, 0, splitk_ws, None, contextlib.nullcontext()
    else:
        wp, pstride = _plane_ptr(ws_)
        wsb = ws if ws is not None else (workspace(need, x2d.device) if need > 256 else None)
        quad_map = None if live is None else _p(live.quad_list)
        N = nper * len(ws_)
        nbytes = 4 * M * K + (6 if wp else 4) * N * K + 4 * N + 4 * M * N * (2 if epi in (EPI_GELU_DROP, EPI_DROP_RESID, EPI_GELU_DROP_SAVE) else 1)
        timed = _Timed("gemm_fwd", 2.0 * M * K * N, nbytes)
    with timed:
        check(_L().gct_linear_fwd(_p(x2d), x2d.stride(0), M, K, w[0], w[1], w[2], ws_[0].stride(0),
                                  wp, pstride, b[0], b[1], b[2], len(ws_), nper, y[0], y[1], y[2],
                                  ldy, epi, _p(resid), _p(pre), p, seed, site, _p(wsb),
                                  0 if wsb is None else wsb.numel() * 4, quad_map, _st()),
              "gct_linear_fwd")


def linear_dgrad(dys: Sequence[torch.Tensor], lddy: int, M: int, ws_: Sequence[torch.Tensor], dx,
                 depi=DEPI_STORE, pre=None, p=0.0, seed=0, site=0, live=None, pre_full=False):
    nper, K = ws_[0].shape
    d = _seg3(dys)
    w = _seg3(ws_)
    _wait_pending(dx)
    with _Timed("gemm_dgrad", 2.0 * M * K * nper * len(ws_)):
        wp, pstride = _plane_ptr(ws_)
        need = _ws_need("gct_linear_dgrad_ws_bytes", M, nper * len(ws_), K)
        wsb = workspace(need, dx.device) if need > 256 else None
        check(_L().gct_linear_dgrad(d[0], d[1], d[2], lddy, M, len(ws_), nper, w[0], w[1], w[2],
                                    ws_[0].stride(0), wp, pstride, K, _p(dx), dx.stride(0), depi,
                                    _p(pre), p, seed, site, _p(wsb), 0 if wsb is None else wsb.numel() * 4,
                                    None if live is None else _p(live.quad_list),
                                    pre.shape[0] if (live is not None and pre is not None and pre_full) else 0,
                                    _st()), "gct_linear_dgrad")


def nonzero_row_tiles(x2d: torch.Tensor):
    _chk(x2d, "x2d")
    rows, cols = x2d.shape
    nt = (rows + 31) // 32
    lst = torch.empty(max(nt, 1), dtype=torch.int32, device=x2d.device)
    cnt = torch.empty(1, dtype=torch.int32, device=x2d.device)
    flags = torch.empty(max(nt, 1), dtype=torch.uint8, device=x2d.device)
    check(_L().gct_nonzero_row_tiles(_p(x2d), x2d.stride(0), rows, cols, _p(lst), _p(cnt), _p(flags), _st()),
          "gct_nonzero_row_tiles")
    return lst, cnt


_SKIPPED = {}
_SKIPPED_MSG = ("{} decoder rows that an earlier forward skipped (loss_rows: rows that do not reach the loss) received a "
                "non-zero gradient in its backward pass: that gradient was ignored, and the optimizer steps launched since "
                "then were skipped on the device (FusedAdam's guard), so no wrong update has been applied; this error is "
                "raised at the first host read-back after the fact.  Call the model without loss_rows "
                "(forward_propagation(..., skip_ignored=False)) for losses other than the reference's ignore_index "
                "cross-entropy.")


def assert_no_skipped_row_gradients():
    n = int(skipped_row_gradients().item())
    if n:
        skipped_row_gradients().zero_()
        raise _lib.GctError(_SKIPPED_MSG.format(n))


def skipped_row_gradients():
    dev = torch.cuda.current_device()
    t = _SKIPPED.get(dev)
    if t is None:
        t = _SKIPPED[dev] = torch.zeros(1, dtype=torch.int32, device=torch.device("cuda", dev))
    return t


class LiveRows:
    SLACK = 256
    fwd = False

    def __init__(self, g2d, B, T, mask_u8, lists=True):
        _chk(g2d, "g2d")
        dev = g2d.device
        M = B * T
        assert g2d.shape[0] == M
        nt, nq = (M + 31) // 32, (M + 3) // 4
        i32 = lambda n: torch.empty(max(n, 1), dtype=torch.int32, device=dev)
        self.B, self.T, self.M, self.dev = B, T, M, dev
        self.live = torch.empty(max(M, 1), dtype=torch.uint8, device=dev)
        self.n_b, self.info = i32(B), i32(8)
        self.cstart = i32(B) if lists else None
        self.quad_list = i32(nq + 32) if lists else None
        qrank = i32(nq) if lists else None
        self.tile_list, self.tile_count = i32(nt), i32(1)
        flags = torch.empty(max(nt, 1), dtype=torch.uint8, device=dev)
        if mask_u8 is None:
            sb = sq = 0
        else:
            _chk(mask_u8, "live_rows.mask", torch.uint8)
            sb, sq = _mask_strides(mask_u8, B, T, T)
        check(_L().gct_live_rows(_p(g2d), g2d.stride(0), B, T, g2d.shape[1], _p(mask_u8), sb, sq, _p(self.live),
                                 _p(self.n_b), _p(self.info), _p(self.cstart), _p(self.quad_list), _p(qrank),
                                 _p(self.tile_list), _p(self.tile_count), _p(flags), _st()), "gct_live_rows")
        self.kt = (self.tile_list, self.tile_count)
        self._host = None
        self.Mc = None

    @classmethod
    def from_rows(cls, rows_u8, B, T, mask_u8):
        _chk(rows_u8, "live_rows.rows", torch.uint8)
        return cls(rows_u8.reshape(B * T, 1).to(torch.float32), B, T, mask_u8)

    def _fill_host(self, v):
        self._host = dict(n_live=v[0], violations=v[1], nonprefix=v[2], tiles=v[3], padded=v[4], quads=v[5], empty=v[6])
        self.Mc = v[4]

    def host(self):
        if self._host is None:
            PendingReadBack(self).finish()
        return self._host

    def scatter_add(self, src2d, dst2d):
        cols = src2d.shape[1]
        check(_L().gct_scatter_add_quads(_p(src2d), src2d.stride(0), _p(self.quad_list), self.Mc, cols, _p(dst2d),
                                         dst2d.stride(0), self.M, _st()), "gct_scatter_add_quads")
        return dst2d

    def check_grad(self, g2d):
        check(_L().gct_dead_rows_nonzero(_p(g2d), g2d.stride(0), self.M, g2d.shape[1], _p(self.live),
                                         _p(skipped_row_gradients()), _st()), "gct_dead_rows_nonzero")

    def empty(self, cols):
        return torch.empty(self.Mc + self.SLACK, cols, dtype=torch.float32, device=self.dev)[:self.Mc]

    def empty_zero_gaps(self, cols):
        t = self.empty(cols)
        check(_L().gct_zero_gap_rows(_p(t), t.stride(0), cols, _p(self.cstart), _p(self.n_b), self.B, self.Mc, _st()),
              "gct_zero_gap_rows")
        return t

    def gather(self, src2d, out=None):
        cols = src2d.shape[1]
        dst = self.empty(cols) if out is None else out
        check(_L().gct_gather_quads(_p(src2d), src2d.stride(0), src2d.shape[0], _p(self.quad_list), self.Mc, cols,
                                    _p(dst), dst.stride(0), _st()), "gct_gather_quads")
        return dst

    def scatter(self, src2d, out=None):
        cols = src2d.shape[1]
        dst = torch.zeros(self.M, cols, dtype=torch.float32, device=self.dev) if out is None else out
        check(_L().gct_scatter_quads(_p(src2d), src2d.stride(0), _p(self.quad_list), self.Mc, cols, _p(dst),
                                     dst.stride(0), self.M, _st()), "gct_scatter_quads")
        return dst


HOST_BLOCKED_S = [0.0]


class PendingReadBack:

    def __init__(self, *objs):
        seen, self.objs = set(), []
        for o in objs:
            if o is not None and o._host is None and id(o) not in seen:
                seen.add(id(o))
                self.objs.append(o)
        self.host = self.ev = None
        if self.objs:
            dev = torch.cat([o.info for o in self.objs] + [skipped_row_gradients()])
            self.host = torch.empty(dev.numel(), dtype=dev.dtype, pin_memory=True)
            self.host.copy_(dev, non_blocking=True)
            self.ev = torch.cuda.Event()
            self.ev.record()

    def finish(self):
        if self.host is None:
            return
        import time
        t0 = time.perf_counter()
        self.ev.synchronize()
        HOST_BLOCKED_S[0] += time.perf_counter() - t0
        v = self.host.tolist()
        self.host = None
        for i, o in enumerate(self.objs):
            if o._host is None:
                o._fill_host(v[8 * i:8 * i + 8])
        if v[-1] != 0:
            skipped_row_gradients().zero_()
            raise _lib.GctError(_SKIPPED_MSG.format(v[-1]))


class KeyRows(LiveRows):

    def __init__(self, mask_u8, B, Lk):
        _chk(mask_u8, "key_rows.mask", torch.uint8)
        dev = mask_u8.device
        M = B * Lk
        nq = (M + 3) // 4
        i32 = lambda n: torch.empty(max(n, 1), dtype=torch.int32, device=dev)
        self.B, self.T, self.M, self.dev = B, Lk, M, dev
        self.live = torch.empty(max(M, 1), dtype=torch.uint8, device=dev)
        self.n_b, self.info = i32(B), i32(8)
        self.cstart, self.quad_list = i32(B), i32(nq + 32)
        qrank = i32(nq)
        check(_L().gct_key_rows(_p(mask_u8), Lk, B, Lk, _p(self.live), _p(self.n_b), _p(self.info), _p(self.cstart),
                                _p(self.quad_list), _p(qrank), _st()), "gct_key_rows")
        self._host = None
        self.Mc = None



def linear_wgrad(dys: Sequence[torch.Tensor], lddy: int, x2d, dws: Sequence[torch.Tensor],
                 dbs: Sequence[Optional[torch.Tensor]], kt=None):
    M, K = x2d.shape
    nper = dws[0].shape[0]
    nseg = len(dws)
    d = _seg3(dys)
    dw = _seg3(dws)
    db = _seg3(dbs)

    def launch():
        ws = kept_workspace(_ws_need("gct_wgrad_ws_bytes", M, nseg * nper, K), x2d.device)
        with _Timed("gemm_wgrad+bias+reduce", 2.0 * M * K * nper * nseg):
            check(_L().gct_linear_wgrad(d[0], d[1], d[2], lddy, M, nseg, nper, _p(x2d), x2d.stride(0),
                                        K, dw[0], dw[1], dw[2], K, db[0], db[1], db[2], _p(ws),
                                        _p(kt[0]) if kt else None, _p(kt[1]) if kt else None, _st()),
                  "gct_linear_wgrad")

    if not SIDE_ENABLED or torch.cuda.is_current_stream_capturing():
        launch()
        return
    main = torch.cuda.current_stream()
    side = _side_stream(x2d.device)
    ready = torch.cuda.Event()
    ready.record(main)
    side.wait_event(ready)
    with torch.cuda.stream(side):
        launch()
        done = torch.cuda.Event()
        done.record(side)
    for t in list(dys) + [x2d]:
        t.record_stream(side)
        _PENDING[t.untyped_storage().data_ptr()] = done


def dropout_bwd(dout2d, p, seed, site, out=None, live=None):
    rows, cols = dout2d.shape
    if live is not None:
        rows = live.Mc
    dy = torch.empty_like(dout2d) if out is None else out
    _wait_pending(out)
    check(_L().gct_dropout_bwd(_p(dout2d), _p(dy), rows, cols, p, seed, site,
                               None if live is None else _p(live.quad_list), _st()), "gct_dropout_bwd")
    return dy


ATTN_DIRECT_MAX_KEYS = 96


class MaskBits:

    def __init__(self, mask_u8, B, Lq, Lk):
        _chk(mask_u8, "attn.mask", torch.uint8)
        if Lk > 256 or Lq > 256:
            raise _lib.GctError(f"attention: sequence length {max(Lq, Lk)} > 256 unsupported")
        sb, sq = _mask_strides(mask_u8, B, Lq, Lk)
        rows = 1 if sq == 0 else Lq
        self.u8, self.B, self.Lq, self.Lk = mask_u8, B, Lq, Lk
        self.bits = torch.empty(B, rows, 8, dtype=torch.int32, device=mask_u8.device)
        self.sb, self.sq = rows * 8, (0 if sq == 0 else 8)
        ntr = 1 if sq == 0 else (Lq + 15) // 16
        self.tiles = torch.empty(B, ntr, dtype=torch.int32, device=mask_u8.device)
        self.t_sb, self.t_su = ntr, (0 if sq == 0 else 1)
        check(_L().gct_attn_mask_pack(_p(mask_u8), sb, sq, B, Lq, Lk, _p(self.bits), _p(self.tiles), _st()),
              "gct_attn_mask_pack")


def pack_mask(mask, B, Lq, Lk) -> Optional["MaskBits"]:
    if mask is None or isinstance(mask, MaskBits):
        if isinstance(mask, MaskBits) and (mask.B, mask.Lk) != (B, Lk):
            raise _lib.GctError(f"packed mask was built for B={mask.B}, Lk={mask.Lk}, not B={B}, Lk={Lk}")
        return mask
    return MaskBits(to_mask_u8(mask), B, Lq, Lk)


def _mb(mask, B, Lq, Lk):
    mb = pack_mask(mask, B, Lq, Lk)
    if mb is None:
        return None, 0, 0, None
    if mb.t_su and mb.Lq != Lq:
        raise _lib.GctError(f"packed mask was built for Lq={mb.Lq}, not Lq={Lq}")
    return mb.bits.data_ptr(), mb.sb, mb.sq, mb


def _tb(mb):
    return (None, 0, 0) if mb is None else (mb.tiles.data_ptr(), mb.t_sb, mb.t_su)


def attn_fwd(q, k, v, ld_q, ld_k, ld_v, mask, B, H, Lq, Lk, dk, p, seed, site, out=None,
             want_probs=False, keys=None, live=None):
    dev = q.device
    if out is not None:
        o = out
    elif live is not None:
        o = live.empty_zero_gaps(H * dk)
    else:
        o = torch.empty(B * Lq, H * dk, dtype=torch.float32, device=dev)
    lse = torch.empty(B * H * Lq, dtype=torch.float32, device=dev)
    probs = torch.empty(B, H, Lq, Lk, dtype=torch.float32, device=dev) if want_probs else None
    mp, sb, sq, mask_owner = _mb(mask, B, Lq, Lk)
    check(_L().gct_attn_fwd(_p(q), ld_q, _p(k), ld_k, _p(v), ld_v, mp, sb, sq, _p(o),
                            o.stride(0), _p(lse), _p(probs), B, H, Lq, Lk, dk,
                            1.0 / math.sqrt(dk), p, seed, site, None if keys is None else _p(keys.cstart),
                            None if keys is None else _p(keys.n_b), *_tb(mask_owner),
                            None if live is None else _p(live.cstart), None if live is None else _p(live.n_b),
                            _st()), "gct_attn_fwd")
    del mask_owner
    return o, lse, probs


_ATTN_BWD_WS = {}


def _attn_bwd_ws(dev, nbytes):
    if nbytes <= 0:
        return None
    key = (dev, _st())
    ws = _ATTN_BWD_WS.get(key)
# ... 258 lines not shown
```

include/gctplus_hip.h:

```cpp
#ifndef GCTPLUS_HIP_H
#define GCTPLUS_HIP_H

#include <stdint.h>

#ifdef __cplusplus
extern "C" {
#endif

#define GCT_OK 0
#define GCT_ERR_ARG (-1)
#define GCT_ERR_HIP (-2)

#define GCT_ABI_VERSION 20

int gct_version(void);
const char* gct_last_error(void);

int64_t gct_wgrad_ws_bytes(int64_t M, int64_t Ntot, int64_t K);
int64_t gct_rowred_ws_bytes(int64_t rows, int64_t cols);

int gct_norm_fwd(const float* x, const float* alpha, const float* bias, float* y,
                 float* mean, float* rstd, int64_t rows, int d, float eps, void* stream);
int gct_norm_bwd(const float* dy, const float* x, const float* alpha, const float* mean,
                 const float* rstd, const float* dres, float* dx, float* dalpha, float* dbias,
                 float* ws, int64_t rows, int d, float eps, const int32_t* quad_map, int64_t src_rows,
                 float* drop_out, float p, uint64_t seed, uint32_t site, void* stream);

int gct_embed_pe_fwd(const int64_t* tok, const float* table, const float* cond, const float* pe,
                     float* out, int B, int S, int n_c, int d, int vocab, float scale, float p,
                     uint64_t seed, uint32_t site, void* stream);
int64_t gct_embed_ws_bytes(int B, int S, int d, int vocab);
int gct_embed_pe_bwd(const float* dout, const int64_t* tok, float* dtable, float* dcond,
                     float* ws, int B, int S, int n_c, int d, int vocab, float scale, float p,
                     uint64_t seed, uint32_t site, void* stream);

#define GCT_EPI_BIAS 0
#define GCT_EPI_GELU_DROP 1
#define GCT_EPI_DROP_RESID 2
#define GCT_EPI_GELU_DROP_SAVE 3
int gct_linear_fwd(const float* x, int64_t ldx, int64_t M, int K,
                   const float* w0, const float* w1, const float* w2, int64_t ldw,
                   const uint16_t* wp0, int64_t plane_stride,
                   const float* b0, const float* b1, const float* b2,
                   int nseg, int nper, float* y0, float* y1, float* y2, int64_t ldy,
                   int epi, const float* resid, float* pre, float p, uint64_t seed, uint32_t site,
                   float* ws, int64_t ws_bytes, const int32_t* quad_map, void* stream);
int64_t gct_linear_fwd_ws_bytes(int64_t M, int K, int Ntot);

#define GCT_DEPI_STORE 0
#define GCT_DEPI_ACCUM 1
#define GCT_DEPI_GELU_BWD 2
#define GCT_DEPI_MUL_SAVED 3
int gct_linear_dgrad(const float* dy0, const float* dy1, const float* dy2, int64_t lddy,
                     int64_t M, int nseg, int nper,
                     const float* w0, const float* w1, const float* w2, int64_t ldw,
                     const uint16_t* wp0, int64_t plane_stride, int K,
                     float* dx, int64_t lddx, int depi, const float* pre, float p, uint64_t seed,
                     uint32_t site, float* ws, int64_t ws_bytes, const int32_t* quad_map, int64_t pre_rows,
                     void* stream);
int64_t gct_linear_dgrad_ws_bytes(int64_t M, int Ntot, int K);

int gct_linear_wgrad(const float* dy0, const float* dy1, const float* dy2, int64_t lddy,
                     int64_t M, int nseg, int nper, const float* x, int64_t ldx, int K,
                     float* dw0, float* dw1, float* dw2, int64_t lddw,
                     float* db0, float* db1, float* db2, float* ws,
                     const int32_t* tile_list, const int32_t* tile_count, void* stream);

#define GCT_GEMM_F32 0
#define GCT_GEMM_BF16X6 1
#define GCT_GEMM_BF16X3 2
int gct_gemm_set_mode(int mode);
int gct_gemm_get_mode(void);
int gct_gemm_launch_counts(int64_t* out2);
int64_t gct_gemm_x6_kernel_launches(void);
int64_t gct_gemm_x3_launches(void);

int gct_split_planes(const float* src, int64_t numel, uint16_t* planes, int64_t plane_stride,
                     void* stream);

int gct_dead_rows_nonzero(const float* g, int64_t ld, int64_t rows, int cols, const uint8_t* live,
                          int32_t* counter, void* stream);
int gct_nonzero_row_tiles(const float* x, int64_t ld, int64_t rows, int cols, int32_t* list,
                          int32_t* count, uint8_t* flags_ws, void* stream);
int gct_live_rows(const float* g, int64_t ld, int B, int T, int cols, const uint8_t* mask, int64_t mask_sb,
                  int64_t mask_sq, uint8_t* live, int32_t* n_b, int32_t* info, int32_t* cstart,
                  int32_t* quad_list, int32_t* qrank_ws, int32_t* tile_list, int32_t* tile_count,
                  uint8_t* tile_flags_ws, void* stream);
int gct_key_rows(const uint8_t* mask, int64_t mask_sb, int B, int Lk, uint8_t* live, int32_t* n_b, int32_t* info,
                 int32_t* cstart, int32_t* quad_list, int32_t* qrank_ws, void* stream);
int gct_gather_quads(const float* src, int64_t ld, int64_t M, const int32_t* quad_list, int64_t nrows, int cols,
                     float* dst, int64_t ldd, void* stream);
int gct_scatter_quads(const float* src, int64_t ld, const int32_t* quad_list, int64_t nrows, int cols, float* dst,
                      int64_t ldd, int64_t M, void* stream);
int gct_zero_gap_rows(float* buf, int64_t ld, int cols, const int32_t* cstart, const int32_t* n_b, int B, int64_t nrows,
                      void* stream);
int gct_scatter_add_quads(const float* src, int64_t ld, const int32_t* quad_list, int64_t nrows, int cols, float* dst,
                          int64_t ldd, int64_t M, void* stream);

int gct_dropout_bwd(const float* dout, float* dy, int64_t rows, int cols, float p, uint64_t seed,
                    uint32_t site, const int32_t* quad_map, void* stream);

#define GCT_ATTN_DIRECT_MAX_KEYS 96
int gct_attn_mask_pack(const uint8_t* mask, int64_t mask_sb, int64_t mask_sq, int B, int Lq, int Lk,
                       uint32_t* bits, uint32_t* tiles, void* stream);
int gct_trg_mask_tokens(const int64_t* tokens, int64_t ld_tok, int64_t pad, int B, int T, uint8_t* out, void* stream);
int gct_attn_fwd(const float* q, int64_t ldq, const float* k, int64_t ldk, const float* v,
                 int64_t ldv, const uint32_t* mbits, int64_t mb_sb, int64_t mb_sq,
                 float* o, int64_t ldo, float* lse, float* probs, int B, int H, int Lq, int Lk,
                 int dk, float scale, float p, uint64_t seed, uint32_t site, const int32_t* kstart,
                 const int32_t* klen, const uint32_t* tbits, int64_t tb_sb, int64_t tb_su,
                 const int32_t* qstart, const int32_t* qlen, void* stream);
int gct_attn_bwd(const float* q, int64_t ldq, const float* k, int64_t ldk, const float* v,
                 int64_t ldv, const uint32_t* mbits, int64_t mb_sb, int64_t mb_sq,
                 const float* o, const float* dout, int64_t ldo, const float* lse,
                 float* dq, int64_t lddq, float* dk_, int64_t lddk, float* dv, int64_t lddv,
                 int B, int H, int Lq, int Lk, int dk, float scale, float p, uint64_t seed,
                 uint32_t site, const int32_t* cstart, const int32_t* nlive, int kv_compact,
                 const int32_t* kstart, const int32_t* klen, const uint32_t* tbits, int64_t tb_sb, int64_t tb_su,
                 void* ws, int64_t ws_bytes, void* stream);
int64_t gct_attn_bwd_ws_bytes(int B, int H, int Lq, int Lk);

int gct_reparam_fwd(const float* mu, const float* log_var, const float* eps_in, float* eps_out,
                    float* z, int64_t n, uint64_t seed, uint32_t site, void* stream);
int gct_reparam_bwd(const float* dz, const float* log_var, const float* eps, const float* dmu_ext,
                    const float* dlv_ext, float* dmu, float* dlv, int64_t n, void* stream);
int gct_kld_fwd(const float* mu, const float* log_var, float* out, float* ws, int64_t n,
                void* stream);
int gct_kld_bwd(const float* mu, const float* log_var, const float* gout, float* dmu, float* dlv,
                int64_t n, void* stream);

int gct_ce_fwd(const float* logits, const int64_t* target, float* out, float* ws, int64_t rows,
               int V, int64_t pad_id, void* stream);
int gct_ce_bwd(const float* logits, const int64_t* target, const float* gout, float* dlogits,
               int64_t rows, int V, int64_t pad_id, void* stream);

int gct_adam_step(float* p, const float* g, float* m, float* v, int64_t n, float lr, float b1,
                  float b2, float eps, int64_t step, float gscale, const int32_t* skip_if_nonzero,
                  void* stream);

int gct_attn_decode(const float* q, int64_t ldq, float* k, float* v, int64_t kv_row,
                    int64_t kv_batch, const uint8_t* valid, int64_t valid_sb, float* o, int64_t ldo,
                    int n, int H, int Lc, int dk, float scale, const int32_t* pos, int cache_off,
                    const float* knew, const float* vnew, int64_t ldn, const int32_t* klen,
                    const int32_t* row_off, void* stream);
int gct_attn_decode_z(const float* q, int64_t ldq, int qoff, const float* z, int64_t z_batch, int lat, int Le,
                      const float* ckv, int64_t ckv_batch, int64_t ld_ckv, int nc, const uint8_t* valid,
                      int64_t valid_sb, const int32_t* klen, float* out, int64_t ldo, int ooff, int n, int H, int dk,
                      float scale, void* stream);
int gct_decode_embed(const int64_t* ys, int64_t ld_ys, const int32_t* pos, int pe_off, const float* table,
                     int vocab, const float* pe, float* out, int n, int d, float scale, const int32_t* row_off,
                     void* stream);
int gct_decode_advance(int32_t* pos, void* stream);
typedef struct GctSampleFilter {
  int32_t k;
  float top_p;
  float inv_temp;
  int32_t reserved;
} GctSampleFilter;
#define GCT_SAMPLE_FILTER_MAX_VOCAB 1024
int gct_select_token(const float* logits, int V, int64_t* ys, int64_t ld_ys, int pos, uint8_t* valid,
                     int64_t valid_sb, uint8_t* done, float* probs_out, int n, int mode,
                     int64_t pad_id, int64_t eos_id, uint64_t seed, const int32_t* pos_dev, int valid_off,
                     const uint64_t* seed_dev, const int32_t* row_off, const GctSampleFilter* filt,
                     const int32_t* item, const int32_t* prefix_len, int item_base, void* stream);

#define GCT_STREAM_MAX_ROWS 8192
#define GCT_STREAM_MAX_LAYERS 16
typedef struct GctStreamState {
  int64_t* ys;
  uint8_t* valid;
  uint8_t* done;
  int32_t* row_off;
  const int32_t* pos;
  float* z3;
  uint8_t* src_valid;
  int32_t* src_klen;
  float* ckv[GCT_STREAM_MAX_LAYERS];
  int32_t* item;
  int32_t* harvest;
  uint8_t* fresh;
  const float* z_pool;
  const uint8_t* valid_pool;
  const int32_t* klen_pool;
  const float* ckv_pool[GCT_STREAM_MAX_LAYERS];
  const int64_t* prefix_pool;
  const int32_t* prefix_len;
  const int32_t* limit;
  int64_t* out_ys;
  int32_t* out_len;
  int32_t* row_of;
  int32_t* start_step;
  int32_t* next_item;
  int32_t* n_harvested;
  const int32_t* enable;
  int64_t rows, items, ld_ys, valid_sb, valid_off, T, width, t0_max, z_row, Lk, ckv_row, layers, pad_id;
} GctStreamState;
int gct_stream_refill(const GctStreamState* state, void* stream);

#define GCT_BEAM_MAX_K 16
#define GCT_BEAM_MAX_VOCAB 65536
int gct_attn_decode_beam(const float* q, int64_t ldq, float* k, float* v, int64_t kv_row, int64_t kv_batch,
                         const uint8_t* valid, int64_t valid_sb, float* o, int64_t ldo, int n, int H, int T, int dk,
                         float scale, const int32_t* pos, int cache_off, const float* knew, const float* vnew,
                         int64_t ldn, const int32_t* kv_src, int64_t ld_src, void* stream);
int gct_beam_select(const float* logits, int V, int n, int k, float* scores, uint8_t* finished, int32_t* lengths,
                    int32_t* parent, int64_t* ys, int64_t ld_ys, uint8_t* valid, int64_t valid_sb, int valid_off,
                    int32_t* kv_src, int64_t ld_src, int T, uint8_t* done, const int32_t* pos_dev, int64_t pad_id,
                    int64_t eos_id, void* stream);

int gct_smiles_tokenize(const char* smi, int with_sep, int32_t* tok_start, int32_t* tok_len,
                        int max_tokens);
int gct_smiles_encode_batch(const char* const* smiles, int n, int with_sep, const char* const* vocab,
                            int vocab_size, int64_t unk_id, int64_t pad_id, int64_t sos_id,
                            int64_t eos_id, int64_t* out, int64_t width, int32_t* lengths);

int gct_copy_rows(const float* src, int64_t src_rpb, int64_t src_off, float* dst, int64_t dst_rpb,
                  int64_t dst_off, int64_t rows, int64_t rpb, int cols, int accumulate,
                  void* stream);
int gct_small_linear_fwd(const float* x, const float* w, const float* b, float* y, int rows,
                         int K, int N, void* stream);
int gct_small_linear_bwd(const float* dy, const float* x, float* dw, float* db, int rows, int K,
                         int N, void* stream);
int gct_reduce_slabs(const float* slabs, int nslab, int64_t stride, float* dst, int64_t n,
                     int accumulate, void* stream);
int gct_reduce_defer_begin(void);
int gct_reduce_defer_flush(void* stream);
int gct_reduce_defer_end(void* stream);
int gct_reduce_defer_pending(void);
int gct_add(const float* a, const float* b, float* y, int64_t n, void* stream);

#ifdef __cplusplus
}
#endif
#endif
```

Measured before the change: 10860.

## Batch all decoder cross-attention K/V projections into one multi-segment GEMM

Adds N-segment (up to 12) forward and dgrad GEMM entry points that use a per-segment offset table and a magic-number divide to pick each segment inside the x6 bf16-split kernel. The decoder now computes the K/V projections of the encoder output for every layer in a single launch, and the backward pass does one combined dgrad into the encoder gradient in place of per-layer launches. It also runs the fc_z wgrad/dgrad on compacted rows. The goal is fewer kernel launches and larger, better-filled GEMMs, at the cost of a larger workspace buffer, extra table indexing inside the kernel, and a fallback to grouped three-segment calls when alignment checks fail.

```diff
diff --git a/gct_plus_amd/csrc/gemm.hip b/gct_plus_amd/csrc/gemm.hip
--- a/gct_plus_amd/csrc/gemm.hip
+++ b/gct_plus_amd/csrc/gemm.hip
@@ -52,6 +52,17 @@
 #ifdef GCT_STAMPS
   unsigned long long* stamps;
 #endif
+};
+
+constexpr int SEG_MAX = GCT_MAX_SEGS;
+struct SegTab {
+  int32_t a[SEG_MAX], b[SEG_MAX], c[SEG_MAX], bias[SEG_MAX];
+  uint32_t magic;
+  int32_t nseg;
+};
+struct GemmArgsN {
+  GemmArgs g;
+  SegTab t;
 };
 
 enum { EPI_SLAB = 32, EPI_D0 = 16 };
@@ -1226,18 +1237,24 @@
 }
 
 template <int MODE, int NP>
-int launch_x6_tail_split(const GemmArgs& g, hipStream_t st, float* ws, int64_t ws_bytes) {
-  if (MODE == X6_WGRAD || g.nsplit != 1 || !ws || !gct_aligned16(ws)) return launch_x6<MODE, NP>(g, st);
+int launch_x6_tail_split(const GemmArgs& g, hipStream_t st, float* ws, int64_t ws_bytes, const SegTab* tab = nullptr) {
+  auto x6 = [&](const GemmArgs& a) {
+    if constexpr (MODE != X6_WGRAD) {
+      if (tab) return launch_x6n<MODE, NP>(a, *tab, st);
+    }
+    return launch_x6<MODE, NP>(a, st);
+  };
+  if (MODE == X6_WGRAD || g.nsplit != 1 || !ws || !gct_aligned16(ws) || (tab && MODE != X6_DGRAD)) return x6(g);
   int64_t m1 = 0;
   const int best = x6_tail_plan(g.M, g.N, g.K, &m1);
   const int64_t m2 = g.M - m1, nkt = g.K / XBK;
   hipStreamCaptureStatus cap = hipStreamCaptureStatusNone;
   if (best == 1 || slab_bytes(best, m2, g.N) > ws_bytes ||
       hipStreamIsCapturing(st, &cap) != hipSuccess || cap != hipStreamCaptureStatusNone)
-    return launch_x6<MODE, NP>(g, st);
+    return x6(g);
   GemmArgs head = g;
   head.M = m1;
-  int rc = launch_x6<MODE, NP>(head, st);
+  int rc = x6(head);
   if (rc) return rc;
   GemmArgs e = g;
   e.M = m2; e.row_base = g.row_base + m1;
@@ -1246,12 +1263,12 @@
   if (e.resid) e.resid += m1 * g.ldc;
   if (e.pre) e.pre += m1 * g.ldc;
   if (e.pre_in && !(g.pre_rows > 0 && g.quad_map)) e.pre_in += m1 * g.ldc;
-  if (nkt <= 32 && x6s_tiles(m2, g.N) <= X6_TAIL_SMALL_MAX) {
+  if (!tab && nkt <= 32 && x6s_tiles(m2, g.N) <= X6_TAIL_SMALL_MAX) {
     if (MODE == X6_FWD && x6s_ok(e, true)) return launch_x6s<X6_FWD, NP>(e, st);
     if (MODE == X6_DGRAD && x6s_dgrad_ok(e, true)) return launch_x6s<X6_DGRAD, NP>(e, st);
   }
   const GemmArgs p = slab_args(e, best, ws);
-  rc = launch_x6<MODE, NP>(p, st);
+  rc = x6(p);
   if (rc) return rc;
   return launch_fixup(e, p, st, "x6 tail fix-up");
 }
@@ -1530,6 +1547,132 @@
   const bool vec = al16(dy0) && al16(dy1) && al16(dy2) && al16(w0) && al16(w1) && al16(w2) &&
                    (lddy % 4 == 0) && (ldw % 4 == 0) && (nper % 4 == 0) && (K % 4 == 0);
   return launch<true, false>(g, vec, (hipStream_t)stream, ws, ws ? ws_bytes : 0);
+}
+
+namespace {
+
+bool seg_offsets(const float* const* p, int nseg, int32_t* out) {
+  for (int s = 0; s < SEG_MAX; ++s) out[s] = 0;
+  if (!p || !p[0]) return true;
+  for (int s = 0; s < nseg; ++s) {
+    const int64_t d = p[s] - p[0];
+    if (d < INT32_MIN || d > INT32_MAX) return false;
+    out[s] = (int32_t)d;
+  }
+  return true;
+}
+
+inline uint32_t seg_magic(int64_t nper) {
+  const int64_t tiles = nper / XBK;
+  return tiles >= 2 ? (uint32_t)((1ull << 32) / (uint64_t)tiles + 1) : 0u;
+}
+
+template <bool B_KC>
+bool nseg_takes_x6(const GemmArgs& g, const SegTab& t, bool vec, const float* ws, int64_t ws_bytes, int* splits) {
+  const int mode = gemm_mode();
+  if (mode != GCT_GEMM_BF16X6 && mode != GCT_GEMM_BF16X3) return false;
+  if (!x6n_ok<B_KC ? X6_FWD : X6_DGRAD>(g, t, vec)) return false;
+  const GemmRoute r = plan_gemm<true, B_KC>(g, vec, mode, ws, ws_bytes);
+  *splits = r.kind == GemmRoute::X6_SPLITK_ALL ? r.splits : 1;
+  return r.kind == GemmRoute::X6 || (!B_KC && r.kind == GemmRoute::X6_SPLITK_ALL);
+}
+
+}
+
+extern "C" int gct_linear_fwd_n(const float* x, int64_t ldx, int64_t M, int K, const float* const* w, int64_t ldw,
+                                const uint16_t* wp0, int64_t plane_stride, const float* const* b, int nseg, int nper,
+                                float* const* y, int64_t ldy, float* ws, int64_t ws_bytes, void* stream) {
+  GCT_CHECK_ARG(x && w && y && M >= 0 && K > 0 && nseg >= 1 && nseg <= SEG_MAX && nper > 0, "linear_fwd_n: bad args");
+  GCT_CHECK_ARG(ws_bytes >= 0, "linear_fwd_n: negative workspace size");
+  for (int s = 0; s < nseg; ++s) {
+    GCT_CHECK_ARG(w[s] && y[s], "linear_fwd_n: missing segment %d", s);
+    GCT_CHECK_ARG(!b || !b[0] || b[s], "linear_fwd_n: bias of segment %d missing", s);
+  }
+  const bool has_b = b && b[0];
+  auto group = [&](int s0, int n) {
+    auto at = [&](const float* const* p, int i) { return i < n ? p[s0 + i] : nullptr; };
+    return gct_linear_fwd(x, ldx, M, K, at(w, 0), at(w, 1), at(w, 2), ldw, wp0 ? wp0 + (w[s0] - w[0]) : nullptr,
+                          plane_stride, has_b ? at(b, 0) : nullptr, has_b ? at(b, 1) : nullptr,
+                          has_b ? at(b, 2) : nullptr, n, nper, y[s0], n > 1 ? y[s0 + 1] : nullptr,
+                          n > 2 ? y[s0 + 2] : nullptr, ldy, GCT_EPI_BIAS, nullptr, nullptr, 0.f, 0, 0, ws, ws_bytes,
+                          nullptr, stream);
+  };
+  if (nseg <= 3) return group(0, nseg);
+  GemmArgsN ga = {};
+  GemmArgs& g = ga.g;
+  g.M = M; g.N = (int64_t)nseg * nper; g.K = K;
+  g.a = mkseg(x, nullptr, nullptr); g.lda = ldx; g.a_nper = INT64_MAX / 4;
+  g.b = mkseg(w[0], w[1], w[2]); g.ldb = ldw; g.b_nper = nper;
+  g.c0 = y[0]; g.c_d1 = y[1] - y[0]; g.c_d2 = y[2] - y[0]; g.ldc = ldy; g.c_nper = nper;
+  g.ksplit = K; g.nsplit = 1; g.epi = GCT_EPI_BIAS;
+  g.bias0 = has_b ? b[0] : nullptr; g.bias_d1 = has_b ? b[1] - b[0] : 0; g.bias_d2 = has_b ? b[2] - b[0] : 0;
+  g.keep_scale = 1.0f;
+  g.bp0 = wp0; g.bp_stride = plane_stride;
+  bool vec = al16(x) && (ldx % 4 == 0) && (ldw % 4 == 0) && (K % 4 == 0);
+  for (int s = 0; s < nseg; ++s) vec = vec && al16(w[s]);
+  ga.t.nseg = nseg; ga.t.magic = seg_magic(nper);
+  const bool fits = seg_offsets(nullptr, nseg, ga.t.a) && seg_offsets(w, nseg, ga.t.b) &&
+                    seg_offsets(y, nseg, ga.t.c) && seg_offsets(has_b ? b : nullptr, nseg, ga.t.bias);
+  int splits = 1;
+  if (fits && M > 0 && nseg_takes_x6<true>(g, ga.t, vec, ws, ws ? ws_bytes : 0, &splits)) {
+    const bool x3 = gemm_mode() == GCT_GEMM_BF16X3;
+    if (!x3) ++g_gemm_launches[1];
+    return x3 ? launch_x6_tail_split<X6_FWD, 2>(g, (hipStream_t)stream, ws, ws ? ws_bytes : 0, &ga.t)
+              : launch_x6_tail_split<X6_FWD, 3>(g, (hipStream_t)stream, ws, ws ? ws_bytes : 0, &ga.t);
+  }
+  for (int s0 = 0; s0 < nseg; s0 += 3) {
+    const int rc = group(s0, nseg - s0 < 3 ? nseg - s0 : 3);
+    if (rc) return rc;
+  }
+  return GCT_OK;
+}
+
+extern "C" int gct_linear_dgrad_n(const float* const* dy, int64_t lddy, int64_t M, int nseg, int nper,
+                                  const float* const* w, int64_t ldw, const uint16_t* wp0, int64_t plane_stride, int K,
+                                  float* dx, int64_t lddx, int depi, float* ws, int64_t ws_bytes, void* stream) {
+  GCT_CHECK_ARG(dy && w && dx && M >= 0 && K > 0 && nseg >= 1 && nseg <= SEG_MAX && nper > 0, "linear_dgrad_n: bad args");
+  GCT_CHECK_ARG(ws_bytes >= 0, "linear_dgrad_n: negative workspace size");
+  GCT_CHECK_ARG(depi == GCT_DEPI_STORE || depi == GCT_DEPI_ACCUM, "linear_dgrad_n: epilogue %d (store or accumulate only)", depi);
+  for (int s = 0; s < nseg; ++s) GCT_CHECK_ARG(w[s] && dy[s], "linear_dgrad_n: missing segment %d", s);
+  auto group = [&](int s0, int n, int epi) {
+    auto at = [&](const float* const* p, int i) { return i < n ? p[s0 + i] : nullptr; };
+    return gct_linear_dgrad(at(dy, 0), at(dy, 1), at(dy, 2), lddy, M, n, nper, at(w, 0), at(w, 1), at(w, 2), ldw,
+                            wp0 ? wp0 + (w[s0] - w[0]) : nullptr, plane_stride, K, dx, lddx, epi, nullptr, 0.f, 0, 0,
+                            ws, ws_bytes, nullptr, 0, stream);
+  };
+  if (nseg <= 3) return group(0, nseg, depi);
+  GemmArgsN ga = {};
+  GemmArgs& g = ga.g;
+  g.M = M; g.N = K; g.K = (int64_t)nseg * nper;
+  g.a = mkseg(dy[0], dy[1], dy[2]); g.lda = lddy; g.a_nper = nper;
+  g.b = mkseg(w[0], w[1], w[2]); g.ldb = ldw; g.b_nper = nper;
+  g.c0 = dx; g.ldc = lddx; g.c_nper = INT64_MAX / 4;
+  g.ksplit = g.K; g.nsplit = 1; g.epi = EPI_D0 + depi;
+  g.keep_scale = 1.0f;
+  g.bp0 = wp0; g.bp_stride = plane_stride;
+  bool vec = (lddy % 4 == 0) && (ldw % 4 == 0) && (nper % 4 == 0) && (K % 4 == 0);
+  for (int s = 0; s < nseg; ++s) vec = vec && al16(dy[s]) && al16(w[s]);
+  ga.t.nseg = nseg; ga.t.magic = seg_magic(nper);
+  const bool fits = seg_offsets(dy, nseg, ga.t.a) && seg_offsets(w, nseg, ga.t.b) &&
+                    seg_offsets(nullptr, nseg, ga.t.c) && seg_offsets(nullptr, nseg, ga.t.bias);
+  int splits = 1;
+  if (fits && M > 0 && nseg_takes_x6<false>(g, ga.t, vec, ws, ws ? ws_bytes : 0, &splits)) {
+    const bool x3 = gemm_mode() == GCT_GEMM_BF16X3;
+    if (!x3) ++g_gemm_launches[1];
+    if (splits > 1) {
+      const GemmArgs p = slab_args(g, splits, ws);
+      int rc = x3 ? launch_x6n<X6_DGRAD, 2>(p, ga.t, (hipStream_t)stream) : launch_x6n<X6_DGRAD, 3>(p, ga.t, (hipStream_t)stream);
+      if (!rc) rc = launch_fixup(g, p, (hipStream_t)stream, "x6 split-K fix-up");
+      return rc;
+    }
+    return x3 ? launch_x6_tail_split<X6_DGRAD, 2>(g, (hipStream_t)stream, ws, ws ? ws_bytes : 0, &ga.t)
+              : launch_x6_tail_split<X6_DGRAD, 3>(g, (hipStream_t)stream, ws, ws ? ws_bytes : 0, &ga.t);
+  }
+  for (int s0 = 0; s0 < nseg; s0 += 3) {
+    const int rc = group(s0, nseg - s0 < 3 ? nseg - s0 : 3, s0 == 0 ? depi : GCT_DEPI_ACCUM);
+    if (rc) return rc;
+  }
+  return GCT_OK;
 }
 
 extern "C" int gct_linear_wgrad(const float* dy0, const float* dy1, const float* dy2, int64_t lddy,
diff --git a/gct_plus_amd/csrc/gemm_x6.inc b/gct_plus_amd/csrc/gemm_x6.inc
--- a/gct_plus_amd/csrc/gemm_x6.inc
+++ b/gct_plus_amd/csrc/gemm_x6.inc
@@ -70,22 +70,44 @@
 typedef float x6_f32x4 __attribute__((ext_vector_type(4)));
 #define X6_MFMA(a_, b_, c_) c_ = __builtin_amdgcn_mfma_f32_16x16x32_bf16(a_, b_, c_, 0, 0, 0)
 
-template <int MODE, int NP = 3>
-__global__ __launch_bounds__(512) __attribute__((amdgpu_waves_per_eu(2, 2))) void
-gemm_x6_kernel(const GemmArgs g) {
+template <int MODE, int NP, bool NSEG>
+__device__ __forceinline__ void gemm_x6_body(const GemmArgs& gk, const SegTab* tab) {
   static_assert(NP == 2 || NP == 3, "bf16x3 or bf16x6");
+  static_assert(!NSEG || MODE != X6_WGRAD, "the weight gradient takes at most three segments");
   extern __shared__ __attribute__((aligned(16))) unsigned char xlds[];
   constexpr bool A_TR = MODE == X6_WGRAD, B_TR = MODE != X6_FWD, B_PL = MODE != X6_WGRAD;
   constexpr int NB = B_PL ? 2 : 4;
   const int tid = threadIdx.x, lane = tid & 63, wave = tid >> 6;
   const int wm = (wave >> 2) * 64, wn = (wave & 3) * 64;
 
-  const unsigned tiles_n = (unsigned)((g.N + XBN - 1) / XBN);
-  const unsigned tiles_m = (unsigned)((g.M + XBM - 1) / XBM);
+  const unsigned tiles_n = (unsigned)((gk.N + XBN - 1) / XBN);
+  const unsigned tiles_m = (unsigned)((gk.M + XBM - 1) / XBM);
   const unsigned per_split = tiles_m * tiles_n;
   const unsigned lid = gct_xcd_remap(blockIdx.x, gridDim.x);
   const unsigned z = lid / per_split, rest = lid - z * per_split;
   const int64_t m0 = (int64_t)(rest / tiles_n) * XBM, n0 = (int64_t)(rest % tiles_n) * XBN;
+
+  int tab_a = 0, tab_b = 0;
+  uint32_t seg_magic = 0;
+  if constexpr (NSEG) {
+    const int tl = lane < SEG_MAX ? lane : 0;
+    tab_a = tab->a[tl];
+    tab_b = tab->b[tl];
+    seg_magic = tab->magic;
+  }
+  auto seg_of = [&](int64_t idx) -> int { return (int)__umulhi((uint32_t)(idx >> 5), seg_magic); };
+  GemmArgs gseg;
+  if constexpr (NSEG && MODE == X6_FWD) {
+    gseg = gk;
+    if (gk.epi != EPI_SLAB) {
+      const int s = seg_of(n0);
+      const int64_t back = (int64_t)s * gk.c_nper;
+      gseg.c0 = gk.c0 + ((int64_t)tab->c[s] - back);
+      if (gk.bias0) gseg.bias0 = gk.bias0 + ((int64_t)tab->bias[s] - back);
+      gseg.c_nper = INT64_MAX / 4;
+    }
+  }
+  const GemmArgs& g = (NSEG && MODE == X6_FWD) ? gseg : gk;
   const int64_t kbeg = (int64_t)z * g.ksplit;
   const int64_t kend = (kbeg + g.ksplit < g.K) ? kbeg + g.ksplit : g.K;
 
@@ -137,17 +159,34 @@
     int64_t loc;
     if (A_TR) { a_fix = seg_off(g.a, m0, g.a_nper, loc); a_fix += loc; }
     else a_fix = m0 * g.lda;
-    if (MODE == X6_FWD) { b_fix = seg_off(g.b, n0, g.b_nper, loc); b_fix += loc * g.ldb; }
-    else b_fix = n0;
+    if (MODE == X6_FWD) {
+      if constexpr (NSEG) {
+        const int s = seg_of(n0);
+        b_fix = (int64_t)__builtin_amdgcn_readlane(tab_b, s) + (n0 - (int64_t)s * g.b_nper) * g.ldb;
+      } else {
+        b_fix = seg_off(g.b, n0, g.b_nper, loc);
+        b_fix += loc * g.ldb;
+      }
+    } else {
+      b_fix = n0;
+    }
   }
   auto abase = [&](int64_t k0) -> const float* {
     if (A_TR) return g.a.p0 + a_fix + k0 * g.lda;
+    if constexpr (NSEG && MODE == X6_DGRAD) {
+      const int s = seg_of(k0);
+      return g.a.p0 + (int64_t)__builtin_amdgcn_readlane(tab_a, s) + a_fix + (k0 - (int64_t)s * g.a_nper);
+    }
     int64_t loc;
     const int64_t so = seg_off(g.a, k0, g.a_nper, loc);
     return g.a.p0 + so + a_fix + loc;
   };
   auto boff = [&](int64_t k0) -> int64_t {
     if (MODE == X6_FWD) return b_fix + k0;
+    if constexpr (NSEG) {
+      const int s = seg_of(k0);
+      return (int64_t)__builtin_amdgcn_readlane(tab_b, s) + (k0 - (int64_t)s * g.b_nper) * g.ldb + b_fix;
+    }
     int64_t loc;
     const int64_t so = seg_off(g.b, k0, g.b_nper, loc);
     return so + loc * g.ldb + b_fix;
@@ -508,6 +547,18 @@
 #endif
 }
 
+template <int MODE, int NP = 3>
+__global__ __launch_bounds__(512) __attribute__((amdgpu_waves_per_eu(2, 2))) void
+gemm_x6_kernel(const GemmArgs g) {
+  gemm_x6_body<MODE, NP, false>(g, nullptr);
+}
+
+template <int MODE, int NP = 3>
+__global__ __launch_bounds__(512) __attribute__((amdgpu_waves_per_eu(2, 2))) void
+gemm_x6n_kernel(const GemmArgsN ga) {
+  gemm_x6_body<MODE, NP, true>(ga.g, &ga.t);
+}
+
 template <int MODE>
 bool x6_ok(const GemmArgs& g, bool vec, int fwd_bn = XBN) {
   auto seg_ok = [](int64_t nper, int64_t extent, int64_t gran) { return nper >= extent || nper % gran == 0; };
@@ -525,6 +576,44 @@
     return g.bp0 && seg_ok(g.a_nper, g.K, XBK) && seg_ok(g.b_nper, g.K, XBK) && g.N % 8 == 0 && g.ldb % 8 == 0 &&
            g.b.d1 % 8 == 0 && g.b.d2 % 8 == 0 && g.bp_stride % 8 == 0 && (((uintptr_t)g.bp0) & 15u) == 0;
   return seg_ok(g.a_nper, g.M, XBM) && g.M % 4 == 0;
+}
+
+template <int MODE>
+bool x6n_ok(const GemmArgs& g, const SegTab& t, bool vec) {
+  if (MODE == X6_WGRAD || !x6_ok<MODE>(g, vec)) return false;
+  const int64_t nper = g.b_nper;
+  if (nper % XBK != 0 || nper < 2 * XBK || nper / XBK >= 65536 || g.K / XBK >= 65536 || g.N / XBK >= 65536) return false;
+  if (MODE == X6_FWD && nper % XBN != 0) return false;
+  for (int s = 0; s < t.nseg; ++s)
+    if (t.a[s] % 4 != 0 || t.b[s] % 8 != 0 || t.c[s] % 4 != 0 || t.bias[s] % 4 != 0) return false;
+  return true;
+}
+
+template <int MODE, int NP>
+int launch_x6n(const GemmArgs& g, const SegTab& t, hipStream_t st) {
+  const int64_t tiles = ((g.M + XBM - 1) / XBM) * ((g.N + XBN - 1) / XBN) * g.nsplit;
+  if (tiles <= 0) return GCT_OK;
+  if (tiles > INT_MAX) {
+    gct_set_error("gemm_x6n: grid too large");
+    return GCT_ERR_ARG;
+  }
+  static bool attr_set = false;
+  if (!attr_set) {
+    hipError_t e = hipFuncSetAttribute((const void*)gemm_x6n_kernel<MODE, NP>,
+                                       hipFuncAttributeMaxDynamicSharedMemorySize, X_LDS_BYTES);
+    if (e != hipSuccess) {
+      gct_set_error("gemm_x6n: cannot reserve %d bytes of LDS: %s", X_LDS_BYTES, hipGetErrorString(e));
+      return GCT_ERR_HIP;
+    }
+    attr_set = true;
+  }
+  GemmArgsN ga;
+  ga.g = g;
+  ga.t = t;
+  hipLaunchKernelGGL((gemm_x6n_kernel<MODE, NP>), dim3((unsigned)tiles), dim3(512), X_LDS_BYTES, st, ga);
+  ++(NP == 3 ? g_x6_kernel_launches : g_x3_kernel_launches);
+  GCT_LAUNCH_CHECK("gemm_x6n");
+  return GCT_OK;
 }
 
 template <int MODE, int NP>
diff --git a/gct_plus_amd/engine.py b/gct_plus_amd/engine.py
--- a/gct_plus_amd/engine.py
+++ b/gct_plus_amd/engine.py
@@ -16,6 +16,7 @@
 COMPACT_KV = os.environ.get("GCT_COMPACT_KV", "1") != "0"
 COMPACT_FWD = os.environ.get("GCT_COMPACT_FWD", "1") != "0"
 COMPACT_ENC_KV = os.environ.get("GCT_COMPACT_ENC_KV", "1") != "0"
+GROUP_KV = os.environ.get("GCT_GROUP_KV", "1") != "0"
 
 
 GRAD_NOTIFY = None
@@ -43,15 +44,18 @@
     enc_rows: int = 0
     dec_rows: int = 0
     live_rows: int = 0
+    group_kv: bool = False
 
 
 def plan_rows(caller, B=0, T=0, Le=0, mask_shape=None, *, loss_rows=False, trg_mask=False, get_attn=False,
               cond2dec=False, cond2lat=False, nconds=0, n_enc=0, n_dec=0, capturing=False, compact_fwd=False,
-              compact_kv=False, compact_enc_kv=False) -> RowMaps:
+              compact_kv=False, compact_enc_kv=False, group_kv=False) -> RowMaps:
     c2d = cond2dec and nconds > 0
     nc_lat = nconds if (not c2d and cond2lat and nconds > 0) else 0
     Td, Lk = T + (nconds if c2d else 0), Le + nc_lat
-    none = RowMaps(nc_lat=nc_lat, enc_rows=B * Le, dec_rows=B * Lk, live_rows=B * Td)
+    grp = bool(group_kv and caller in (MODEL, DECODER) and not capturing and not get_attn
+               and 2 <= n_dec <= ops.MAX_SEGS // 2)
+    none = RowMaps(nc_lat=nc_lat, enc_rows=B * Le, dec_rows=B * Lk, live_rows=B * Td, group_kv=grp)
     if caller == ENCODER or capturing:
         return none
     if caller == MODEL:
@@ -71,8 +75,8 @@
 
 class RowPlan:
 
-    def __init__(self, ek=None, dk=None, lr=None, rows=(0, 0, 0)):
-        self._maps, self._rows = (ek, dk, lr), rows
+    def __init__(self, ek=None, dk=None, lr=None, rows=(0, 0, 0), group_kv=False):
+        self._maps, self._rows, self.group_kv = (ek, dk, lr), rows, group_kv
         self._pending = ops.PendingReadBack(ek, dk, lr)
         self._usable = None
         self.enc_keys = self.dec_keys = self.live = None
@@ -92,9 +96,10 @@
                          get_attn=getattr(dec, "get_attn", False), cond2dec=getattr(dec, "use_cond2dec", False),
                          cond2lat=getattr(dec, "use_cond2lat", False), nconds=getattr(dec, "nconds", 0), n_enc=n_enc,
                          n_dec=0 if dec is None else len(dec.layers), capturing=torch.cuda.is_current_stream_capturing(),
-                         compact_fwd=COMPACT_FWD, compact_kv=COMPACT_KV, compact_enc_kv=COMPACT_ENC_KV)
+                         compact_fwd=COMPACT_FWD, compact_kv=COMPACT_KV, compact_enc_kv=COMPACT_ENC_KV,
+                         group_kv=GROUP_KV)
         if not (want.enc_keys or want.dec_keys or want.live):
-            return cls()
+            return cls(group_kv=want.group_kv)
         ek = dk = lr = None
         if want.enc_keys or want.dec_keys:
             sm = ops.to_mask_u8(src_mask).view(B, Le)
@@ -108,7 +113,7 @@
         if want.live:
             lr = ops.LiveRows.from_rows(loss_rows.to(torch.uint8).contiguous().reshape(B, T), B, T,
                                         ops.to_mask_u8(trg_mask))
-        return cls(ek, dk, lr, (want.enc_rows, want.dec_rows, want.live_rows))
+        return cls(ek, dk, lr, (want.enc_rows, want.dec_rows, want.live_rows), want.group_kv)
 
     def finish(self) -> "RowPlan":
         if self._usable is None:
@@ -261,9 +266,11 @@
     trg_mask_u8: Optional[torch.Tensor]
     keys: object
     live: object
-
-
-def mha_fwd(run: Run, m, xq, xkv, B, Lq, Lk, mask_u8, resid, want_probs=False, keys=None, live=None):
+    z2c: Optional[torch.Tensor] = None
+    grouped: bool = False
+
+
+def mha_fwd(run: Run, m, xq, xkv, B, Lq, Lk, mask_u8, resid, want_probs=False, keys=None, live=None, kv=None):
     d, H = m.d_model, m.h
     dk = d // H
     self_attn = xkv is xq
@@ -283,10 +290,13 @@
     else:
         qb = _empty(Mq, d, xq)
         ops.linear_fwd(xq, [m.q_linear.weight], [m.q_linear.bias], [qb], d)
-        kvb = _empty(B * Lk, 2 * d, xkv) if keys is None else keys.empty(2 * d)
-        ops.linear_fwd(xkv, [m.k_linear.weight, m.v_linear.weight],
-                       [m.k_linear.bias, m.v_linear.bias], [kvb, kvb[:, d:]], 2 * d)
-        q, k, v, ldq, ldkv = qb, kvb, kvb[:, d:], d, 2 * d
+        if kv is not None:
+            kvb = kv
+        else:
+            kvb = _empty(B * Lk, 2 * d, xkv) if keys is None else keys.empty(2 * d)
+            ops.linear_fwd(xkv, [m.k_linear.weight, m.v_linear.weight],
+                           [m.k_linear.bias, m.v_linear.bias], [kvb, kvb[:, d:]], 2 * d)
+        q, k, v, ldq, ldkv = qb, kvb, kvb[:, d:], d, kvb.stride(0)
     site_p = run.site()
     o, lse, probs = ops.attn_fwd(q, k, v, ldq, ldkv, ldkv, mask_u8, B, H, Lq, Lk, dk, run.p,
                                  run.seed, site_p, want_probs=want_probs, keys=keys, live=live)
@@ -303,7 +313,7 @@
 
 
 def mha_bwd(run: Run, m, sv: MhaSaved, dy, G: GradSink, dxq_out, depi_q, dxkv_out=None,
-            depi_kv=ops.DEPI_STORE, live=None, gdrop=None):
+            depi_kv=ops.DEPI_STORE, live=None, gdrop=None, dkv_out=None):
     B, Lq, Lk, keys = sv.B, sv.Lq, sv.Lk, sv.keys
     d, H = m.d_model, m.h
     dk = d // H
@@ -339,23 +349,26 @@
                          depi=depi_q)
     else:
         dq = new(d)
-        if keys is None:
+        if dkv_out is not None:
+            dkv = dkv_out
+        elif keys is None:
             dkv = _empty(Mk, 2 * d, dy)
         else:
             dkv = keys.empty_zero_gaps(2 * d)
-        ops.attn_bwd(sv.qb, sv.kvb, sv.kvb[:, d:], d, 2 * d, 2 * d, sv.mask_u8, sv.o, do, sv.lse, dq, dkv, dkv[:, d:],
-                     d, 2 * d, 2 * d, B, H, Lq, Lk, dk, run.p, run.seed, sv.site_p, live=live, keys=keys)
+        ldkv, lddkv = sv.kvb.stride(0), dkv.stride(0)
+        ops.attn_bwd(sv.qb, sv.kvb, sv.kvb[:, d:], d, ldkv, ldkv, sv.mask_u8, sv.o, do, sv.lse, dq, dkv, dkv[:, d:],
+                     d, lddkv, lddkv, B, H, Lq, Lk, dk, run.p, run.seed, sv.site_p, live=live, keys=keys)
         ops.linear_wgrad([dq], d, xq_in, [G(m.q_linear.weight)], [G(m.q_linear.bias)], kt=kt)
-        ops.linear_wgrad([dkv, dkv[:, d:]], 2 * d, sv.xkv,
+        ops.linear_wgrad([dkv, dkv[:, d:]], lddkv, sv.xkv,
                          [G(m.k_linear.weight), G(m.v_linear.weight)],
                          [G(m.k_linear.bias), G(m.v_linear.bias)])
         ops.linear_dgrad([dq], d, Mq, [m.q_linear.weight], dxq_out, depi=depi_q)
         if sv.self_split:
             dxk = keys.empty(d)
-            ops.linear_dgrad([dkv, dkv[:, d:]], 2 * d, Mk, [m.k_linear.weight, m.v_linear.weight], dxk)
+            ops.linear_dgrad([dkv, dkv[:, d:]], lddkv, Mk, [m.k_linear.weight, m.v_linear.weight], dxk)
             keys.scatter_add(dxk, dxq_out)
         elif dxkv_out is not None:
-            ops.linear_dgrad([dkv, dkv[:, d:]], 2 * d, Mk, [m.k_linear.weight, m.v_linear.weight],
+            ops.linear_dgrad([dkv, dkv[:, d:]], lddkv, Mk, [m.k_linear.weight, m.v_linear.weight],
                              dxkv_out, depi=depi_kv)
 
 
@@ -428,26 +441,29 @@
     return g, (None if dr is None else gdbuf)
 
 
-def dec_layer_fwd(run: Run, layer, x, e, B, T, Lk, src_mask_u8, trg_mask_u8, want_probs=False, keys=None, live=None):
+def dec_layer_fwd(run: Run, layer, x, e, B, T, Lk, src_mask_u8, trg_mask_u8, want_probs=False, keys=None, live=None,
+                  kv=None):
     x2, m1, r1 = ops.norm_fwd(x, layer.norm_1.alpha, layer.norm_1.bias, layer.norm_1.eps)
     xa, sa1, p1 = mha_fwd(run, layer.attn_1, x2, x2, B, T, T, trg_mask_u8, x, want_probs, live=live)
     x2, m2, r2 = ops.norm_fwd(xa, layer.norm_2.alpha, layer.norm_2.bias, layer.norm_2.eps)
-    xb, sa2, p2 = mha_fwd(run, layer.attn_2, x2, e, B, T, Lk, src_mask_u8, xa, want_probs, keys=keys, live=live)
+    xb, sa2, p2 = mha_fwd(run, layer.attn_2, x2, e, B, T, Lk, src_mask_u8, xa, want_probs, keys=keys, live=live,
+                          kv=kv)
     x2, m3, r3 = ops.norm_fwd(xb, layer.norm_3.alpha, layer.norm_3.bias, layer.norm_3.eps)
     xc, sf = ffn_fwd(run, layer.ff, x2, xb, live=live)
     return xc, DecLayerSaved(x, m1, r1, sa1, xa, m2, r2, sa2, xb, m3, r3, sf), p1, p2
 
 
 def dec_layer_bwd(run: Run, layer, sv: DecLayerSaved, g, de, first_de, G: GradSink, live=None, gd=None, gdbuf=None,
-                  below=None):
+                  below=None, dkv=None):
     t = torch.empty_like(g) if live is None else live.empty(g.shape[1])
     with ops.deferred_reductions():
         ffn_bwd(run, layer.ff, sv.ffn, g, G, t, ops.DEPI_STORE, live=live, gdrop=gd)
         dr = _mha_drop(run, sv.attn_2, gdbuf)
         ops.norm_bwd(t, sv.xb, layer.norm_3.alpha, sv.m3, sv.r3, G(layer.norm_3.alpha), G(layer.norm_3.bias),
                      dres=g, out=g, eps=layer.norm_3.eps, live=live, drop=dr)
-        mha_bwd(run, layer.attn_2, sv.attn_2, g, G, t, ops.DEPI_STORE, de,
-                ops.DEPI_STORE if first_de else ops.DEPI_ACCUM, live=live, gdrop=None if dr is None else gdbuf)
+        mha_bwd(run, layer.attn_2, sv.attn_2, g, G, t, ops.DEPI_STORE, None if dkv is not None else de,
+                ops.DEPI_STORE if first_de else ops.DEPI_ACCUM, live=live, gdrop=None if dr is None else gdbuf,
+                dkv_out=dkv)
         dr = _mha_drop(run, sv.attn_1, gdbuf)
         ops.norm_bwd(t, sv.xa, layer.norm_2.alpha, sv.m2, sv.r2, G(layer.norm_2.alpha), G(layer.norm_2.bias),
                      dres=g, out=g, eps=layer.norm_2.eps, live=live, drop=dr)
@@ -525,10 +541,16 @@
     site_pe = run.site()
     x = ops.embed_pe_fwd(trg, dec.embed.embed.weight, cond_x, _pe2d(dec.pe, T), nc if c2d else 0,
                          math.sqrt(d), run.p, run.seed, site_pe)
-    ez = _empty(B * Le, d, z2)
-    ops.linear_fwd(z2, [dec.fc_z.weight], [dec.fc_z.bias], [ez], d)
+    live, keys = plan.live, plan.dec_keys
+    z2c = None
+    if keys is not None and not c2l:
+        z2c = keys.gather(z2)
+        e = keys.empty(d)
+        ops.linear_fwd(z2c, [dec.fc_z.weight], [dec.fc_z.bias], [e], d)
+    else:
+        e = ez = _empty(B * Le, d, z2)
+        ops.linear_fwd(z2, [dec.fc_z.weight], [dec.fc_z.bias], [ez], d)
     Lk = Le
-    e = ez
     if c2l:
         Lk = Le + nc
         cl = ops.small_linear_fwd(dconds.contiguous(), dec.embed_cond2lat.weight,
@@ -540,21 +562,31 @@
             ones = torch.ones(B, nc, dtype=torch.uint8, device=src_mask_u8.device)
             src_mask_u8 = torch.cat([ones, src_mask_u8.view(B, Le)], dim=1).contiguous()
     layers, p1s, p2s = [], [], []
-    live, keys = plan.live, plan.dec_keys
     if live is not None:
         x = live.gather(x)
-    if keys is not None:
+    if keys is not None and z2c is None:
         e = keys.gather(e)
     src_m = ops.pack_mask(src_mask_u8, B, T, Lk)
     trg_m = ops.pack_mask(trg_mask_u8, B, T, T)
-    for layer in dec.layers:
-        x, sv, p1, p2 = dec_layer_fwd(run, layer, x, e, B, T, Lk, src_m, trg_m, want_probs, keys=keys, live=live)
+    nl = len(dec.layers)
+    grouped = bool(plan.group_kv and not want_probs and 2 <= nl <= ops.MAX_SEGS // 2)
+    kv_all = None
+    if grouped:
+        kv_all = _empty(e.shape[0], nl * 2 * d, e) if keys is None else keys.empty(nl * 2 * d)
+        att = [layer.attn_2 for layer in dec.layers]
+        ops.linear_fwd(e, [w for a in att for w in (a.k_linear.weight, a.v_linear.weight)],
+                       [b for a in att for b in (a.k_linear.bias, a.v_linear.bias)],
+                       [kv_all[:, c:] for c in range(0, nl * 2 * d, d)], nl * 2 * d)
+    for i, layer in enumerate(dec.layers):
+        x, sv, p1, p2 = dec_layer_fwd(run, layer, x, e, B, T, Lk, src_m, trg_m, want_probs, keys=keys, live=live,
+                                      kv=kv_all[:, i * 2 * d:(i + 1) * 2 * d] if grouped else None)
         layers.append(sv)
         p1s.append(p1)
         p2s.append(p2)
     y, mean, rstd = ops.norm_fwd(x, dec.norm.alpha, dec.norm.bias, dec.norm.eps)
     saved = DecoderSaved(trg, z2, dconds, site_pe, layers, x, mean, rstd, B, T, Le, Lk, c2d, c2l,
-                         trg_mask_u8.u8 if isinstance(trg_mask_u8, ops.MaskBits) else trg_mask_u8, keys, live)
+                         trg_mask_u8.u8 if isinstance(trg_mask_u8, ops.MaskBits) else trg_mask_u8, keys, live, z2c,
+                         grouped)
     if live is not None:
         return y, saved, p1s, p2s
     return y.view(B, T, d), saved, p1s, p2s
@@ -585,15 +617,24 @@
                  eps=dec.norm.eps, live=live, drop=dr)
     gd = None if dr is None else gdbuf
     de = new_de()
-    for i in range(len(layers) - 1, -1, -1):
-        g, gd = dec_layer_bwd(run, dec.layers[i], layers[i], g, de, i == len(layers) - 1, G, live=live, gd=gd,
-                              gdbuf=gdbuf, below=layers[i - 1].ffn if i > 0 else None)
+    nl, dkv_all = len(layers), None
+    if sv.grouped:
+        Mk = layers[0].attn_2.xkv.shape[0]
+        dkv_all = _empty(Mk, nl * 2 * d, dy) if keys is None else keys.empty_zero_gaps(nl * 2 * d)
+    for i in range(nl - 1, -1, -1):
+        g, gd = dec_layer_bwd(run, dec.layers[i], layers[i], g, de, i == nl - 1, G, live=live, gd=gd,
+                              gdbuf=gdbuf, below=layers[i - 1].ffn if i > 0 else None,
+                              dkv=dkv_all[:, i * 2 * d:(i + 1) * 2 * d] if sv.grouped else None)
+    if sv.grouped:
+        att = [layer.attn_2 for layer in dec.layers]
+        ops.linear_dgrad([dkv_all[:, c:] for c in range(0, nl * 2 * d, d)], nl * 2 * d, Mk,
+                         [w for a in att for w in (a.k_linear.weight, a.v_linear.weight)], de)
     run.kt = None
     if live is not None:
         g = live.scatter(g)
     if len(dec.layers) == 0:
         de.zero_()
-    if keys is not None:
+    if keys is not None and sv.z2c is None:
         de = keys.scatter(de)
     dcx = torch.empty(B, nc * d, dtype=torch.float32, device=g.device) if sv.c2d else None
     ops.embed_pe_bwd(g, sv.trg, G(dec.embed.embed.weight), dcx, nc if sv.c2d else 0, math.sqrt(d), run.p,
@@ -609,6 +650,14 @@
                              G(dec.embed_cond2lat.bias))
         dez = _empty(B * Le, d, g)
         ops.copy_rows(de, Lk, nc, dez, Le, 0, B * Le, Le, d)
+    if sv.z2c is not None:
+        ops.linear_wgrad([de], d, sv.z2c, [G(dec.fc_z.weight)], [G(dec.fc_z.bias)])
+        dz = None
+        if need_dz:
+            dzc = keys.empty(sv.z2.shape[1])
+            ops.linear_dgrad([de], d, de.shape[0], [dec.fc_z.weight], dzc)
+            dz = keys.scatter(dzc).view(B, Le, -1)
+        return dz
     ops.linear_wgrad([dez], d, sv.z2, [G(dec.fc_z.weight)], [G(dec.fc_z.bias)])
     dz = None
     if need_dz:
diff --git a/gct_plus_amd/ops.py b/gct_plus_amd/ops.py
--- a/gct_plus_amd/ops.py
+++ b/gct_plus_amd/ops.py
@@ -299,6 +299,8 @@
                live=None):
     M, K = x2d.shape
     nper = ws_[0].shape[0]
+    if len(ws_) > 3:
+        return _linear_fwd_n(x2d, ws_, bs, outs, ldy, epi, resid, pre, splitk_ws, ws, live)
     w = _seg3(ws_)
     b = _seg3(bs)
     y = _seg3(outs)
@@ -324,9 +326,66 @@
               "gct_linear_fwd")
 
 
+MAX_SEGS = 12
+
+
+def _ptr_array(ts: Sequence[torch.Tensor]):
+    import ctypes
+    arr = (ctypes.c_void_p * len(ts))(*[t.data_ptr() for t in ts])
+    return arr, ctypes.cast(arr, ctypes.c_void_p)
+
+
+def _linear_fwd_n(x2d, ws_, bs, outs, ldy, epi, resid, pre, splitk_ws, ws, live):
+    M, K = x2d.shape
+    nseg, nper = len(ws_), ws_[0].shape[0]
+    if nseg > MAX_SEGS or len(outs) != nseg or len(bs) != nseg:
+        raise _lib.GctError(f"linear_fwd: {nseg} weight segments, {len(bs)} biases, {len(outs)} outputs (at most {MAX_SEGS})")
+    if epi != EPI_BIAS or resid is not None or pre is not None or splitk_ws is not None or live is not None:
+        raise _lib.GctError("linear_fwd: more than three segments take the plain bias epilogue only")
+    has_b = bs[0] is not None
+    if any((t is not None) != has_b for t in bs):
+        raise _lib.GctError("linear_fwd: every segment has a bias, or none has")
+    for t in list(ws_) + list(outs) + (list(bs) if has_b else []):
+        _chk(t, "segment")
+    need = _ws_need("gct_linear_fwd_ws_bytes", M, K, nper * nseg)
+    if ws is not None and ws.numel() * 4 < need:
+        raise _lib.GctError(f"linear_fwd: workspace of {ws.numel() * 4} B < {need} B")
+    wp, pstride = _plane_ptr(ws_)
+    wsb = ws if ws is not None else (workspace(need, x2d.device) if need > 256 else None)
+    N = nper * nseg
+    wk, wa = _ptr_array(ws_)
+    yk, ya = _ptr_array(outs)
+    bk, ba = _ptr_array(bs) if has_b else (None, None)
+    with _Timed("gemm_fwd", 2.0 * M * K * N, 4 * M * K + (6 if wp else 4) * N * K + 4 * N + 4 * M * N):
+        check(_L().gct_linear_fwd_n(_p(x2d), x2d.stride(0), M, K, wa, ws_[0].stride(0), wp, pstride, ba, nseg, nper,
+                                    ya, ldy, _p(wsb), 0 if wsb is None else wsb.numel() * 4, _st()),
+              "gct_linear_fwd_n")
+    del wk, yk, bk
+
+
 def linear_dgrad(dys: Sequence[torch.Tensor], lddy: int, M: int, ws_: Sequence[torch.Tensor], dx,
                  depi=DEPI_STORE, pre=None, p=0.0, seed=0, site=0, live=None, pre_full=False):
     nper, K = ws_[0].shape
+    if len(ws_) > 3:
+        nseg = len(ws_)
+        if nseg > MAX_SEGS or len(dys) != nseg:
+            raise _lib.GctError(f"linear_dgrad: {nseg} weight segments, {len(dys)} gradients (at most {MAX_SEGS})")
+        if depi not in (DEPI_STORE, DEPI_ACCUM) or pre is not None or live is not None:
+            raise _lib.GctError("linear_dgrad: more than three segments store or accumulate only")
+        for t in list(ws_) + list(dys):
+            _chk(t, "segment")
+        _wait_pending(dx)
+        dk, da = _ptr_array(dys)
+        wk, wa = _ptr_array(ws_)
+        with _Timed("gemm_dgrad", 2.0 * M * K * nper * nseg):
+            wp, pstride = _plane_ptr(ws_)
+            need = _ws_need("gct_linear_dgrad_ws_bytes", M, nper * nseg, K)
+            wsb = workspace(need, dx.device) if need > 256 else None
+            check(_L().gct_linear_dgrad_n(da, lddy, M, nseg, nper, wa, ws_[0].stride(0), wp, pstride, K, _p(dx),
+                                          dx.stride(0), depi, _p(wsb), 0 if wsb is None else wsb.numel() * 4, _st()),
+                  "gct_linear_dgrad_n")
+        del dk, wk
+        return
     d = _seg3(dys)
     w = _seg3(ws_)
     _wait_pending(dx)
diff --git a/include/gctplus_hip.h b/include/gctplus_hip.h
--- a/include/gctplus_hip.h
+++ b/include/gctplus_hip.h
@@ -11,7 +11,7 @@
 #define GCT_ERR_ARG (-1)
 #define GCT_ERR_HIP (-2)
 
-#define GCT_ABI_VERSION 20
+#define GCT_ABI_VERSION 21
 
 int gct_version(void);
 const char* gct_last_error(void);
@@ -59,6 +59,14 @@
                      uint32_t site, float* ws, int64_t ws_bytes, const int32_t* quad_map, int64_t pre_rows,
                      void* stream);
 int64_t gct_linear_dgrad_ws_bytes(int64_t M, int Ntot, int K);
+
+#define GCT_MAX_SEGS 12
+int gct_linear_fwd_n(const float* x, int64_t ldx, int64_t M, int K, const float* const* w, int64_t ldw,
+                     const uint16_t* wp0, int64_t plane_stride, const float* const* b, int nseg, int nper,
+                     float* const* y, int64_t ldy, float* ws, int64_t ws_bytes, void* stream);
+int gct_linear_dgrad_n(const float* const* dy, int64_t lddy, int64_t M, int nseg, int nper,
+                       const float* const* w, int64_t ldw, const uint16_t* wp0, int64_t plane_stride, int K,
+                       float* dx, int64_t lddx, int depi, float* ws, int64_t ws_bytes, void* stream);
 
 int gct_linear_wgrad(const float* dy0, const float* dy1, const float* dy2, int64_t lddy,
                      int64_t M, int nseg, int nper, const float* x, int64_t ldx, int K,
```

Measured after the change: 10960, median of 6. About the same (+1.0%).
